# gavin-gqzhang/UniGen

Measured on NVIDIA B200. Metric: denoise steps/sec at 1024^2 Flux-arch +1 cond, higher is better.
Workload: dtype bf16

## Files before the change

### include/unigen_b200.h

```cpp
#ifndef UNIGEN_B200_H_
#define UNIGEN_B200_H_

#include <stddef.h>
#include <stdint.h>

#ifdef __cplusplus
extern "C" {
#endif

#define UG_ABI_VERSION 9

typedef enum {
  UG_OK = 0,
  UG_ERR_INVALID = -1,
  UG_ERR_UNSUPPORTED = -2,
  UG_ERR_CUDA = -3,
  UG_ERR_NO_DEVICE = -4
} ug_status;

const char* ug_last_error(void);
int ug_abi_version(void);
int ug_device_check(void);
int64_t ug_launch_count(void);
void ug_reset_launch_count(void);

#define UG_ACT_NONE 0
#define UG_ACT_GELU_TANH 1
#define UG_MAX_SEGMENTS 8
#define UG_MAX_PEERS 8
#define UG_PEER_HEADER_BYTES 4096
#define UG_PEER_HANDLE_BYTES 64

typedef struct ug_gemm_args {
  const void* a;
  int64_t a_row_stride;
  int64_t a_batch_stride;
  const void* w;
  int64_t w_row_stride;
  int64_t w_batch_stride;
  void* c;
  int64_t c_row_stride;
  int64_t c_batch_stride;
  int32_t batch;
  int32_t rows;
  int32_t n;
  int32_t k;
  const void* bias;
  int64_t bias_batch_stride;
  const float* gate;
  int64_t gate_batch_stride;
  float alpha;
  int32_t act;
  const void* residual;
  int64_t res_row_stride;
  int64_t res_batch_stride;
  int32_t variant;
  int32_t reserved;
  const float* lora_t;
  int64_t lora_t_row_stride;
  int64_t lora_t_batch_stride;
  const void* lora_b;
  int32_t lora_rank;
  int32_t lora_block_n;
  int32_t lora_nseg;
  int32_t lora_seg_bounds[UG_MAX_SEGMENTS + 1];
  int32_t lora_seg_group[UG_MAX_SEGMENTS];
  const void* qk_norm_weight;
  const float* qk_cos_sin;
  int32_t qk_head_dim;
  int32_t qk_d;
  float qk_eps;
  int32_t reserved2;
  int64_t gate_seg_stride;
  const void* a2;
  int64_t a2_row_stride, a2_batch_stride;
  const void* w2;
  int64_t w2_row_stride;
  int32_t k2;
  int32_t colmask_block;
} ug_gemm_args;

int ug_gemm_bf16(const ug_gemm_args* args, void* stream);

int ug_lora_down(const void* x, int64_t x_row_stride, int64_t x_batch_stride, const void* a_stack, float* t,
                 int64_t t_row_stride, int64_t t_batch_stride, int32_t batch, int32_t rows, int32_t k,
                 int32_t rank_total, int32_t nseg, const int32_t* seg_bounds_host, const int32_t* seg_group_host,
                 void* stream);
int ug_lora_down_wide(const void* x, int64_t x_row_stride, int64_t x_batch_stride, const void* a_stack, void* t_wide,
                      int64_t t_row_stride, int64_t t_batch_stride, int32_t batch, int32_t rows, int32_t k,
                      int32_t rank_total, int32_t groups, int32_t block, int32_t nseg, const int32_t* seg_bounds_host,
                      const int32_t* seg_group_host, void* stream);

typedef struct ug_attn_args {
  const void* q;
  const void* k;
  const void* v;
  void* o;
  int64_t q_row_stride, q_batch_stride;
  int64_t k_row_stride, k_batch_stride;
  int64_t v_row_stride, v_batch_stride;
  int64_t o_row_stride, o_batch_stride;
  int32_t batch, heads, seq, head_dim;
  float scale;
  int32_t n_seg;
  const int32_t* seg_bounds;
  const uint32_t* seg_visible;
  int32_t variant;
  int32_t reserved;
} ug_attn_args;

int ug_attention_bf16(const ug_attn_args* args, void* stream);
int ug_expand_segment_mask(int32_t seq, int32_t n_seg, const int32_t* seg_bounds_host,
                           const uint32_t* seg_visible_host, uint8_t* mask_dev, void* stream);

int ug_ln_modulate(const void* x, int64_t x_row_stride, int64_t x_batch_stride, void* out, int64_t o_row_stride,
                   int64_t o_batch_stride, const float* shift, const float* scale, int64_t mod_batch_stride,
                   int32_t batch, int32_t rows, int32_t d, float eps, void* stream);

int ug_ln_modulate_segs(const void* x, int64_t x_row_stride, int64_t x_batch_stride, void* out, int64_t o_row_stride,
                        int64_t o_batch_stride, const float* shift, const float* scale, int64_t mod_batch_stride,
                        int64_t mod_seg_stride, int32_t nseg, const int32_t* seg_bounds_host, int32_t batch, int32_t rows,
                        int32_t d, float eps, void* stream);

int ug_ln_modulate_slots(const void* x, int64_t x_row_stride, void* out, int64_t o_row_stride, const float* shift,
                         const float* scale, int64_t mod_expert_stride, int64_t mod_index_stride,
                         const int32_t* slot_token, int32_t experts, int32_t capacity, int32_t tokens_per_batch,
                         int32_t empty_index, int32_t d, float eps, void* stream);
int ug_gated_add_slots(void* x, int64_t x_row_stride, const void* y, int64_t y_row_stride, const float* gate,
                       int64_t mod_expert_stride, int64_t mod_index_stride, const int32_t* slot_token, int32_t experts,
                       int32_t capacity, int32_t tokens_per_batch, int32_t empty_index, int32_t d, void* stream);

int ug_qk_rmsnorm_rope(void* x, int64_t row_stride, int64_t batch_stride, int32_t batch, int32_t rows,
                       int32_t heads, int32_t head_dim, const void* norm_weight_bf16, int32_t heads_per_weight,
                       float eps, const float* cos_sin, void* stream);

int ug_rope_table(const float* ids, int32_t rows, const int32_t* axes_dim_host, float theta, float* cos_sin,
                  void* stream);

int ug_gemv(const float* x, int64_t x_stride, const void* w, const void* bias, float* out, int64_t out_stride,
            int32_t batch, int32_t n, int32_t k, int32_t silu_in, int32_t silu_out, int32_t accumulate,
            void* stream);

#define UG_MAX_GEMV_JOBS 1024
struct ug_peer_table;
typedef struct ug_gemv_job {
  const void* w;
  const void* bias;
  const float* x;
  float* out;
  int64_t x_stride, out_stride;
  int32_t n, k;
  int32_t first_group;
  int32_t flags;
} ug_gemv_job;
int ug_gemv_grouped(const ug_gemv_job* jobs_dev, int32_t n_jobs, int32_t total_groups, int32_t batch, int32_t group_begin,
                    int32_t group_end, const struct ug_peer_table* peers_or_null, void* stream);
int ug_silu_f32(const float* x, float* out, int64_t n, void* stream);

int ug_timestep_embedding(const float* t, int64_t t_stride, int32_t batch, int32_t dim, float scale, float* out, void* stream);

int ug_add_bf16(const void* a, int64_t a_row_stride, int64_t a_batch_stride, const void* b, int64_t b_row_stride,
                int64_t b_batch_stride, void* out, int64_t o_row_stride, int64_t o_batch_stride, int32_t batch,
                int32_t rows, int32_t d, void* stream);
int ug_copy_bf16(const void* src, int64_t s_row_stride, int64_t s_batch_stride, void* dst, int64_t d_row_stride,
                 int64_t d_batch_stride, int32_t batch, int32_t rows, int32_t d, void* stream);
int ug_cast_f32_to_bf16(const float* src, void* dst, int64_t n, void* stream);
int ug_cast_bf16_to_f32(const void* src, float* dst, int64_t n, void* stream);

int ug_moe_route(const void* x, const float* wg, const float* rts_uniform, int32_t tokens, int32_t d,
                 int32_t experts, int32_t capacity, int32_t* expert_idx, int32_t* slot, float* prob,
                 int32_t* slot_token, int64_t* exp_counts, float* l_aux, float* workspace, void* stream);

int ug_moe_gather_modulate(const void* x, const int32_t* slot_token, const float* mod, int64_t mod_expert_stride,
                           int64_t mod_batch_stride, const void* addend, void* out, int32_t experts,
                           int32_t capacity, int32_t tokens_per_batch, int32_t d, void* stream);
int ug_moe_combine(const void* y, const int32_t* expert_idx, const int32_t* slot, const float* prob, void* out,
                   int32_t tokens, int32_t capacity, int32_t d, void* stream);

int ug_euler_step(void* latents_bf16, const void* velocity_bf16, float sigma, float sigma_next, int64_t n, void* stream);
int ug_euler_step_table(void* latents_bf16, const void* velocity_bf16, const float* sigmas_dev, int32_t step, int64_t n,
                        void* stream);
int ug_cfg_combine(const void* uncond_bf16, const void* text_bf16, float guidance_scale, void* out_bf16, int64_t n, void* stream);
int ug_pack_latents(const void* src_bf16, void* dst_bf16, int32_t batch, int32_t channels, int32_t height, int32_t width,
                    int32_t unpack, void* stream);

typedef struct ug_peer_table {
  int32_t world, rank;
  void* base[UG_MAX_PEERS];
} ug_peer_table;

int ug_peer_alloc(size_t bytes, void** dev_ptr);
int ug_peer_free(void* dev_ptr);
int ug_peer_export(const void* dev_ptr, uint8_t handle[UG_PEER_HANDLE_BYTES]);
int ug_peer_open(const uint8_t handle[UG_PEER_HANDLE_BYTES], void** peer_ptr);
int ug_peer_close(void* peer_ptr);
int ug_peer_barrier(const ug_peer_table* table, void* stream);
int ug_peer_set_timeout_ms(int64_t milliseconds);
int ug_peer_error(const ug_peer_table* table, int32_t* error_host);
int ug_peer_error_async(const ug_peer_table* table, int32_t* error_host_pinned, void* stream);

typedef struct ug_qkv_scatter_args {
  const void* qkv;
  int64_t row_stride;
  int32_t rows, heads, head_dim;
  float eps;
  const void* norm_weight;
  const float* cos_sin;
  int64_t dst_offset;
  int32_t seq_total, dst_row0;
} ug_qkv_scatter_args;
int ug_qkv_scatter(const ug_peer_table* table, const ug_qkv_scatter_args* args, void* stream);

int ug_attention_bf16_peer(const ug_attn_args* args, const ug_peer_table* table, int64_t o_offset, int32_t rows_per_rank,
                           void* stream);

int ug_peer_bcast_rows(const ug_peer_table* table, const void* src, int64_t src_row_stride, int32_t rows, int32_t d,
                       int64_t dst_offset, int64_t dst_row_stride, int32_t dst_row0, void* stream);

int ug_unpatchify(const void* tokens_bf16, void* image_bf16, int32_t batch, int32_t h, int32_t w, int32_t p, int32_t channels,
                  void* stream);

#define UG_FLUX_MAX_CONDITIONS 4
typedef struct ug_flux_desc {
  int32_t num_layers, num_single_layers;
  int32_t heads, head_dim;
  int32_t in_channels, joint_dim, pooled_dim;
  int32_t guidance_embeds;
  int32_t axes_dims_rope[3];
  float theta;
  int32_t n_ctrl_double, n_ctrl_single;
  int32_t experts, condition_nums;
  int32_t use_shared_expert, single_add, use_pooled_prompt_embeds;
// ... 68 lines not shown
```

### unigen_b200/_lib.py

```python
from __future__ import annotations

import ctypes as C
from pathlib import Path

PKG_DIR = Path(__file__).resolve().parent
LIB_PATH = PKG_DIR / "libunigen_b200.so"

UG_ACT_NONE = 0
UG_ACT_GELU_TANH = 1
UG_MAX_SEGMENTS = 8
UG_GROUPNORM_MAX_CHUNKS = 1024
UG_ABI_VERSION = 9


class UgError(RuntimeError):
    pass


class GemmArgs(C.Structure):
    _fields_ = [
        ("a", C.c_void_p), ("a_row_stride", C.c_int64), ("a_batch_stride", C.c_int64),
        ("w", C.c_void_p), ("w_row_stride", C.c_int64), ("w_batch_stride", C.c_int64),
        ("c", C.c_void_p), ("c_row_stride", C.c_int64), ("c_batch_stride", C.c_int64),
        ("batch", C.c_int32), ("rows", C.c_int32), ("n", C.c_int32), ("k", C.c_int32),
        ("bias", C.c_void_p), ("bias_batch_stride", C.c_int64),
        ("gate", C.c_void_p), ("gate_batch_stride", C.c_int64),
        ("alpha", C.c_float), ("act", C.c_int32),
        ("residual", C.c_void_p), ("res_row_stride", C.c_int64), ("res_batch_stride", C.c_int64),
        ("variant", C.c_int32), ("reserved", C.c_int32),
        ("lora_t", C.c_void_p), ("lora_t_row_stride", C.c_int64), ("lora_t_batch_stride", C.c_int64),
        ("lora_b", C.c_void_p), ("lora_rank", C.c_int32), ("lora_block_n", C.c_int32), ("lora_nseg", C.c_int32),
        ("lora_seg_bounds", C.c_int32 * (UG_MAX_SEGMENTS + 1)), ("lora_seg_group", C.c_int32 * UG_MAX_SEGMENTS),
        ("qk_norm_weight", C.c_void_p), ("qk_cos_sin", C.c_void_p), ("qk_head_dim", C.c_int32), ("qk_d", C.c_int32),
        ("qk_eps", C.c_float), ("reserved2", C.c_int32), ("gate_seg_stride", C.c_int64),
        ("a2", C.c_void_p), ("a2_row_stride", C.c_int64), ("a2_batch_stride", C.c_int64),
        ("w2", C.c_void_p), ("w2_row_stride", C.c_int64), ("k2", C.c_int32), ("colmask_block", C.c_int32),
    ]


class Conv2dArgs(C.Structure):
    _fields_ = [("x", C.c_void_p), ("w", C.c_void_p), ("bias", C.c_void_p), ("residual", C.c_void_p), ("res_pixel_stride", C.c_int64),
                ("y", C.c_void_p), ("y_pixel_stride", C.c_int64), ("batch", C.c_int32), ("h", C.c_int32), ("w_px", C.c_int32),
                ("c_in", C.c_int32), ("c_out", C.c_int32), ("alpha", C.c_float), ("variant", C.c_int32), ("reserved", C.c_int32)]


UG_MAX_PEERS = 8
UG_PEER_HEADER_BYTES = 4096
UG_PEER_HANDLE_BYTES = 64


class PeerTable(C.Structure):
    _fields_ = [("world", C.c_int32), ("rank", C.c_int32), ("base", C.c_void_p * UG_MAX_PEERS)]


class QkvScatterArgs(C.Structure):
    _fields_ = [("qkv", C.c_void_p), ("row_stride", C.c_int64), ("rows", C.c_int32), ("heads", C.c_int32),
                ("head_dim", C.c_int32), ("eps", C.c_float), ("norm_weight", C.c_void_p), ("cos_sin", C.c_void_p),
                ("dst_offset", C.c_int64), ("seq_total", C.c_int32), ("dst_row0", C.c_int32)]


UG_MAX_GEMV_JOBS = 1024


class GemvJob(C.Structure):
    _fields_ = [("w", C.c_void_p), ("bias", C.c_void_p), ("x", C.c_void_p), ("out", C.c_void_p),
                ("x_stride", C.c_int64), ("out_stride", C.c_int64), ("n", C.c_int32), ("k", C.c_int32),
                ("first_group", C.c_int32), ("flags", C.c_int32)]


UG_FLUX_MAX_CONDITIONS = 4


class FluxDesc(C.Structure):
    _fields_ = [("num_layers", C.c_int32), ("num_single_layers", C.c_int32), ("heads", C.c_int32), ("head_dim", C.c_int32),
                ("in_channels", C.c_int32), ("joint_dim", C.c_int32), ("pooled_dim", C.c_int32), ("guidance_embeds", C.c_int32),
                ("axes_dims_rope", C.c_int32 * 3), ("theta", C.c_float), ("n_ctrl_double", C.c_int32), ("n_ctrl_single", C.c_int32),
                ("experts", C.c_int32), ("condition_nums", C.c_int32), ("use_shared_expert", C.c_int32), ("single_add", C.c_int32),
                ("use_pooled_prompt_embeds", C.c_int32)]


class FluxInputs(C.Structure):
    _fields_ = [("batch", C.c_int32), ("n_img", C.c_int32), ("n_txt", C.c_int32), ("conditioning_scale", C.c_float),
                ("hidden_states", C.c_void_p), ("encoder_hidden_states", C.c_void_p), ("pooled_projections", C.c_void_p),
                ("timestep", C.c_void_p), ("timestep_stride", C.c_int64), ("guidance", C.c_void_p), ("img_ids", C.c_void_p),
                ("txt_ids", C.c_void_p), ("condition_hidden_states", C.c_void_p * UG_FLUX_MAX_CONDITIONS),
                ("condition_pooled_projections", C.c_void_p * UG_FLUX_MAX_CONDITIONS),
                ("condition_ids", C.c_void_p * UG_FLUX_MAX_CONDITIONS), ("rts_uniform", C.c_void_p * UG_FLUX_MAX_CONDITIONS)]


class FluxOutputs(C.Structure):
    _fields_ = [("velocity", C.c_void_p), ("expert_counts", C.c_void_p), ("l_aux", C.c_void_p)]


class AttnArgs(C.Structure):
    _fields_ = [
        ("q", C.c_void_p), ("k", C.c_void_p), ("v", C.c_void_p), ("o", C.c_void_p),
        ("q_row_stride", C.c_int64), ("q_batch_stride", C.c_int64),
        ("k_row_stride", C.c_int64), ("k_batch_stride", C.c_int64),
        ("v_row_stride", C.c_int64), ("v_batch_stride", C.c_int64),
        ("o_row_stride", C.c_int64), ("o_batch_stride", C.c_int64),
        ("batch", C.c_int32), ("heads", C.c_int32), ("seq", C.c_int32), ("head_dim", C.c_int32),
        ("scale", C.c_float), ("n_seg", C.c_int32),
        ("seg_bounds", C.POINTER(C.c_int32)), ("seg_visible", C.POINTER(C.c_uint32)),
        ("variant", C.c_int32), ("reserved", C.c_int32),
    ]


_VP, _I32, _I64, _F32 = C.c_void_p, C.c_int32, C.c_int64, C.c_float
SIGNATURES = {
    "ug_last_error": (C.c_char_p, []),
    "ug_abi_version": (C.c_int, []),
    "ug_device_check": (C.c_int, []),
    "ug_launch_count": (C.c_int64, []),
    "ug_reset_launch_count": (None, []),
    "ug_gemm_bf16": (C.c_int, [C.POINTER(GemmArgs), _VP]),
    "ug_lora_down": (C.c_int, [_VP, _I64, _I64, _VP, _VP, _I64, _I64, _I32, _I32, _I32, _I32, _I32,
                               C.POINTER(C.c_int32), C.POINTER(C.c_int32), _VP]),
    "ug_lora_down_wide": (C.c_int, [_VP, _I64, _I64, _VP, _VP, _I64, _I64, _I32, _I32, _I32, _I32, _I32, _I32, _I32,
                                    C.POINTER(C.c_int32), C.POINTER(C.c_int32), _VP]),
    "ug_attention_bf16": (C.c_int, [C.POINTER(AttnArgs), _VP]),
    "ug_expand_segment_mask": (C.c_int, [_I32, _I32, C.POINTER(C.c_int32), C.POINTER(C.c_uint32), _VP, _VP]),
    "ug_ln_modulate": (C.c_int, [_VP, _I64, _I64, _VP, _I64, _I64, _VP, _VP, _I64, _I32, _I32, _I32, _F32, _VP]),
    "ug_ln_modulate_segs": (C.c_int, [_VP, _I64, _I64, _VP, _I64, _I64, _VP, _VP, _I64, _I64, _I32, C.POINTER(C.c_int32), _I32, _I32,
                                      _I32, _F32, _VP]),
    "ug_ln_modulate_slots": (C.c_int, [_VP, _I64, _VP, _I64, _VP, _VP, _I64, _I64, _VP, _I32, _I32, _I32, _I32, _I32, _F32, _VP]),
    "ug_gated_add_slots": (C.c_int, [_VP, _I64, _VP, _I64, _VP, _I64, _I64, _VP, _I32, _I32, _I32, _I32, _I32, _VP]),
    "ug_qk_rmsnorm_rope": (C.c_int, [_VP, _I64, _I64, _I32, _I32, _I32, _I32, _VP, _I32, _F32, _VP, _VP]),
    "ug_rope_table": (C.c_int, [_VP, _I32, C.POINTER(C.c_int32), _F32, _VP, _VP]),
    "ug_gemv": (C.c_int, [_VP, _I64, _VP, _VP, _VP, _I64, _I32, _I32, _I32, _I32, _I32, _I32, _VP]),
    "ug_gemv_grouped": (C.c_int, [_VP, _I32, _I32, _I32, _I32, _I32, C.POINTER(PeerTable), _VP]),
    "ug_silu_f32": (C.c_int, [_VP, _VP, _I64, _VP]),
    "ug_flux_create": (C.c_int, [C.POINTER(FluxDesc), C.POINTER(C.c_void_p)]),
    "ug_flux_destroy": (None, [_VP]),
    "ug_flux_bind_weight": (C.c_int, [_VP, C.c_char_p, _VP, _I32, C.POINTER(C.c_int64), _I32]),
    "ug_flux_workspace_bytes": (C.c_size_t, [_VP, _I32, _I32, _I32]),
    "ug_flux_forward": (C.c_int, [_VP, C.POINTER(FluxInputs), C.POINTER(FluxOutputs), _VP, C.c_size_t, _VP]),
    "ug_timestep_embedding": (C.c_int, [_VP, _I64, _I32, _I32, _F32, _VP, _VP]),
    "ug_add_bf16": (C.c_int, [_VP, _I64, _I64, _VP, _I64, _I64, _VP, _I64, _I64, _I32, _I32, _I32, _VP]),
    "ug_copy_bf16": (C.c_int, [_VP, _I64, _I64, _VP, _I64, _I64, _I32, _I32, _I32, _VP]),
    "ug_cast_f32_to_bf16": (C.c_int, [_VP, _VP, _I64, _VP]),
    "ug_cast_bf16_to_f32": (C.c_int, [_VP, _VP, _I64, _VP]),
    "ug_moe_route": (C.c_int, [_VP, _VP, _VP, _I32, _I32, _I32, _I32, _VP, _VP, _VP, _VP, _VP, _VP, _VP, _VP]),
    "ug_moe_gather_modulate": (C.c_int, [_VP, _VP, _VP, _I64, _I64, _VP, _VP, _I32, _I32, _I32, _I32, _VP]),
    "ug_moe_combine": (C.c_int, [_VP, _VP, _VP, _VP, _VP, _I32, _I32, _I32, _VP]),
    "ug_euler_step": (C.c_int, [_VP, _VP, _F32, _F32, _I64, _VP]),
    "ug_euler_step_table": (C.c_int, [_VP, _VP, _VP, _I32, _I64, _VP]),
    "ug_cfg_combine": (C.c_int, [_VP, _VP, _F32, _VP, _I64, _VP]),
    "ug_pack_latents": (C.c_int, [_VP, _VP, _I32, _I32, _I32, _I32, _I32, _VP]),
    "ug_peer_alloc": (C.c_int, [C.c_size_t, C.POINTER(C.c_void_p)]),
    "ug_peer_free": (C.c_int, [_VP]),
    "ug_peer_export": (C.c_int, [_VP, C.POINTER(C.c_uint8)]),
    "ug_peer_open": (C.c_int, [C.POINTER(C.c_uint8), C.POINTER(C.c_void_p)]),
    "ug_peer_close": (C.c_int, [_VP]),
    "ug_peer_barrier": (C.c_int, [C.POINTER(PeerTable), _VP]),
    "ug_peer_error": (C.c_int, [C.POINTER(PeerTable), C.POINTER(C.c_int32)]),
    "ug_peer_set_timeout_ms": (C.c_int, [_I64]),
    "ug_peer_error_async": (C.c_int, [C.POINTER(PeerTable), _VP, _VP]),
    "ug_qkv_scatter": (C.c_int, [C.POINTER(PeerTable), C.POINTER(QkvScatterArgs), _VP]),
    "ug_attention_bf16_peer": (C.c_int, [C.POINTER(AttnArgs), C.POINTER(PeerTable), _I64, _I32, _VP]),
    "ug_peer_bcast_rows": (C.c_int, [C.POINTER(PeerTable), _VP, _I64, _I32, _I32, _I64, _I64, _I32, _VP]),
    "ug_unpatchify": (C.c_int, [_VP, _VP, _I32, _I32, _I32, _I32, _I32, _VP]),
    "ug_conv3x3_bf16": (C.c_int, [C.POINTER(Conv2dArgs), _VP]),
    "ug_im2col_bf16": (C.c_int, [_VP, _I32, _I64, _I64, _I64, _I64, _VP, _I32, _I32, _I32, _I32, _I32, _I32, _I32, _I32, _I32, _I32, _I32,
                                 _I32, _F32, _F32, _VP]),
    "ug_groupnorm_bf16": (C.c_int, [_VP, _VP, _VP, _VP, _VP, _I32, _I32, _I32, _I32, _F32, _I32, _VP]),
    "ug_upsample2x_nhwc_bf16": (C.c_int, [_VP, _VP, _I32, _I32, _I32, _I32, _VP]),
    "ug_softmax_rows_bf16": (C.c_int, [_VP, _I64, _I32, _I32, _VP]),
    "ug_nhwc_to_nchw": (C.c_int, [_VP, _I64, _VP, _I32, _I32, _I32, _I32, _I32, _VP]),
    "ug_vae_sample": (C.c_int, [_VP, _I64, _VP, _VP, _I32, _I32, _I32, _F32, _F32, _VP]),
}

_lib = None


def load() -> C.CDLL:
    global _lib
    if _lib is not None:
        return _lib
    if not LIB_PATH.exists():
        raise UgError(
            f"{LIB_PATH} is missing: run `python -c 'import __graft_entry__ as g; g.build()'` "
            "(there is no CPU fallback for the UniGen hot path)")
    lib = C.CDLL(str(LIB_PATH))
    for name, (res, args) in SIGNATURES.items():
        fn = getattr(lib, name)
        fn.restype = res
        fn.argtypes = args
    got = int(lib.ug_abi_version())
    if got != UG_ABI_VERSION:
# ... 11 lines not shown
```

### unigen_b200/csrc/ug_flux.cu

```cuda
#include <cuda_bf16.h>

#include <cmath>
#include <cstring>
#include <map>
#include <string>
#include <vector>

#include "ug_host.h"

namespace {

struct Tensor {
  const void* p = nullptr;
  int dtype = 0;
  int64_t shape[4] = {0, 0, 0, 0};
  int ndim = 0;
};

struct Lin { const void* w = nullptr; const void* b = nullptr; };

struct DoubleW {
  Lin norm1, norm1_ctx, qkv, add_qkv, to_out, to_add_out, ff1, ff2, ffc1, ffc2;
  const void* rms = nullptr;
  const void* rms_ctx = nullptr;
};
struct SingleW { Lin norm, qkv, mlp, out; const void* rms = nullptr; };
struct TimeTextW { Lin t1, t2, g1, g2, p1, p2; };

struct View {
  void* p; int64_t rs, bs; int rows;
};

constexpr size_t kAlign = 256;
inline size_t align_up(size_t x) { return (x + kAlign - 1) / kAlign * kAlign; }

}

struct ug_flux {
  ug_flux_desc d;
  int D = 0;
  std::map<std::string, Tensor> weights;
  bool resolved = false;
  Lin x_embedder, context_embedder, norm_out, proj_out, control_context_embedder, control_x_embedder;
  TimeTextW time_text, control_time_text, control_condition;
  std::vector<DoubleW> dbl, cdbl, shared;
  std::vector<SingleW> sgl, csgl;
  std::vector<Lin> add_dbl, add_sgl;
  const float* gate_wg = nullptr;
  const void *exp_w[2] = {nullptr, nullptr}, *exp_b[2] = {nullptr, nullptr}, *exp_mod_w[2] = {nullptr, nullptr}, *exp_mod_b[2] = {nullptr, nullptr};
  cudaStream_t side = nullptr, text = nullptr;
  cudaEvent_t ev_fork = nullptr, ev_mod = nullptr, ev_t0 = nullptr, ev_t1 = nullptr;
  void* plan_ws = nullptr;
  int plan_B = 0, plan_N = 0, plan_T = 0;
  int early_jobs = 0, early_groups = 0, late_jobs = 0, late_groups = 0;
};

using namespace ug;

#define UG_TRY(expr)            \
  do {                          \
    int st__ = (expr);          \
    if (st__ != UG_OK) return st__; \
  } while (0)

extern "C" int ug_flux_create(const ug_flux_desc* desc, ug_flux** out) {
  UG_CHECK_ARG(desc && out, "flux_create: null argument");
  UG_CHECK_ARG(desc->num_layers >= 1 && desc->num_single_layers >= 0 && desc->heads >= 1 && (desc->head_dim == 64 || desc->head_dim == 128),
               "flux_create: bad architecture (head_dim must be 64 or 128)");
  UG_CHECK_ARG(desc->axes_dims_rope[0] + desc->axes_dims_rope[1] + desc->axes_dims_rope[2] == desc->head_dim,
               "flux_create: axes_dims_rope must sum to head_dim");
  UG_CHECK_ARG(desc->n_ctrl_double >= 1 && desc->n_ctrl_double <= desc->num_layers && desc->n_ctrl_single >= 0 &&
                   desc->n_ctrl_single <= desc->num_single_layers, "flux_create: control block counts out of range");
  UG_CHECK_ARG(desc->condition_nums >= 1 && desc->condition_nums <= UG_FLUX_MAX_CONDITIONS && desc->experts >= 1 && desc->experts <= 32,
               "flux_create: 1..%d conditions and 1..32 experts", UG_FLUX_MAX_CONDITIONS);
  ug_flux* h = new ug_flux();
  h->d = *desc;
  h->D = desc->heads * desc->head_dim;
  cudaError_t e = cudaStreamCreateWithFlags(&h->side, cudaStreamNonBlocking);
  if (e == cudaSuccess) e = cudaStreamCreateWithFlags(&h->text, cudaStreamNonBlocking);
  for (cudaEvent_t* ev : {&h->ev_fork, &h->ev_mod, &h->ev_t0, &h->ev_t1})
    if (e == cudaSuccess) e = cudaEventCreateWithFlags(ev, cudaEventDisableTiming);
  if (e != cudaSuccess) {
    set_error("flux_create: %s", cudaGetErrorString(e));
    delete h;
    return UG_ERR_CUDA;
  }
  *out = h;
  return UG_OK;
}

extern "C" void ug_flux_destroy(ug_flux* h) {
  if (!h) return;
  if (h->side) cudaStreamDestroy(h->side);
  if (h->text) cudaStreamDestroy(h->text);
  for (cudaEvent_t ev : {h->ev_fork, h->ev_mod, h->ev_t0, h->ev_t1})
    if (ev) cudaEventDestroy(ev);
  delete h;
}

extern "C" int ug_flux_bind_weight(ug_flux* h, const char* name, const void* dev_ptr, int32_t dtype, const int64_t* shape, int32_t ndim) {
  UG_CHECK_ARG(h && name && dev_ptr && shape && ndim >= 1 && ndim <= 4 && (dtype == 0 || dtype == 1), "flux_bind_weight: bad argument");
  Tensor t;
  t.p = dev_ptr; t.dtype = dtype; t.ndim = ndim;
  for (int i = 0; i < ndim; ++i) t.shape[i] = shape[i];
  h->weights[name] = t;
  h->resolved = false;
  h->plan_ws = nullptr;
  return UG_OK;
}

namespace {

struct Resolver {
  ug_flux* h;
  int status = UG_OK;
  const Tensor* get(const std::string& name, int dtype, int64_t s0, int64_t s1 = -1) {
    auto it = h->weights.find(name);
    if (it == h->weights.end()) { fail("weight %s is not bound", name); return nullptr; }
    const Tensor& t = it->second;
    if (t.dtype != dtype) { fail("weight %s has the wrong dtype", name); return nullptr; }
    if (t.shape[0] != s0 || (s1 >= 0 && (t.ndim < 2 || t.shape[1] != s1)) || (s1 < 0 && t.ndim != 1)) {
      fail("weight %s has the wrong shape", name);
      return nullptr;
    }
    return &t;
  }
  void fail(const char* fmt, const std::string& name) {
    if (status == UG_OK) { set_error(fmt, name.c_str()); status = UG_ERR_INVALID; }
  }
  Lin lin(const std::string& p, int64_t out_f, int64_t in_f) {
    Lin l;
    const Tensor* w = get(p + ".weight", 0, out_f, in_f);
    const Tensor* b = get(p + ".bias", 0, out_f);
    if (w && b) { l.w = w->p; l.b = b->p; }
    return l;
  }
  Lin fused(const std::vector<std::string>& names, int64_t out_each, int64_t in_f) {
    Lin first = lin(names[0], out_each, in_f);
    for (size_t i = 1; i < names.size() && status == UG_OK; ++i) {
      Lin l = lin(names[i], out_each, in_f);
      if (status != UG_OK) break;
      const char* want_w = static_cast<const char*>(first.w) + i * out_each * in_f * 2;
      const char* want_b = static_cast<const char*>(first.b) + i * out_each * 2;
      if (l.w != want_w || l.b != want_b) fail("%s: q / k / v (stacked expert) weights must be bound as one contiguous block", names[i]);
    }
    return first;
  }
  const void* rms_pair(const std::string& a, const std::string& b, int64_t dh) {
    const Tensor* ta = get(a, 0, dh);
    const Tensor* tb = get(b, 0, dh);
    if (!ta || !tb) return nullptr;
    if (static_cast<const char*>(tb->p) != static_cast<const char*>(ta->p) + dh * 2) fail("%s: norm_q / norm_k weights must be contiguous", b);
    return ta->p;
  }
  DoubleW dbl(const std::string& p, int64_t D, int64_t dh) {
    DoubleW w;
    w.norm1 = lin(p + ".norm1.linear", 6 * D, D);
    w.norm1_ctx = lin(p + ".norm1_context.linear", 6 * D, D);
    w.qkv = fused({p + ".attn.to_q", p + ".attn.to_k", p + ".attn.to_v"}, D, D);
    w.add_qkv = fused({p + ".attn.add_q_proj", p + ".attn.add_k_proj", p + ".attn.add_v_proj"}, D, D);
    w.to_out = lin(p + ".attn.to_out.0", D, D);
    w.to_add_out = lin(p + ".attn.to_add_out", D, D);
    w.rms = rms_pair(p + ".attn.norm_q.weight", p + ".attn.norm_k.weight", dh);
    w.rms_ctx = rms_pair(p + ".attn.norm_added_q.weight", p + ".attn.norm_added_k.weight", dh);
    w.ff1 = lin(p + ".ff.net.0.proj", 4 * D, D);
    w.ff2 = lin(p + ".ff.net.2", D, 4 * D);
    w.ffc1 = lin(p + ".ff_context.net.0.proj", 4 * D, D);
    w.ffc2 = lin(p + ".ff_context.net.2", D, 4 * D);
    return w;
  }
  SingleW sgl(const std::string& p, int64_t D, int64_t dh) {
    SingleW w;
    w.norm = lin(p + ".norm.linear", 3 * D, D);
    w.qkv = fused({p + ".attn.to_q", p + ".attn.to_k", p + ".attn.to_v"}, D, D);
    w.mlp = lin(p + ".proj_mlp", 4 * D, D);
    w.out = lin(p + ".proj_out", D, 5 * D);
    w.rms = rms_pair(p + ".attn.norm_q.weight", p + ".attn.norm_k.weight", dh);
    return w;
  }
  TimeTextW time_text(const std::string& p, int64_t D, int64_t pooled, bool guidance) {
    TimeTextW w;
    w.t1 = lin(p + ".timestep_embedder.linear_1", D, 256);
    w.t2 = lin(p + ".timestep_embedder.linear_2", D, D);
    if (guidance) {
      w.g1 = lin(p + ".guidance_embedder.linear_1", D, 256);
      w.g2 = lin(p + ".guidance_embedder.linear_2", D, D);
    }
    w.p1 = lin(p + ".text_embedder.linear_1", D, pooled);
    w.p2 = lin(p + ".text_embedder.linear_2", D, D);
    return w;
  }
};

int resolve(ug_flux* h) {
  if (h->resolved) return UG_OK;
  const ug_flux_desc& d = h->d;
  const int64_t D = h->D, dh = d.head_dim, P = d.pooled_dim, E = d.experts;
  Resolver r{h};
  auto idx = [](const char* p, int i) { return std::string(p) + "." + std::to_string(i); };
  h->x_embedder = r.lin("x_embedder", D, d.in_channels);
  h->context_embedder = r.lin("context_embedder", D, d.joint_dim);
  h->time_text = r.time_text("time_text_embed", D, P, d.guidance_embeds != 0);
  h->dbl.clear(); h->sgl.clear(); h->cdbl.clear(); h->csgl.clear(); h->add_dbl.clear(); h->add_sgl.clear(); h->shared.clear();
  for (int i = 0; i < d.num_layers; ++i) h->dbl.push_back(r.dbl(idx("transformer_blocks", i), D, dh));
  for (int i = 0; i < d.num_single_layers; ++i) h->sgl.push_back(r.sgl(idx("single_transformer_blocks", i), D, dh));
  h->norm_out = r.lin("norm_out.linear", 2 * D, D);
  h->proj_out = r.lin("proj_out", d.in_channels, D);
  h->control_time_text = r.time_text("control_time_text_embed", D, P, d.guidance_embeds != 0);
  h->control_condition = r.time_text("control_condition_embed", D, P, d.guidance_embeds != 0);
  h->control_context_embedder = r.lin("control_context_embedder", D, D);
  h->control_x_embedder = r.lin("control_x_embedder", D, d.in_channels);
  for (int j = 0; j < d.n_ctrl_double; ++j) {
    h->cdbl.push_back(r.dbl(idx("control_joint_trans_blocks", j), D, dh));
    h->add_dbl.push_back(r.lin(idx("controlnet_add_joint_blocks", j), D, D));
  }
  for (int j = 0; j < d.n_ctrl_single; ++j) {
    h->csgl.push_back(r.sgl(idx("control_single_trans_blocks", j), D, dh));
    h->add_sgl.push_back(r.lin(idx("controlnet_add_single_blocks", j), D, D));
  }
  if (const Tensor* g = r.get("moe.moe_layer.gate.wg.weight", 1, E, D)) h->gate_wg = static_cast<const float*>(g->p);
  for (int br = 0; br < 2; ++br) {
    std::vector<std::string> lin0, lin1;
    for (int e = 0; e < E; ++e) {
      const std::string p = "moe.moe_layer.experts.deepspeed_experts." + std::to_string(e) + "." + std::to_string(br);
      lin0.push_back(p + ".0");
      lin1.push_back(p + ".1");
    }
    Lin a = r.fused(lin0, D, D), m = r.fused(lin1, D, P);
    h->exp_w[br] = a.w; h->exp_b[br] = a.b; h->exp_mod_w[br] = m.w; h->exp_mod_b[br] = m.b;
  }
  if (d.use_shared_expert)
    for (int s = 0; s < 2; ++s) h->shared.push_back(r.dbl(idx("shared_expert", s), D, dh));
  if (r.status != UG_OK) return r.status;
  h->resolved = true;
  return UG_OK;
}

struct Layout {
  size_t X, NX, QKV, AO, FF, CAT, CH, CS, CENC, COND, HC, G, A, YC, YH, EH, EC, CIN, MOD, TEMBS, STEMBS, tmp, t_emb, g_emb, MODC, MODH,
      rope, rope0, rope1, NO, route_idx, route_slot, route_prob, route_slot_token, route_ws, jobs, total;
  int n_mod, capacity;
};

Layout make_layout(const ug_flux* h, int B, int N, int T) {
  const ug_flux_desc& d = h->d;
  const size_t D = h->D, S = T + N, Smax = T + 2 * (size_t)N, E = d.experts;
  Layout L;
  size_t off = 0;
  auto take = [&](size_t bytes) { size_t o = off; off = align_up(off + bytes); return o; };
  L.capacity = (int)((B * (size_t)N + E - 1) / E);
  if (L.capacity < 4) L.capacity = 4;
  const size_t C = L.capacity;
  L.n_mod = 12 * (d.num_layers + d.n_ctrl_double + 1 + d.condition_nums) + 3 * (d.num_single_layers + d.n_ctrl_single) + 2;
  L.X = take(B * S * D * 2); L.NX = take(B * Smax * D * 2); L.QKV = take(B * Smax * 3 * D * 2); L.AO = take(B * Smax * D * 2);
  L.FF = take(B * Smax * 4 * D * 2); L.CAT = take(B * S * 5 * D * 2); L.CH = take(B * (size_t)N * D * 2); L.CS = take(B * S * D * 2);
  L.CENC = take(B * (size_t)T * D * 2); L.COND = take(B * (size_t)N * D * 2); L.HC = take(B * 2 * (size_t)N * D * 2);
  L.G = take(B * (size_t)N * D * 2); L.A = take(E * C * D * 2); L.YC = take(E * C * D * 2); L.YH = take(E * C * D * 2);
  L.EH = take(B * (size_t)N * D * 2); L.EC = take(B * (size_t)N * D * 2); L.CIN = take(B * (size_t)N * D * 2);
  L.MOD = take((size_t)B * L.n_mod * D * 4);
  L.TEMBS = take((3 + d.condition_nums) * (size_t)B * D * 4); L.STEMBS = take((3 + d.condition_nums) * (size_t)B * D * 4);
  L.tmp = take((size_t)B * D * 4); L.t_emb = take((size_t)B * 256 * 4); L.g_emb = take((size_t)B * 256 * 4);
  L.MODC = take((size_t)B * E * D * 4); L.MODH = take((size_t)B * E * D * 4);
  L.rope = take(S * d.head_dim * 4); L.rope0 = take(2 * (size_t)N * d.head_dim * 4); L.rope1 = take(Smax * d.head_dim * 4);
  L.NO = take(B * (size_t)N * D * 2);
  L.route_idx = take((size_t)B * N * 4); L.route_slot = take((size_t)B * N * 4); L.route_prob = take((size_t)B * N * 4);
  L.route_slot_token = take(E * C * 4); L.route_ws = take(((size_t)B * N * E + E) * 4);
  L.jobs = take(UG_MAX_GEMV_JOBS * sizeof(ug_gemv_job));
  L.total = off;
  return L;
}

}

extern "C" size_t ug_flux_workspace_bytes(const ug_flux* h, int32_t batch, int32_t n_img, int32_t n_txt) {
  if (!h || batch < 1 || n_img < 1 || n_txt < 1) return 0;
  return make_layout(h, batch, n_img, n_txt).total;
}

namespace {

struct Step {
  ug_flux* h;
  const ug_flux_inputs* in;
  const ug_flux_outputs* out;
  char* ws;
  Layout L;
  cudaStream_t main;
  int B, N, T, S, D, H, dh, E;
  float cscale;
  float* mod(int slot) const { return reinterpret_cast<float*>(ws + L.MOD) + (size_t)slot * D; }
  int64_t mod_bs() const { return (int64_t)L.n_mod * D; }
  __nv_bfloat16* bf(size_t off) const { return reinterpret_cast<__nv_bfloat16*>(ws + off); }
  float* f32(size_t off) const { return reinterpret_cast<float*>(ws + off); }
  View view(size_t off, int row0, int rows, int64_t rs, int64_t total_rows) const {
    return View{bf(off) + (int64_t)row0 * rs, rs, total_rows * rs, rows};
  }

  int gemm(cudaStream_t s, View a, int k, Lin w, int n, View c, const float* gate = nullptr, const View* res = nullptr, int act = UG_ACT_NONE,
           float alpha = 1.0f, int batch = -1, int64_t w_batch_stride = 0, int64_t bias_batch_stride = 0, const void* qk_rms = nullptr,
           const float* qk_cos_sin = nullptr) const {
    ug_gemm_args g;
    memset(&g, 0, sizeof(g));
    g.a = a.p; g.a_row_stride = a.rs; g.a_batch_stride = a.bs;
    g.w = w.w; g.w_row_stride = k; g.w_batch_stride = w_batch_stride;
    g.c = c.p; g.c_row_stride = c.rs; g.c_batch_stride = c.bs;
    g.batch = batch < 0 ? B : batch; g.rows = a.rows; g.n = n; g.k = k;
    g.bias = w.b; g.bias_batch_stride = bias_batch_stride;
    g.gate = gate; g.gate_batch_stride = gate ? mod_bs() : 0;
    g.alpha = alpha; g.act = act;
    if (res) { g.residual = res->p; g.res_row_stride = res->rs; g.res_batch_stride = res->bs; }
    if (qk_rms) {
      g.qk_norm_weight = qk_rms; g.qk_cos_sin = qk_cos_sin; g.qk_head_dim = dh; g.qk_d = D; g.qk_eps = 1e-6f;
    }
    return ug_gemm_bf16(&g, s);
  }
  int ln(cudaStream_t s, View x, View o, const float* shift, const float* scale) const {
    return ug_ln_modulate(x.p, x.rs, x.bs, o.p, o.rs, o.bs, shift, scale, mod_bs(), B, x.rows, D, 1e-6f, s);
  }
  int gemv(const float* x, Lin w, float* o, int n, int k, int silu_out, int accumulate, int64_t x_stride, int64_t o_stride) const {
    return ug_gemv(x, x_stride, w.w, w.b, o, o_stride, B, n, k, 0, silu_out, accumulate, main);
  }
  int time_text(const TimeTextW& w, const float* pooled, int64_t pooled_stride, float* dst, bool accumulate) const {
    float* tmp = f32(L.tmp);
    UG_TRY(gemv(f32(L.t_emb), w.t1, tmp, D, 256, 1, 0, 256, D));
    UG_TRY(gemv(tmp, w.t2, dst, D, D, 0, accumulate ? 1 : 0, D, D));
    if (in->guidance && w.g1.w) {
      UG_TRY(gemv(f32(L.g_emb), w.g1, tmp, D, 256, 1, 0, 256, D));
      UG_TRY(gemv(tmp, w.g2, dst, D, D, 0, 1, D, D));
    }
    UG_TRY(gemv(pooled, w.p1, tmp, D, h->d.pooled_dim, 1, 0, pooled_stride, D));
    return gemv(tmp, w.p2, dst, D, D, 0, 1, D, D);
  }
  int rope(size_t off, std::initializer_list<std::pair<const float*, int>> tables) const {
    int r0 = 0;
    for (auto& t : tables) {
      UG_TRY(ug_rope_table(t.first, t.second, h->d.axes_dims_rope, h->d.theta, f32(off) + (size_t)r0 * dh, main));
      r0 += t.second;
    }
    return UG_OK;
  }
  int attention(int Sq, View o) const {
    ug_attn_args a;
    memset(&a, 0, sizeof(a));
    __nv_bfloat16* qkv = bf(L.QKV);
    const int64_t rs = 3 * (int64_t)D, bs = (int64_t)(T + 2 * N) * rs;
    a.q = qkv; a.k = qkv + D; a.v = qkv + 2 * D; a.o = o.p;
    a.q_row_stride = a.k_row_stride = a.v_row_stride = rs;
    a.q_batch_stride = a.k_batch_stride = a.v_batch_stride = bs;
    a.o_row_stride = o.rs; a.o_batch_stride = o.bs;
    a.batch = B; a.heads = H; a.seq = Sq; a.head_dim = dh;
    a.scale = (float)(1.0 / sqrt((double)dh));
    return ug_attention_bf16(&a, main);
  }
  int double_block(const DoubleW& w, int slot_smp, int slot_ctx, View smp_in, View ctx_in, View smp_out, const View* ctx_out, size_t rope_off) const {
    const int n_ctx = ctx_in.rows, n_smp = smp_in.rows, Sq = n_ctx + n_smp;
    const int64_t Smax = T + 2 * (int64_t)N;
    View nx_c = view(L.NX, 0, n_ctx, D, Smax), nx_s = view(L.NX, n_ctx, n_smp, D, Smax);
    View qkv_c = view(L.QKV, 0, n_ctx, 3 * D, Smax), qkv_s = view(L.QKV, n_ctx, n_smp, 3 * D, Smax);
    View ff_c = view(L.FF, 0, n_ctx, 4 * D, Smax), ff_s = view(L.FF, n_ctx, n_smp, 4 * D, Smax);
    View ao_c = view(L.AO, 0, n_ctx, D, Smax), ao_s = view(L.AO, n_ctx, n_smp, D, Smax), ao = view(L.AO, 0, Sq, D, Smax);
    const float *sh_a = mod(slot_smp), *sc_a = mod(slot_smp + 1), *g_a = mod(slot_smp + 2), *sh_m = mod(slot_smp + 3), *sc_m = mod(slot_smp + 4),
                *g_m = mod(slot_smp + 5);
    const float *csh_a = mod(slot_ctx), *csc_a = mod(slot_ctx + 1), *cg_a = mod(slot_ctx + 2), *csh_m = mod(slot_ctx + 3),
                *csc_m = mod(slot_ctx + 4), *cg_m = mod(slot_ctx + 5);
    const bool fork = ctx_out != nullptr;
    cudaStream_t ts = fork ? h->text : main;
    if (fork) { cudaEventRecord(h->ev_t0, main); cudaStreamWaitEvent(ts, h->ev_t0, 0); }
    const float* rp = f32(rope_off);
    UG_TRY(ln(ts, ctx_in, nx_c, csh_a, csc_a));
    UG_TRY(gemm(ts, nx_c, D, w.add_qkv, 3 * D, qkv_c, nullptr, nullptr, UG_ACT_NONE, 1.0f, -1, 0, 0, w.rms_ctx, rp));
    UG_TRY(ln(main, smp_in, nx_s, sh_a, sc_a));
    UG_TRY(gemm(main, nx_s, D, w.qkv, 3 * D, qkv_s, nullptr, nullptr, UG_ACT_NONE, 1.0f, -1, 0, 0, w.rms, rp + (size_t)n_ctx * dh));
    if (fork) { cudaEventRecord(h->ev_t1, ts); cudaStreamWaitEvent(main, h->ev_t1, 0); }
    UG_TRY(attention(Sq, ao));
    if (fork) {
      cudaEventRecord(h->ev_t0, main); cudaStreamWaitEvent(ts, h->ev_t0, 0);
      UG_TRY(gemm(ts, ao_c, D, w.to_add_out, D, *ctx_out, cg_a, &ctx_in));
      UG_TRY(ln(ts, *ctx_out, nx_c, csh_m, csc_m));
      UG_TRY(gemm(ts, nx_c, D, w.ffc1, 4 * D, ff_c, nullptr, nullptr, UG_ACT_GELU_TANH));
      UG_TRY(gemm(ts, ff_c, 4 * D, w.ffc2, D, *ctx_out, cg_m, ctx_out));
    }
    UG_TRY(gemm(main, ao_s, D, w.to_out, D, smp_out, g_a, &smp_in));
    UG_TRY(ln(main, smp_out, nx_s, sh_m, sc_m));
    UG_TRY(gemm(main, nx_s, D, w.ff1, 4 * D, ff_s, nullptr, nullptr, UG_ACT_GELU_TANH));
    UG_TRY(gemm(main, ff_s, 4 * D, w.ff2, D, smp_out, g_m, &smp_out));
    if (fork) { cudaEventRecord(h->ev_t1, ts); cudaStreamWaitEvent(main, h->ev_t1, 0); }
    return UG_OK;
  }

  int single_block(const SingleW& w, int slot, View x_in, View x_out) const {
    const int64_t Smax = T + 2 * (int64_t)N;
    View nx = view(L.NX, 0, S, D, Smax), qkv = view(L.QKV, 0, S, 3 * D, Smax);
    View cat = view(L.CAT, 0, S, 5 * D, S);
    View cat_attn = cat, cat_mlp = cat;
    cat_mlp.p = bf(L.CAT) + D;
    UG_TRY(ln(main, x_in, nx, mod(slot), mod(slot + 1)));
    UG_TRY(gemm(main, nx, D, w.qkv, 3 * D, qkv, nullptr, nullptr, UG_ACT_NONE, 1.0f, -1, 0, 0, w.rms, f32(L.rope)));
    UG_TRY(gemm(main, nx, D, w.mlp, 4 * D, cat_mlp, nullptr, nullptr, UG_ACT_GELU_TANH));
    UG_TRY(attention(S, cat_attn));
    return gemm(main, cat, 5 * D, w.out, D, x_out, mod(slot + 2), &x_in);
  }

  int add(View a, View b, View o) const {
    return ug_add_bf16(a.p, a.rs, a.bs, b.p, b.rs, b.bs, o.p, o.rs, o.bs, B, a.rows, D, main);
  }
};

struct JobBuilder {
  std::vector<ug_gemv_job> early, late;
  int g_early = 0, g_late = 0;
  void push(bool is_early, Lin w, const float* x, float* out, int n, int k, int64_t out_stride) {
    ug_gemv_job j;
    memset(&j, 0, sizeof(j));
    j.w = w.w; j.bias = w.b; j.x = x; j.out = out; j.x_stride = k; j.out_stride = out_stride; j.n = n; j.k = k; j.flags = 0;
    int& g = is_early ? g_early : g_late;
    j.first_group = g;
    g += (n + 3) / 4;
    (is_early ? early : late).push_back(j);
  }
};

}

extern "C" int ug_flux_forward(ug_flux* h, const ug_flux_inputs* in, const ug_flux_outputs* out, void* workspace, size_t workspace_bytes,
                               void* stream) {
  UG_CHECK_ARG(h && in && out && workspace, "flux_forward: null argument");
  UG_TRY(resolve(h));
  const ug_flux_desc& d = h->d;
  const int B = in->batch, N = in->n_img, T = in->n_txt, D = h->D, E = d.experts, n_cond = d.condition_nums;
  UG_CHECK_ARG(B >= 1 && B <= 8 && N >= 1 && T >= 1, "flux_forward: bad shape batch %d n_img %d n_txt %d (batch <= 8)", B, N, T);
  UG_CHECK_ARG(T != N, "flux_forward: T == N: the reference MOELayer would also dispatch the text tensor (unsupported)");
  UG_CHECK_ARG(in->hidden_states && in->encoder_hidden_states && in->pooled_projections && in->timestep && in->img_ids && in->txt_ids,
               "flux_forward: missing input");
  UG_CHECK_ARG(!in->guidance == !d.guidance_embeds || !in->guidance, "flux_forward: guidance given to a model without guidance embeddings");
  for (int c = 0; c < n_cond; ++c)
    UG_CHECK_ARG(in->condition_hidden_states[c] && in->condition_pooled_projections[c] && in->condition_ids[c] && in->rts_uniform[c],
                 "flux_forward: missing input of condition %d", c);
  UG_CHECK_ARG(out->velocity && out->expert_counts && out->l_aux, "flux_forward: missing output buffer");
  UG_CHECK_ARG((reinterpret_cast<uintptr_t>(workspace) & (kAlign - 1)) == 0, "flux_forward: workspace must be %d-byte aligned", (int)kAlign);
  Step s;
  s.h = h; s.in = in; s.out = out; s.ws = static_cast<char*>(workspace);
  s.L = make_layout(h, B, N, T);
  UG_CHECK_ARG(workspace_bytes >= s.L.total, "flux_forward: workspace of %zu bytes is smaller than ug_flux_workspace_bytes() = %zu",
               workspace_bytes, s.L.total);
  s.main = reinterpret_cast<cudaStream_t>(stream);
  s.B = B; s.N = N; s.T = T; s.S = T + N; s.D = D; s.H = d.heads; s.dh = d.head_dim; s.E = E;
  s.cscale = in->conditioning_scale;
  const Layout& L = s.L;
  const int S = s.S, C = L.capacity;
  const int64_t Smax = T + 2 * (int64_t)N;
  cudaStream_t main = s.main;

  const int nd = d.num_layers, ncd = d.n_ctrl_double, ns = d.num_single_layers, ncs = d.n_ctrl_single;
  std::vector<int> s_d(nd), s_dc(nd), s_cd(ncd), s_cdc(ncd), s_s(ns), s_cs(ncs), s_sh0(n_cond), s_sh0c(n_cond);
  int s_sh1 = 0, s_sh1c = 0, s_out = 0, slot = 0;
  float* stembs = s.f32(L.STEMBS);
  const float *s_temb = stembs, *s_ctemb = stembs + (size_t)B * D, *s_cdtemb = stembs + 2 * (size_t)B * D;
  JobBuilder jb;
  const int64_t mbs = s.mod_bs();
  auto job = [&](bool early, Lin w, const float* x, int chunks) {
    const int s0 = slot;
    slot += chunks;
    jb.push(early, w, x, s.mod(s0), chunks * D, D, mbs);
    return s0;
  };
  for (int i = 0; i < nd; ++i) { s_d[i] = job(i == 0, h->dbl[i].norm1, s_temb, 6); s_dc[i] = job(i == 0, h->dbl[i].norm1_ctx, s_temb, 6); }
  for (int j = 0; j < ncd; ++j) { s_cd[j] = job(j == 0, h->cdbl[j].norm1, s_cdtemb, 6); s_cdc[j] = job(j == 0, h->cdbl[j].norm1_ctx, s_cdtemb, 6); }
  for (int i = 0; i < ns; ++i) s_s[i] = job(false, h->sgl[i].norm, s_temb, 3);
  for (int j = 0; j < ncs; ++j) s_cs[j] = job(false, h->csgl[j].norm, s_cdtemb, 3);
  if (d.use_shared_expert) {
    for (int c = 0; c < n_cond; ++c) {
      const float* x = stembs + (size_t)(3 + c) * B * D;
      s_sh0[c] = job(true, h->shared[0].norm1, x, 6);
      s_sh0c[c] = job(true, h->shared[0].norm1_ctx, x, 6);
    }
    s_sh1 = job(true, h->shared[1].norm1, s_ctemb, 6);
    s_sh1c = job(true, h->shared[1].norm1_ctx, s_ctemb, 6);
  }
  s_out = job(false, h->norm_out, s_temb, 2);
  UG_CHECK_ARG(slot <= L.n_mod && jb.early.size() + jb.late.size() <= UG_MAX_GEMV_JOBS, "flux_forward: AdaLN job table overflow");
  ug_gemv_job* jobs_dev = reinterpret_cast<ug_gemv_job*>(s.ws + L.jobs);
  if (h->plan_ws != workspace || h->plan_B != B || h->plan_N != N || h->plan_T != T) {
    std::vector<ug_gemv_job> all(jb.early);
    all.insert(all.end(), jb.late.begin(), jb.late.end());
    cudaError_t e = cudaMemcpyAsync(jobs_dev, all.data(), all.size() * sizeof(ug_gemv_job), cudaMemcpyHostToDevice, main);
    if (e == cudaSuccess) e = cudaStreamSynchronize(main);
    if (e != cudaSuccess) {
      set_error("flux_forward: uploading the AdaLN job table failed: %s", cudaGetErrorString(e));
      return UG_ERR_CUDA;
    }
    h->plan_ws = workspace; h->plan_B = B; h->plan_N = N; h->plan_T = T;
  }

  View X = s.view(L.X, 0, S, D, S), x_txt = s.view(L.X, 0, T, D, S), x_img = s.view(L.X, T, N, D, S);
  View hs{const_cast<void*>(in->hidden_states), d.in_channels, (int64_t)N * d.in_channels, N};
  View es{const_cast<void*>(in->encoder_hidden_states), d.joint_dim, (int64_t)T * d.joint_dim, T};
  UG_TRY(s.gemm(main, hs, d.in_channels, h->x_embedder, D, x_img));
  UG_TRY(s.gemm(main, es, d.joint_dim, h->context_embedder, D, x_txt));
  UG_TRY(ug_timestep_embedding(in->timestep, in->timestep_stride, B, 256, 1000.0f, s.f32(L.t_emb), main));
  if (in->guidance) UG_TRY(ug_timestep_embedding(in->guidance, 1, B, 256, 1000.0f, s.f32(L.g_emb), main));
  float* tembs = s.f32(L.TEMBS);
  float *temb = tembs, *ctemb = tembs + (size_t)B * D, *cdtemb = tembs + 2 * (size_t)B * D;
  const int64_t P = d.pooled_dim;
  UG_TRY(s.time_text(h->time_text, in->pooled_projections, P, temb, false));
  if (d.use_pooled_prompt_embeds) {
    UG_TRY(s.time_text(h->control_time_text, in->pooled_projections, P, ctemb, false));
  } else {
    cudaMemsetAsync(s.f32(L.MODC), 0, (size_t)B * P * 4, main);
    UG_TRY(s.time_text(h->control_time_text, s.f32(L.MODC), P, ctemb, false));
  }
  for (int c = 0; c < n_cond; ++c) {
    UG_TRY(s.time_text(h->control_condition, in->condition_pooled_projections[c], P, tembs + (size_t)(3 + c) * B * D, false));
    UG_TRY(s.time_text(h->control_condition, in->condition_pooled_projections[c], P, cdtemb, c > 0));
  }
  UG_TRY(ug_silu_f32(tembs, stembs, (int64_t)(3 + n_cond) * B * D, main));
  UG_TRY(s.rope(L.rope, {{in->txt_ids, T}, {in->img_ids, N}}));

  const int n_early = (int)jb.early.size(), n_late = (int)jb.late.size();
  UG_TRY(ug_gemv_grouped(jobs_dev, n_early, jb.g_early, B, 0, jb.g_early, nullptr, main));
  cudaEventRecord(h->ev_fork, main);
  cudaStreamWaitEvent(h->side, h->ev_fork, 0);
  UG_TRY(ug_gemv_grouped(jobs_dev + n_early, n_late, jb.g_late, B, 0, jb.g_late, nullptr, h->side));
  cudaEventRecord(h->ev_mod, h->side);
  bool mods_joined = false;

  View CENC = s.view(L.CENC, 0, T, D, T), CH = s.view(L.CH, 0, N, D, N), CIN = s.view(L.CIN, 0, N, D, N), COND = s.view(L.COND, 0, N, D, N);
  bool routed = false;
  for (int i = 0; i < nd; ++i) {
    if (i == 1 && !mods_joined) { cudaStreamWaitEvent(main, h->ev_mod, 0); mods_joined = true; }
    UG_TRY(s.double_block(h->dbl[i], s_d[i], s_dc[i], x_img, x_txt, x_img, &x_txt, L.rope));
    const int j = (int)((double)i / ((double)nd / (double)ncd));
    View ctrl_in = x_img;
    if (!routed) {
      UG_TRY(s.gemm(main, x_txt, D, h->control_context_embedder, D, CENC));
      for (int c = 0; c < n_cond; ++c) {
        View cs{const_cast<void*>(in->condition_hidden_states[c]), d.in_channels, (int64_t)N * d.in_channels, N};
        UG_TRY(s.gemm(main, cs, d.in_channels, h->control_x_embedder, D, COND));
        UG_TRY(s.rope(L.rope0, {{in->condition_ids[c], N}, {in->img_ids, N}}));
        UG_TRY(s.rope(L.rope1, {{in->txt_ids, T}, {in->img_ids, N}, {in->condition_ids[c], N}}));
        View G = s.view(L.G, 0, N, D, N);
// ... 64 lines not shown
```

### unigen_b200/csrc/ug_gemm.cu

```cuda
#include <cstdlib>
#include <cstring>

#include "ug_host.h"
#include "ug_ptx.cuh"

namespace ug {

constexpr int kEpiWarps = 8;
constexpr int kGemmThreads = 64 + 32 * kEpiWarps;

struct GemmParams {
  int rows, n, k, batch;
  int m_tiles, n_tiles, k_blocks, total_tiles;
  int group_m;
  int k1_blocks;
  __nv_bfloat16* c;
  long long c_rs, c_bs;
  const __nv_bfloat16* bias;
  long long bias_bs;
  const float* gate;
  long long gate_bs;
  int colmask_block;
  long long gate_seg_stride;
  float alpha;
  int act;
  const __nv_bfloat16* res;
  long long res_rs, res_bs;
  int w_batched;
  const float* lora_t;
  long long lora_t_rs, lora_t_bs;
  const __nv_bfloat16* lora_b;
  int lora_r, lora_block_n, lora_nseg;
  int lora_bounds[UG_MAX_SEGMENTS + 1];
  int lora_group[UG_MAX_SEGMENTS];
  const __nv_bfloat16* qk_w;
  const float* qk_cos_sin;
  int qk_dh, qk_d;
  float qk_eps;
  int conv_cblocks, conv_w;
};

struct ConvDesc {
  const void* x;
  int batch, h, w, c_in;
};

template <int kCta, int BN, int kStages, bool kTmaEpi = false>
struct GemmCfg {
  static constexpr int BM = 128;
  static constexpr int BK = 64;
  static constexpr int BN_LOAD = BN / kCta;
  static constexpr int A_BYTES = BM * BK * 2;
  static constexpr int B_BYTES = BN_LOAD * BK * 2;
  static constexpr int STAGE_BYTES = A_BYTES + B_BYTES;
  static constexpr int TMEM_COLS = 2 * BN;
  static constexpr int EPI_SLABS = BN / (64 * (kEpiWarps / 4));
  static constexpr int EPI_SLAB_BYTES = 32 * 128;
  static constexpr int EPI_WARP_BYTES = EPI_SLABS * EPI_SLAB_BYTES;
  static constexpr int EPI_BYTES = kTmaEpi ? kEpiWarps * EPI_WARP_BYTES : 0;
  static constexpr int EPI_BARS = kTmaEpi ? kEpiWarps * EPI_SLABS : 0;
  static constexpr int BAR_BYTES = (2 * kStages + 4 + EPI_BARS) * 8 + 16;
  static constexpr int SMEM_BYTES = kStages * STAGE_BYTES + EPI_BYTES + BAR_BYTES + 1024;
  static_assert(TMEM_COLS == 256 || TMEM_COLS == 512, "TMEM allocation must be a power of two");
  static_assert(SMEM_BYTES <= 227 * 1024, "shared memory budget");
};

__device__ __forceinline__ int lora_group_of(const GemmParams& p, int r) {
  int g = -1;
  for (int s = 0; s < p.lora_nseg; ++s)
    if (r >= p.lora_bounds[s] && r < p.lora_bounds[s + 1]) g = p.lora_group[s];
  return g;
}

__device__ __forceinline__ int seg_index_of(const GemmParams& p, int r) {
  int g = 0;
  for (int s = 0; s < p.lora_nseg; ++s)
    if (r >= p.lora_bounds[s] && r < p.lora_bounds[s + 1]) g = s;
  return g;
}

__device__ __forceinline__ void epilogue_chunk(const GemmParams& p, const uint32_t (&v)[32], int b, int r, int col0,
                                               int lora_g, const float* gate_row) {
  const long long c_off = (long long)b * p.c_bs + (long long)r * p.c_rs;
  const long long r_off = (long long)b * p.res_bs + (long long)r * p.res_rs;
  uint4 rv4[4];
  if (p.res) {
#pragma unroll
    for (int j = 0; j < 4; ++j)
      rv4[j] = (col0 + 8 * j < p.n) ? *reinterpret_cast<const uint4*>(p.res + r_off + col0 + 8 * j) : make_uint4(0, 0, 0, 0);
  }
  float lt[16];
  const __nv_bfloat16* lb = nullptr;
  if (lora_g >= 0) {
    const float* tp = p.lora_t + (long long)b * p.lora_t_bs + (long long)r * p.lora_t_rs + (col0 / p.lora_block_n) * p.lora_r;
#pragma unroll
    for (int i = 0; i < 16; i += 4) {
      if (i < p.lora_r) {
        const float4 t4 = *reinterpret_cast<const float4*>(tp + i);
        lt[i] = t4.x; lt[i + 1] = t4.y; lt[i + 2] = t4.z; lt[i + 3] = t4.w;
      }
    }
    lb = p.lora_b + ((long long)lora_g * p.n) * p.lora_r;
  }
#pragma unroll
  for (int j = 0; j < 4; ++j) {
    const int c = col0 + 8 * j;
    if (c >= p.n) break;
    float x[8];
#pragma unroll
    for (int i = 0; i < 8; ++i) x[i] = __uint_as_float(v[8 * j + i]);
    if (lb) {
#pragma unroll
      for (int i = 0; i < 8; ++i) {
        const __nv_bfloat16* bp = lb + (long long)(c + i) * p.lora_r;
        float acc = 0.f;
#pragma unroll
        for (int q = 0; q < 16; q += 4) {
          if (q < p.lora_r) {
            const uint2 u = *reinterpret_cast<const uint2*>(bp + q);
            const float2 b0 = unpack_bf16x2(u.x), b1 = unpack_bf16x2(u.y);
            acc += lt[q] * b0.x + lt[q + 1] * b0.y + lt[q + 2] * b1.x + lt[q + 3] * b1.y;
          }
        }
        x[i] += acc;
      }
    }
    if (p.bias) {
      uint4 bv = *reinterpret_cast<const uint4*>(p.bias + (long long)b * p.bias_bs + c);
      float2 f0 = unpack_bf16x2(bv.x), f1 = unpack_bf16x2(bv.y), f2 = unpack_bf16x2(bv.z), f3 = unpack_bf16x2(bv.w);
      x[0] += f0.x; x[1] += f0.y; x[2] += f1.x; x[3] += f1.y;
      x[4] += f2.x; x[5] += f2.y; x[6] += f3.x; x[7] += f3.y;
    }
    if (p.act == UG_ACT_GELU_TANH) {
#pragma unroll
      for (int i = 0; i < 8; ++i) x[i] = gelu_tanh(x[i]);
    }
    if (gate_row) {
      const float* g = gate_row + c;
      float4 g0 = *reinterpret_cast<const float4*>(g), g1 = *reinterpret_cast<const float4*>(g + 4);
      x[0] *= g0.x * p.alpha; x[1] *= g0.y * p.alpha; x[2] *= g0.z * p.alpha; x[3] *= g0.w * p.alpha;
      x[4] *= g1.x * p.alpha; x[5] *= g1.y * p.alpha; x[6] *= g1.z * p.alpha; x[7] *= g1.w * p.alpha;
    } else if (p.alpha != 1.0f) {
#pragma unroll
      for (int i = 0; i < 8; ++i) x[i] *= p.alpha;
    }
    if (p.res) {
      const uint4 rv = rv4[j];
      float2 f0 = unpack_bf16x2(rv.x), f1 = unpack_bf16x2(rv.y), f2 = unpack_bf16x2(rv.z), f3 = unpack_bf16x2(rv.w);
      x[0] += f0.x; x[1] += f0.y; x[2] += f1.x; x[3] += f1.y;
      x[4] += f2.x; x[5] += f2.y; x[6] += f3.x; x[7] += f3.y;
    }
    uint4 o;
    o.x = pack_bf16x2(x[0], x[1]);
    o.y = pack_bf16x2(x[2], x[3]);
    o.z = pack_bf16x2(x[4], x[5]);
    o.w = pack_bf16x2(x[6], x[7]);
    *reinterpret_cast<uint4*>(p.c + c_off + c) = o;
  }
}

__device__ __forceinline__ uint4 epilogue_group8(const GemmParams& p, const uint32_t* v8, int b, int c, const float* gate_row,
                                                 const uint4& rv) {
  float x[8];
#pragma unroll
  for (int i = 0; i < 8; ++i) x[i] = __uint_as_float(v8[i]);
  if (p.bias) {
    const uint4 bv = *reinterpret_cast<const uint4*>(p.bias + (long long)b * p.bias_bs + c);
    const float2 f0 = unpack_bf16x2(bv.x), f1 = unpack_bf16x2(bv.y), f2 = unpack_bf16x2(bv.z), f3 = unpack_bf16x2(bv.w);
    x[0] += f0.x; x[1] += f0.y; x[2] += f1.x; x[3] += f1.y;
    x[4] += f2.x; x[5] += f2.y; x[6] += f3.x; x[7] += f3.y;
  }
  if (p.act == UG_ACT_GELU_TANH) {
#pragma unroll
    for (int i = 0; i < 8; ++i) x[i] = gelu_tanh(x[i]);
  }
  if (gate_row) {
    const float* g = gate_row + c;
    const float4 g0 = *reinterpret_cast<const float4*>(g), g1 = *reinterpret_cast<const float4*>(g + 4);
    x[0] *= g0.x * p.alpha; x[1] *= g0.y * p.alpha; x[2] *= g0.z * p.alpha; x[3] *= g0.w * p.alpha;
    x[4] *= g1.x * p.alpha; x[5] *= g1.y * p.alpha; x[6] *= g1.z * p.alpha; x[7] *= g1.w * p.alpha;
  } else if (p.alpha != 1.0f) {
#pragma unroll
    for (int i = 0; i < 8; ++i) x[i] *= p.alpha;
  }
  if (p.res) {
    const float2 f0 = unpack_bf16x2(rv.x), f1 = unpack_bf16x2(rv.y), f2 = unpack_bf16x2(rv.z), f3 = unpack_bf16x2(rv.w);
    x[0] += f0.x; x[1] += f0.y; x[2] += f1.x; x[3] += f1.y;
    x[4] += f2.x; x[5] += f2.y; x[6] += f3.x; x[7] += f3.y;
  }
  uint4 o;
  o.x = pack_bf16x2(x[0], x[1]);
  o.y = pack_bf16x2(x[2], x[3]);
  o.z = pack_bf16x2(x[4], x[5]);
  o.w = pack_bf16x2(x[6], x[7]);
  return o;
}

__device__ __forceinline__ uint4 epilogue_qk_group8(const GemmParams& p, const uint32_t* v8, int b, int r, int c, int which, float rstd) {
  const int c_in_head = c % p.qk_dh;
  float x[8];
#pragma unroll
  for (int i = 0; i < 8; ++i) x[i] = __uint_as_float(v8[i]);
  if (p.bias) {
    const uint4 bv = *reinterpret_cast<const uint4*>(p.bias + (long long)b * p.bias_bs + c);
    const float2 f0 = unpack_bf16x2(bv.x), f1 = unpack_bf16x2(bv.y), f2 = unpack_bf16x2(bv.z), f3 = unpack_bf16x2(bv.w);
    x[0] += f0.x; x[1] += f0.y; x[2] += f1.x; x[3] += f1.y;
    x[4] += f2.x; x[5] += f2.y; x[6] += f3.x; x[7] += f3.y;
  }
  const uint4 wv = *reinterpret_cast<const uint4*>(p.qk_w + which * p.qk_dh + c_in_head);
  const float2 w0 = unpack_bf16x2(wv.x), w1 = unpack_bf16x2(wv.y), w2 = unpack_bf16x2(wv.z), w3 = unpack_bf16x2(wv.w);
  x[0] *= rstd * w0.x; x[1] *= rstd * w0.y; x[2] *= rstd * w1.x; x[3] *= rstd * w1.y;
  x[4] *= rstd * w2.x; x[5] *= rstd * w2.y; x[6] *= rstd * w3.x; x[7] *= rstd * w3.y;
  if (p.qk_cos_sin) {
    const float* cs = p.qk_cos_sin + (long long)min(r, p.rows - 1) * p.qk_dh + c_in_head;
    const float4 t0 = __ldg(reinterpret_cast<const float4*>(cs)), t1 = __ldg(reinterpret_cast<const float4*>(cs + 4));
    const float co[4] = {t0.x, t0.z, t1.x, t1.z}, si[4] = {t0.y, t0.w, t1.y, t1.w};
#pragma unroll
    for (int q = 0; q < 4; ++q) {
      const float a0 = x[2 * q], a1 = x[2 * q + 1];
      x[2 * q] = a0 * co[q] - a1 * si[q];
      x[2 * q + 1] = a1 * co[q] + a0 * si[q];
    }
  }
  uint4 o;
  o.x = pack_bf16x2(x[0], x[1]);
  o.y = pack_bf16x2(x[2], x[3]);
  o.z = pack_bf16x2(x[4], x[5]);
  o.w = pack_bf16x2(x[6], x[7]);
  return o;
}

__device__ __forceinline__ void epilogue_qkv_chunk(const GemmParams& p, const uint32_t (&v)[32], int b, int r, int col0,
                                                   int c_in_head, int which, float rstd) {
  const long long c_off = (long long)b * p.c_bs + (long long)r * p.c_rs;
  const float* cs = (which < 2 && p.qk_cos_sin) ? p.qk_cos_sin + (long long)r * p.qk_dh + c_in_head : nullptr;
  const __nv_bfloat16* wq = p.qk_w + which * p.qk_dh + c_in_head;
#pragma unroll
  for (int j = 0; j < 4; ++j) {
    const int c = col0 + 8 * j;
    float x[8];
#pragma unroll
    for (int i = 0; i < 8; ++i) x[i] = __uint_as_float(v[8 * j + i]);
    if (p.bias) {
      uint4 bv = *reinterpret_cast<const uint4*>(p.bias + (long long)b * p.bias_bs + c);
      float2 f0 = unpack_bf16x2(bv.x), f1 = unpack_bf16x2(bv.y), f2 = unpack_bf16x2(bv.z), f3 = unpack_bf16x2(bv.w);
      x[0] += f0.x; x[1] += f0.y; x[2] += f1.x; x[3] += f1.y;
      x[4] += f2.x; x[5] += f2.y; x[6] += f3.x; x[7] += f3.y;
    }
    if (which < 2) {
      uint4 wv = *reinterpret_cast<const uint4*>(wq + 8 * j);
      float2 w0 = unpack_bf16x2(wv.x), w1 = unpack_bf16x2(wv.y), w2 = unpack_bf16x2(wv.z), w3 = unpack_bf16x2(wv.w);
      x[0] *= rstd * w0.x; x[1] *= rstd * w0.y; x[2] *= rstd * w1.x; x[3] *= rstd * w1.y;
      x[4] *= rstd * w2.x; x[5] *= rstd * w2.y; x[6] *= rstd * w3.x; x[7] *= rstd * w3.y;
      if (cs) {
        const float4 t0 = *reinterpret_cast<const float4*>(cs + 8 * j), t1 = *reinterpret_cast<const float4*>(cs + 8 * j + 4);
        const float co[4] = {t0.x, t0.z, t1.x, t1.z}, si[4] = {t0.y, t0.w, t1.y, t1.w};
#pragma unroll
        for (int q = 0; q < 4; ++q) {
          const float a0 = x[2 * q], a1 = x[2 * q + 1];
          x[2 * q] = a0 * co[q] - a1 * si[q];
          x[2 * q + 1] = a1 * co[q] + a0 * si[q];
        }
      }
    }
    uint4 o;
    o.x = pack_bf16x2(x[0], x[1]);
    o.y = pack_bf16x2(x[2], x[3]);
    o.z = pack_bf16x2(x[4], x[5]);
    o.w = pack_bf16x2(x[6], x[7]);
    *reinterpret_cast<uint4*>(p.c + c_off + c) = o;
  }
}

__device__ __forceinline__ float chunk_sumsq(const GemmParams& p, const uint32_t (&v)[32], int b, int col0) {
  float ss = 0.f;
#pragma unroll
  for (int j = 0; j < 4; ++j) {
    float x[8];
#pragma unroll
    for (int i = 0; i < 8; ++i) x[i] = __uint_as_float(v[8 * j + i]);
    if (p.bias) {
      uint4 bv = *reinterpret_cast<const uint4*>(p.bias + (long long)b * p.bias_bs + col0 + 8 * j);
      float2 f0 = unpack_bf16x2(bv.x), f1 = unpack_bf16x2(bv.y), f2 = unpack_bf16x2(bv.z), f3 = unpack_bf16x2(bv.w);
      x[0] += f0.x; x[1] += f0.y; x[2] += f1.x; x[3] += f1.y;
      x[4] += f2.x; x[5] += f2.y; x[6] += f3.x; x[7] += f3.y;
    }
#pragma unroll
    for (int i = 0; i < 8; ++i) ss += x[i] * x[i];
  }
  return ss;
}

__device__ __forceinline__ void tile_coords(const GemmParams& p, int tile, int mb_count, int& mb, int& nt) {
  const int band = p.group_m * p.n_tiles;
  const int g = tile / band, in_band = tile - g * band;
  const int first = g * p.group_m;
  const int size = min(mb_count - first, p.group_m);
  mb = first + in_band % size;
  nt = in_band / size;
}

template <int kCta, int BN, int kStages, bool kTmaEpi>
__global__ void __launch_bounds__(kGemmThreads, 1)
gemm_bf16_kernel(const __grid_constant__ CUtensorMap tma_a, const __grid_constant__ CUtensorMap tma_w,
                 const __grid_constant__ CUtensorMap tma_a2, const __grid_constant__ CUtensorMap tma_w2,
                 const __grid_constant__ CUtensorMap tma_c, const __grid_constant__ CUtensorMap tma_r, const GemmParams p) {
  using Cfg = GemmCfg<kCta, BN, kStages, kTmaEpi>;
  extern __shared__ uint8_t smem_raw[];
  uint8_t* smem = smem_raw + ((1024u - (smem_u32(smem_raw) & 1023u)) & 1023u);
  uint8_t* smem_a = smem;
  uint8_t* smem_b = smem + kStages * Cfg::A_BYTES;
  uint8_t* smem_epi = smem + kStages * Cfg::STAGE_BYTES;
  uint64_t* full = reinterpret_cast<uint64_t*>(smem + kStages * Cfg::STAGE_BYTES + Cfg::EPI_BYTES);
  uint64_t* empty = full + kStages;
  uint64_t* tmem_full = empty + kStages;
  uint64_t* tmem_empty = tmem_full + 2;
  uint64_t* res_bars = tmem_empty + 2;
  uint32_t* tmem_slot = reinterpret_cast<uint32_t*>(res_bars + Cfg::EPI_BARS);

  const int warp = threadIdx.x >> 5;
  const int lane = threadIdx.x & 31;
  const uint32_t cta_rank = (kCta == 2) ? cluster_ctarank() : 0u;

  if (warp == 0 && lane == 0) {
    tma_prefetch_desc(&tma_a);
    tma_prefetch_desc(&tma_w);
    if (p.k1_blocks < p.k_blocks) {
      tma_prefetch_desc(&tma_a2);
      tma_prefetch_desc(&tma_w2);
    }
    for (int s = 0; s < kStages; ++s) {
      mbar_init(&full[s], 1);
      mbar_init(&empty[s], 1);
    }
    for (int s = 0; s < 2; ++s) {
      mbar_init(&tmem_full[s], 1);
      mbar_init(&tmem_empty[s], kEpiWarps * kCta);
    }
    for (int s = 0; s < Cfg::EPI_BARS; ++s) mbar_init(&res_bars[s], 1);
    if constexpr (kTmaEpi) {
      tma_prefetch_desc(&tma_c);
      if (p.res) tma_prefetch_desc(&tma_r);
    }
    fence_mbar_init();
  }
  if (warp == 1) tmem_alloc<kCta>(tmem_slot, Cfg::TMEM_COLS);
  tc_fence_before();
  if constexpr (kCta == 2) cluster_sync_all(); else __syncthreads();
  tc_fence_after();
  const uint32_t tmem_base = *tmem_slot;

  const int unit = (kCta == 2) ? (blockIdx.x >> 1) : blockIdx.x;
  const int num_units = (kCta == 2) ? (gridDim.x >> 1) : gridDim.x;
  const int mb_count = p.m_tiles * p.batch;

  if (warp == 0) {
    int stage = 0;
    uint32_t phase = 0;
    for (int tile = unit; tile < p.total_tiles; tile += num_units) {
      int mb, nt;
      tile_coords(p, tile, mb_count, mb, nt);
      const int b = mb / p.m_tiles, mt = mb % p.m_tiles;
      const int row0 = mt * (Cfg::BM * kCta) + (int)cta_rank * Cfg::BM;
      const int wrow0 = nt * BN + (int)cta_rank * Cfg::BN_LOAD;
      const int wb = p.w_batched ? b : 0;
      int conv_y0 = 0, conv_x0 = 0, conv_tap = 0, conv_cb = 0;
      if (p.conv_cblocks) {
        conv_y0 = row0 / p.conv_w;
        conv_x0 = row0 - conv_y0 * p.conv_w;
      }
      for (int kb = 0; kb < p.k_blocks; ++kb) {
        mbar_wait(&empty[stage], phase ^ 1);
        if (elect_one_sync()) {
          void* sa = smem_a + stage * Cfg::A_BYTES;
          void* sb = smem_b + stage * Cfg::B_BYTES;
          if (p.conv_cblocks) {
            const int dy = conv_tap / 3, dx = conv_tap - 3 * dy;
            if constexpr (kCta == 1) {
              mbar_arrive_expect_tx(&full[stage], Cfg::STAGE_BYTES);
              tma_load_4d(sa, &tma_a, &full[stage], conv_cb * Cfg::BK, conv_x0 + dx - 1, conv_y0 + dy - 1, b);
              tma_load_3d(sb, &tma_w, &full[stage], kb * Cfg::BK, wrow0, 0);
            } else {
              if (cta_rank == 0) mbar_arrive_expect_tx(&full[stage], 2 * Cfg::STAGE_BYTES);
              tma_load_4d_2sm(sa, &tma_a, &full[stage], conv_cb * Cfg::BK, conv_x0 + dx - 1, conv_y0 + dy - 1, b);
              tma_load_3d_2sm(sb, &tma_w, &full[stage], kb * Cfg::BK, wrow0, 0);
            }
          } else {
            const bool second = kb >= p.k1_blocks;
            const CUtensorMap* ma = second ? &tma_a2 : &tma_a;
            const CUtensorMap* mw = second ? &tma_w2 : &tma_w;
            const int kc = (second ? kb - p.k1_blocks : kb) * Cfg::BK;
            if constexpr (kCta == 1) {
              mbar_arrive_expect_tx(&full[stage], Cfg::STAGE_BYTES);
              tma_load_3d(sa, ma, &full[stage], kc, row0, b);
              tma_load_3d(sb, mw, &full[stage], kc, wrow0, second ? 0 : wb);
            } else {
              if (cta_rank == 0) mbar_arrive_expect_tx(&full[stage], 2 * Cfg::STAGE_BYTES);
              tma_load_3d_2sm(sa, ma, &full[stage], kc, row0, b);
              tma_load_3d_2sm(sb, mw, &full[stage], kc, wrow0, second ? 0 : wb);
            }
          }
        }
        if (p.conv_cblocks && ++conv_cb == p.conv_cblocks) { conv_cb = 0; ++conv_tap; }
        __syncwarp();
        if (++stage == kStages) { stage = 0; phase ^= 1; }
      }
    }
  } else if (warp == 1) {
    if (cta_rank == 0) {
      constexpr uint32_t idesc = make_idesc_bf16(Cfg::BM * kCta, BN, false, false);
      int stage = 0;
      uint32_t phase = 0;
      int it = 0;
      for (int tile = unit; tile < p.total_tiles; tile += num_units, ++it) {
        const int as = it & 1;
        const uint32_t aphase = (it >> 1) & 1;
        mbar_wait(&tmem_empty[as], aphase ^ 1);
        tc_fence_after();
        const uint32_t d_tmem = tmem_base + as * BN;
        for (int kb = 0; kb < p.k_blocks; ++kb) {
          mbar_wait(&full[stage], phase);
          tc_fence_after();
          if (elect_one_sync()) {
            const uint64_t a_desc = make_sdesc_sw128(smem_u32(smem_a + stage * Cfg::A_BYTES), 16, 1024);
            const uint64_t b_desc = make_sdesc_sw128(smem_u32(smem_b + stage * Cfg::B_BYTES), 16, 1024);
#pragma unroll
            for (int k = 0; k < Cfg::BK / 16; ++k) {
              umma_ss<kCta>(d_tmem, a_desc + 2 * k, b_desc + 2 * k, idesc, (kb | k) != 0 ? 1u : 0u);
            }
            if constexpr (kCta == 1) {
              umma_commit(&empty[stage]);
              if (kb == p.k_blocks - 1) umma_commit(&tmem_full[as]);
            } else {
              umma_commit_2sm(&empty[stage], 0b11);
              if (kb == p.k_blocks - 1) umma_commit_2sm(&tmem_full[as], 0b11);
            }
          }
          __syncwarp();
          if (++stage == kStages) { stage = 0; phase ^= 1; }
        }
      }
    }
  } else {
    const int q = warp & 3;
    const int col_half = (warp - 2) >> 2;
    const int row_local = q * 32 + lane;
    uint32_t res_phase = 0;
    (void)res_phase;
    int it = 0;
    for (int tile = unit; tile < p.total_tiles; tile += num_units, ++it) {
      int mb, nt;
      tile_coords(p, tile, mb_count, mb, nt);
      const int b = mb / p.m_tiles, mt = mb % p.m_tiles;
      const int r = mt * (Cfg::BM * kCta) + (int)cta_rank * Cfg::BM + row_local;
      const int n0 = nt * BN;
      const int as = it & 1;
      const uint32_t aphase = (it >> 1) & 1;
      if constexpr (!kTmaEpi) {
        mbar_wait(&tmem_full[as], aphase);
        tc_fence_after();
      }
      const uint32_t taddr = tmem_base + ((uint32_t)(q * 32) << 16) + as * BN;
      const int lora_g = (p.lora_t || p.colmask_block) ? lora_group_of(p, r) : -1;
      const float* gate_row = p.gate ? p.gate + (long long)b * p.gate_bs + (p.gate_seg_stride ? seg_index_of(p, r) * p.gate_seg_stride : 0)
                                     : nullptr;
      auto release_acc = [&]() {
        tc_fence_before();
        __syncwarp();
        if (lane == 0) {
          if (kCta == 1 || cta_rank == 0) mbar_arrive(&tmem_empty[as]);
          else mbar_arrive_cluster(&tmem_empty[as], 0);
        }
      };
      if constexpr (kTmaEpi) {
        const int ew = warp - 2;
        uint8_t* slab0 = smem_epi + ew * Cfg::EPI_WARP_BYTES;
        uint64_t* rbar = res_bars + ew * Cfg::EPI_SLABS;
        const int r0 = mt * (Cfg::BM * kCta) + (int)cta_rank * Cfg::BM + q * 32;
        const int cw0 = n0 + col_half * (BN / (kEpiWarps / 4));
        if (lane == 0) bulk_wait_group_read<0>();
        __syncwarp();
        if (p.res && lane == 0) {
#pragma unroll
          for (int sl = 0; sl < Cfg::EPI_SLABS; ++sl) {
            if (cw0 + 64 * sl < p.n) {
              mbar_arrive_expect_tx(&rbar[sl], Cfg::EPI_SLAB_BYTES);
              tma_load_3d(slab0 + sl * Cfg::EPI_SLAB_BYTES, &tma_r, &rbar[sl], cw0 + 64 * sl, r0, b);
            }
          }
        }
        mbar_wait(&tmem_full[as], aphase);
        tc_fence_after();
        constexpr int kChunksPerWarp = (BN / 32) / (kEpiWarps / 4);
        const int ch0 = col_half * kChunksPerWarp;
        int qk_which = 2;
        float qk_rstd[2] = {1.f, 1.f};
        if constexpr (BN == 256) {
          if (p.qk_w && cw0 < p.n) qk_which = cw0 / p.qk_d;
          if (qk_which < 2) {
            float ss[2] = {0.f, 0.f};
#pragma unroll
            for (int ch = 0; ch < kChunksPerWarp; ++ch) {
              uint32_t v[32];
              tmem_ld_32x32(taddr + (ch0 + ch) * 32, v);
              tmem_ld_wait();
              if (cw0 + 32 * ch < p.n) ss[(p.qk_dh == 64) ? (ch >> 1) : 0] += chunk_sumsq(p, v, b, cw0 + 32 * ch);
            }
            if (p.qk_dh != 64) ss[1] = ss[0];
            qk_rstd[0] = rsqrtf(ss[0] / (float)p.qk_dh + p.qk_eps);
            qk_rstd[1] = rsqrtf(ss[1] / (float)p.qk_dh + p.qk_eps);
          }
        }
#pragma unroll 1
        for (int sl = 0; sl < Cfg::EPI_SLABS; ++sl) {
          const int cs0 = cw0 + 64 * sl;
          const bool active = cs0 < p.n;
          uint8_t* slab = slab0 + sl * Cfg::EPI_SLAB_BYTES;
          if (p.res && active) {
            mbar_wait(&rbar[sl], (res_phase >> sl) & 1u);
            res_phase ^= 1u << sl;
          }
#pragma unroll
          for (int h = 0; h < 2; ++h) {
            uint32_t v[32];
            tmem_ld_32x32(taddr + (ch0 + 2 * sl + h) * 32, v);
            tmem_ld_wait();
            if (sl == Cfg::EPI_SLABS - 1 && h == 1) release_acc();
            if (active) {
#pragma unroll
              for (int j = 0; j < 4; ++j) {
                const int c = cs0 + 32 * h + 8 * j;
                uint4* cell = reinterpret_cast<uint4*>(slab + lane * 128 + (((4 * h + j) ^ (lane & 7)) << 4));
                if (c < p.n) {
                  if (qk_which < 2) *cell = epilogue_qk_group8(p, &v[8 * j], b, r, c, qk_which, sl == 0 ? qk_rstd[0] : qk_rstd[1]);
                  else *cell = epilogue_group8(p, &v[8 * j], b, c, gate_row, p.res ? *cell : make_uint4(0, 0, 0, 0));
                }
              }
            }
          }
          if (active) {
            fence_proxy_async_smem();
            __syncwarp();
            if (lane == 0) {
              tma_store_3d(&tma_c, slab, cs0, r0, b);
              bulk_commit_group();
            }
          }
        }
      } else if (p.qk_w) {
        const int cph = p.qk_dh >> 5;
        constexpr int kHalf = BN / (kEpiWarps / 4);
        const bool split = (kHalf % p.qk_dh) == 0;
        const int c_lo = split ? col_half * kHalf : 0;
        const int c_hi = split ? c_lo + kHalf : (col_half == 0 ? BN : 0);
        if (c_hi == 0) release_acc();
#pragma unroll 1
        for (int c_h = c_lo; c_h < c_hi; c_h += p.qk_dh) {
          const int col_h = n0 + c_h;
          const bool active = col_h < p.n;
          const int which = active ? col_h / p.qk_d : 2;
          float rstd = 1.f;
          if (which < 2) {
            float ss = 0.f;
#pragma unroll 1
            for (int ch = 0; ch < cph; ++ch) {
              uint32_t v[32];
              tmem_ld_32x32(taddr + c_h + ch * 32, v);
              tmem_ld_wait();
              ss += chunk_sumsq(p, v, b, col_h + ch * 32);
            }
            rstd = rsqrtf(ss / (float)p.qk_dh + p.qk_eps);
          }
#pragma unroll 1
          for (int ch = 0; ch < cph; ++ch) {
            uint32_t v[32];
            tmem_ld_32x32(taddr + c_h + ch * 32, v);
            tmem_ld_wait();
            if (c_h + p.qk_dh >= c_hi && ch == cph - 1) release_acc();
            if (r < p.rows && active) epilogue_qkv_chunk(p, v, b, r, col_h + ch * 32, ch * 32, which, rstd);
          }
        }
      } else {
        constexpr int kChunksPerWarp = (BN / 32) / (kEpiWarps / 4);
        const int ch0 = col_half * kChunksPerWarp;
#pragma unroll 1
        for (int ch = ch0; ch < ch0 + kChunksPerWarp; ++ch) {
          uint32_t v[32];
          tmem_ld_32x32(taddr + ch * 32, v);
          tmem_ld_wait();
          if (ch == ch0 + kChunksPerWarp - 1) release_acc();
          const int col0 = n0 + ch * 32;
          if (p.colmask_block && col0 / p.colmask_block != lora_g) {
#pragma unroll
            for (int i = 0; i < 32; ++i) v[i] = 0u;
            if (r < p.rows && col0 < p.n) epilogue_chunk(p, v, b, r, col0, -1, nullptr);
          } else if (r < p.rows && col0 < p.n) epilogue_chunk(p, v, b, r, col0, p.lora_t ? lora_g : -1, gate_row);
        }
      }
    }
  }

  if constexpr (kTmaEpi) {
    if (warp >= 2 && lane == 0) bulk_wait_group<0>();
  }
  tc_fence_before();
  if constexpr (kCta == 2) cluster_sync_all(); else __syncthreads();
  if (warp == 1) {
    tc_fence_after();
    tmem_dealloc<kCta>(tmem_base, Cfg::TMEM_COLS);
  }
}

template <int kCta, int BN, int kStages, bool kTmaEpi = false>
static int launch_gemm(const ug_gemm_args& a, cudaStream_t stream, const ConvDesc* conv = nullptr) {
  using Cfg = GemmCfg<kCta, BN, kStages, kTmaEpi>;
  auto kern = gemm_bf16_kernel<kCta, BN, kStages, kTmaEpi>;
  static bool attr_done[64] = {false};
  if (int st = ensure_dynamic_smem(kern, Cfg::SMEM_BYTES, attr_done, "gemm"); st != UG_OK) return st;
  CUtensorMap tma_a, tma_w;
  if (conv) {
    const uint32_t bw = conv->w % Cfg::BM == 0 ? (uint32_t)Cfg::BM : (uint32_t)conv->w;
    uint64_t dims[4] = {(uint64_t)conv->c_in, (uint64_t)conv->w, (uint64_t)conv->h, (uint64_t)conv->batch};
    uint64_t strides[3] = {(uint64_t)conv->c_in * 2, (uint64_t)conv->w * conv->c_in * 2, (uint64_t)conv->h * conv->w * conv->c_in * 2};
    uint32_t box[4] = {(uint32_t)Cfg::BK, bw, (uint32_t)Cfg::BM / bw, 1};
    int st = encode_tmap_bf16(&tma_a, conv->x, 4, dims, strides, box);
    if (st != UG_OK) return st;
  } else {
    uint64_t dims[3] = {(uint64_t)a.k, (uint64_t)a.rows, (uint64_t)a.batch};
    uint64_t bs = a.batch > 1 ? (uint64_t)a.a_batch_stride : (uint64_t)a.rows * a.a_row_stride;
    uint64_t strides[2] = {(uint64_t)a.a_row_stride * 2, bs * 2};
    uint32_t box[3] = {(uint32_t)Cfg::BK, (uint32_t)Cfg::BM, 1};
    int st = encode_tmap_bf16(&tma_a, a.a, 3, dims, strides, box);
    if (st != UG_OK) return st;
  }
  const bool w_batched = a.w_batch_stride != 0 && a.batch > 1;
  {
    uint64_t dims[3] = {(uint64_t)a.k, (uint64_t)a.n, (uint64_t)(w_batched ? a.batch : 1)};
    uint64_t bs = w_batched ? (uint64_t)a.w_batch_stride : (uint64_t)a.n * a.w_row_stride;
    uint64_t strides[2] = {(uint64_t)a.w_row_stride * 2, bs * 2};
    uint32_t box[3] = {(uint32_t)Cfg::BK, (uint32_t)Cfg::BN_LOAD, 1};
    int st = encode_tmap_bf16(&tma_w, a.w, 3, dims, strides, box);
    if (st != UG_OK) return st;
  }
  CUtensorMap tma_a2 = tma_a, tma_w2 = tma_w;
  int k2_blocks = 0;
  if (a.a2) {
    {
      uint64_t dims[3] = {(uint64_t)a.k2, (uint64_t)a.rows, (uint64_t)a.batch};
      uint64_t bs = a.batch > 1 ? (uint64_t)a.a2_batch_stride : (uint64_t)a.rows * a.a2_row_stride;
      uint64_t strides[2] = {(uint64_t)a.a2_row_stride * 2, bs * 2};
      uint32_t box[3] = {(uint32_t)Cfg::BK, (uint32_t)Cfg::BM, 1};
      int st = encode_tmap_bf16(&tma_a2, a.a2, 3, dims, strides, box);
      if (st != UG_OK) return st;
    }
    {
      uint64_t dims[3] = {(uint64_t)a.k2, (uint64_t)a.n, 1};
      uint64_t strides[2] = {(uint64_t)a.w2_row_stride * 2, (uint64_t)a.n * a.w2_row_stride * 2};
      uint32_t box[3] = {(uint32_t)Cfg::BK, (uint32_t)Cfg::BN_LOAD, 1};
      int st = encode_tmap_bf16(&tma_w2, a.w2, 3, dims, strides, box);
      if (st != UG_OK) return st;
    }
    k2_blocks = (a.k2 + Cfg::BK - 1) / Cfg::BK;
  }
  CUtensorMap tma_c = tma_a, tma_r = tma_a;
  if constexpr (kTmaEpi) {
    uint32_t box[3] = {64, 32, 1};
    {
      uint64_t dims[3] = {(uint64_t)a.n, (uint64_t)a.rows, (uint64_t)a.batch};
      uint64_t bs = a.batch > 1 ? (uint64_t)a.c_batch_stride : (uint64_t)a.rows * a.c_row_stride;
      uint64_t strides[2] = {(uint64_t)a.c_row_stride * 2, bs * 2};
      int st = encode_tmap_bf16(&tma_c, a.c, 3, dims, strides, box);
      if (st != UG_OK) return st;
    }
    if (a.residual) {
      uint64_t dims[3] = {(uint64_t)a.n, (uint64_t)a.rows, (uint64_t)a.batch};
      uint64_t bs = a.batch > 1 ? (uint64_t)a.res_batch_stride : (uint64_t)a.rows * a.res_row_stride;
      uint64_t strides[2] = {(uint64_t)a.res_row_stride * 2, bs * 2};
      int st = encode_tmap_bf16(&tma_r, a.residual, 3, dims, strides, box);
      if (st != UG_OK) return st;
    }
  }
  GemmParams p;
  p.rows = a.rows; p.n = a.n; p.k = a.k; p.batch = a.batch;
  p.m_tiles = (a.rows + Cfg::BM * kCta - 1) / (Cfg::BM * kCta);
  p.n_tiles = (a.n + BN - 1) / BN;
  {
    const long long a_bytes = (long long)a.batch * a.rows * (a.k + (a.a2 ? a.k2 : 0)) * 2;
    const int mb_all = p.m_tiles * a.batch;
    p.group_m = mb_all;
    if (a_bytes > (40LL << 20) && !(a.w_batch_stride != 0 && a.batch > 1)) {
      const long long tile_bytes = (long long)Cfg::BM * kCta * (a.k + (a.a2 ? a.k2 : 0)) * 2;
      long long gm = (24LL << 20) / tile_bytes;
      gm = gm < 2 ? 2 : (gm > 16 ? 16 : gm);
      p.group_m = gm < mb_all ? (int)gm : mb_all;
    }
  }
  p.k1_blocks = (a.k + Cfg::BK - 1) / Cfg::BK;
  p.k_blocks = p.k1_blocks + k2_blocks;
  p.total_tiles = p.m_tiles * p.n_tiles * a.batch;
  p.c = (__nv_bfloat16*)a.c; p.c_rs = a.c_row_stride; p.c_bs = a.c_batch_stride;
  p.bias = (const __nv_bfloat16*)a.bias; p.bias_bs = a.bias_batch_stride;
  p.gate = a.gate; p.gate_bs = a.gate_batch_stride; p.gate_seg_stride = a.gate_seg_stride; p.colmask_block = a.colmask_block;
  p.alpha = a.alpha; p.act = a.act;
  p.res = (const __nv_bfloat16*)a.residual; p.res_rs = a.res_row_stride; p.res_bs = a.res_batch_stride;
  p.w_batched = w_batched ? 1 : 0;
  p.qk_w = (const __nv_bfloat16*)a.qk_norm_weight; p.qk_cos_sin = a.qk_cos_sin; p.qk_dh = a.qk_head_dim;
  p.qk_d = a.qk_d; p.qk_eps = a.qk_eps;
  p.conv_cblocks = conv ? conv->c_in / Cfg::BK : 0;
  p.conv_w = conv ? conv->w : 0;
  p.lora_t = a.lora_t; p.lora_t_rs = a.lora_t_row_stride; p.lora_t_bs = a.lora_t_batch_stride;
  p.lora_b = (const __nv_bfloat16*)a.lora_b;
  p.lora_r = a.lora_rank; p.lora_block_n = a.lora_block_n > 0 ? a.lora_block_n : a.n; p.lora_nseg = a.lora_nseg;
  for (int i = 0; i <= UG_MAX_SEGMENTS; ++i) p.lora_bounds[i] = i <= a.lora_nseg ? a.lora_seg_bounds[i] : a.rows;
  for (int i = 0; i < UG_MAX_SEGMENTS; ++i) p.lora_group[i] = i < a.lora_nseg ? a.lora_seg_group[i] : -1;

  const int sms = num_sms();
  int units = kCta == 2 ? sms / 2 : sms;
  if (units > p.total_tiles) units = p.total_tiles;
  cudaLaunchConfig_t cfg = {};
  cfg.gridDim = dim3(units * kCta);
  cfg.blockDim = dim3(kGemmThreads);
  cfg.dynamicSmemBytes = Cfg::SMEM_BYTES;
  cfg.stream = stream;
  cudaLaunchAttribute attr[1];
  attr[0].id = cudaLaunchAttributeClusterDimension;
  attr[0].val.clusterDim.x = kCta;
  attr[0].val.clusterDim.y = 1;
  attr[0].val.clusterDim.z = 1;
  cfg.attrs = attr;
  cfg.numAttrs = 1;
  cudaError_t e = cudaLaunchKernelEx(&cfg, kern, tma_a, tma_w, tma_a2, tma_w2, tma_c, tma_r, p);
  if (e != cudaSuccess) {
    set_error("gemm: launch failed: %s", cudaGetErrorString(e));
    return UG_ERR_CUDA;
  }
  count_launch();
  return UG_OK;
}

static bool staged_epilogue_default() {
  static int cached = -1;
  if (cached < 0) {
    const char* e = getenv("UG_GEMM_EPILOGUE");
    cached = (e && strcmp(e, "direct") == 0) ? 0 : 1;
  }
  return cached == 1;
}

static int pick_tile_variant(int batch, int rows, int n) {
  const int sms = num_sms();
  struct Cand { int v, tm, tn; double rate; int units; };
  const Cand cands[3] = {{2, 256, 256, 2.0, sms / 2}, {1, 128, 256, 0.98, sms}, {3, 128, 128, 0.67, sms}};
  double best = 0.0;
  int variant = 0;
  for (const Cand& c : cands) {
    const long long tiles = (long long)batch * ((rows + c.tm - 1) / c.tm) * ((n + c.tn - 1) / c.tn);
    const long long waves = (tiles + c.units - 1) / c.units;
    const double t = (double)waves * c.tm * c.tn / c.rate;
    if (variant == 0 || t < best) { best = t; variant = c.v; }
  }
  return variant;
}

}

extern "C" int ug_gemm_bf16(const ug_gemm_args* args, void* stream) {
  using namespace ug;
  UG_CHECK_ARG(args != nullptr, "gemm: null args");
  const ug_gemm_args& a = *args;
  UG_CHECK_ARG(a.a && a.w && a.c, "gemm: null operand pointer");
  UG_CHECK_ARG(a.batch >= 1 && a.rows >= 1 && a.n >= 1 && a.k >= 1, "gemm: empty problem (batch %d rows %d n %d k %d)",
               a.batch, a.rows, a.n, a.k);
  UG_CHECK_ARG(a.k % 8 == 0 && a.n % 8 == 0, "gemm: n (%d) and k (%d) must be multiples of 8", a.n, a.k);
  UG_CHECK_ARG(a.a_row_stride % 8 == 0 && a.w_row_stride % 8 == 0 && a.c_row_stride % 8 == 0,
               "gemm: row strides must be multiples of 8 elements (16 bytes)");
  UG_CHECK_ARG(a.a_row_stride >= a.k && a.w_row_stride >= a.k && a.c_row_stride >= a.n, "gemm: row stride smaller than row");
  UG_CHECK_ARG((reinterpret_cast<uintptr_t>(a.c) & 15) == 0, "gemm: C not 16-byte aligned");
  UG_CHECK_ARG(a.batch == 1 || (a.a_batch_stride % 8 == 0 && a.c_batch_stride % 8 == 0), "gemm: batch strides must be multiples of 8");
  if (a.residual) {
    UG_CHECK_ARG(a.res_row_stride % 8 == 0 && (reinterpret_cast<uintptr_t>(a.residual) & 15) == 0, "gemm: residual alignment");
  }
  if (a.bias) UG_CHECK_ARG((reinterpret_cast<uintptr_t>(a.bias) & 15) == 0 && a.bias_batch_stride % 8 == 0, "gemm: bias alignment");
  if (a.gate) UG_CHECK_ARG((reinterpret_cast<uintptr_t>(a.gate) & 15) == 0 && a.gate_batch_stride % 4 == 0, "gemm: gate alignment");
  if (a.gate_seg_stride) {
    UG_CHECK_ARG(a.gate && a.gate_seg_stride % 4 == 0 && a.lora_nseg >= 1 && a.lora_nseg <= UG_MAX_SEGMENTS,
                 "gemm: gate_seg_stride needs a gate and the row-segment table (lora_nseg / lora_seg_bounds)");
  }
  UG_CHECK_ARG(a.act == UG_ACT_NONE || a.act == UG_ACT_GELU_TANH, "gemm: unknown activation %d", a.act);
  if (a.qk_norm_weight) {
    UG_CHECK_ARG(a.qk_head_dim == 64 || a.qk_head_dim == 128, "gemm: fused QK-norm needs head_dim 64 or 128 (got %d)", a.qk_head_dim);
    UG_CHECK_ARG(a.qk_d > 0 && a.qk_d % a.qk_head_dim == 0 && a.n % a.qk_head_dim == 0 && a.n == 3 * a.qk_d,
                 "gemm: fused QK-norm expects n = 3 * qk_d with qk_d a multiple of head_dim (n %d, qk_d %d)", a.n, a.qk_d);
    UG_CHECK_ARG(!a.lora_t && !a.gate && !a.residual && a.act == UG_ACT_NONE && a.alpha == 1.0f,
                 "gemm: the fused QK-norm epilogue composes with bias only");
    UG_CHECK_ARG((reinterpret_cast<uintptr_t>(a.qk_norm_weight) & 15) == 0 &&
                     (!a.qk_cos_sin || (reinterpret_cast<uintptr_t>(a.qk_cos_sin) & 15) == 0), "gemm: QK-norm operand alignment");
  }
  if (a.lora_t) {
    UG_CHECK_ARG(a.lora_b && (a.lora_rank == 4 || a.lora_rank == 8 || a.lora_rank == 12 || a.lora_rank == 16),
                 "gemm: LoRA needs lora_b and a rank in {4, 8, 12, 16} (got %d)", a.lora_rank);
    UG_CHECK_ARG(a.lora_nseg >= 1 && a.lora_nseg <= UG_MAX_SEGMENTS, "gemm: lora_nseg %d out of range", a.lora_nseg);
    UG_CHECK_ARG((a.lora_block_n <= 0 ? a.n : a.lora_block_n) % 32 == 0, "gemm: lora_block_n must be a multiple of 32");
    UG_CHECK_ARG(a.lora_t_row_stride % 4 == 0 && (reinterpret_cast<uintptr_t>(a.lora_t) & 15) == 0 &&
                     (reinterpret_cast<uintptr_t>(a.lora_b) & 7) == 0,
                 "gemm: LoRA operand alignment");
  }
  if (a.colmask_block) {
    UG_CHECK_ARG(a.colmask_block % 32 == 0 && a.lora_nseg >= 1 && a.lora_nseg <= UG_MAX_SEGMENTS && !a.bias && !a.gate && !a.residual &&
                     a.act == UG_ACT_NONE && !a.lora_t,
                 "gemm: colmask_block must be a multiple of 32, needs the row-segment table and composes with no other epilogue op");
  }
  if (a.a2) {
    UG_CHECK_ARG(a.w2 && a.k2 >= 8 && a.k2 % 8 == 0, "gemm: second operand pair needs w2 and k2 (%d) a positive multiple of 8", a.k2);
    UG_CHECK_ARG(a.a2_row_stride % 8 == 0 && a.w2_row_stride % 8 == 0 && a.a2_row_stride >= a.k2 && a.w2_row_stride >= a.k2 &&
                     (a.batch == 1 || a.a2_batch_stride % 8 == 0),
                 "gemm: second operand pair strides must be multiples of 8 elements and cover k2");
  }
  cudaStream_t s = reinterpret_cast<cudaStream_t>(stream);
  int variant = a.variant;
  if (variant == 0) {
    variant = pick_tile_variant(a.batch, a.rows, a.n);
    if (a.n <= 128) variant = 3;
  }
  const bool special = a.lora_t || a.colmask_block;
  if (a.variant == 0 && !special && staged_epilogue_default() && !(a.qk_norm_weight && a.qk_d % 128 != 0)) {
    if (a.qk_norm_weight && variant == 3) {
      const int sms = num_sms();
      const long long t2 = (long long)a.batch * ((a.rows + 255) / 256) * ((a.n + 255) / 256);
      const long long t1 = (long long)a.batch * ((a.rows + 127) / 128) * ((a.n + 255) / 256);
      const double c2 = (double)((t2 + sms / 2 - 1) / (sms / 2)) * 256 * 256 / 2.0, c1 = (double)((t1 + sms - 1) / sms) * 128 * 256 / 0.98;
      variant = c2 <= c1 ? 2 : 1;
    }
    variant = variant == 2 ? 4 : (variant == 1 ? 5 : 6);
  }
  if (variant >= 4 && variant <= 6) {
    UG_CHECK_ARG(!special, "gemm: variants 4-6 (staged epilogue) do not compose with lora_t / colmask_block");
    UG_CHECK_ARG(!a.qk_norm_weight || (variant != 6 && a.qk_d % 128 == 0),
                 "gemm: the staged fused QK-norm epilogue needs a 256-column tile (variants 4 / 5) and qk_d a multiple of 128");
    UG_CHECK_ARG(!a.residual || a.res_batch_stride % 8 == 0 || a.batch == 1, "gemm: residual batch stride must be a multiple of 8");
  }
  switch (variant) {
    case 1: return launch_gemm<1, 256, 4>(a, s);
    case 2: return launch_gemm<2, 256, 6>(a, s);
    case 3: return launch_gemm<1, 128, 6>(a, s);
    case 4: return launch_gemm<2, 256, 5, true>(a, s);
    case 5: return launch_gemm<1, 256, 3, true>(a, s);
    case 6: return launch_gemm<1, 128, 6, true>(a, s);
    default:
      set_error("gemm: unknown variant %d", a.variant);
      return UG_ERR_INVALID;
  }
}

extern "C" int ug_conv3x3_bf16(const ug_conv2d_args* args, void* stream) {
  using namespace ug;
  UG_CHECK_ARG(args != nullptr, "conv3x3: null args");
  const ug_conv2d_args& c = *args;
  UG_CHECK_ARG(c.x && c.w && c.y, "conv3x3: null operand pointer");
  UG_CHECK_ARG(c.batch >= 1 && c.h >= 1 && c.w_px >= 1, "conv3x3: empty image");
  UG_CHECK_ARG(c.c_in >= 64 && c.c_in % 64 == 0, "conv3x3: c_in (%d) must be a multiple of 64 (use ug_im2col_bf16 + ug_gemm_bf16 otherwise)", c.c_in);
  UG_CHECK_ARG(c.c_out >= 8 && c.c_out % 8 == 0 && c.y_pixel_stride >= c.c_out && c.y_pixel_stride % 8 == 0,
               "conv3x3: c_out (%d) and the output pixel stride (%d) must be multiples of 8", c.c_out, (int)c.y_pixel_stride);
  UG_CHECK_ARG(c.w_px % 128 == 0 || (c.w_px <= 128 && 128 % c.w_px == 0),
               "conv3x3: image width %d must be a multiple of 128 or divide 128 (use ug_im2col_bf16 + ug_gemm_bf16 otherwise)", c.w_px);
  UG_CHECK_ARG((reinterpret_cast<uintptr_t>(c.y) & 15) == 0 && (reinterpret_cast<uintptr_t>(c.x) & 15) == 0 &&
                   (reinterpret_cast<uintptr_t>(c.w) & 15) == 0, "conv3x3: operands must be 16-byte aligned");
  if (c.bias) UG_CHECK_ARG((reinterpret_cast<uintptr_t>(c.bias) & 15) == 0, "conv3x3: bias alignment");
  if (c.residual)
    UG_CHECK_ARG((reinterpret_cast<uintptr_t>(c.residual) & 15) == 0 && c.res_pixel_stride >= c.c_out && c.res_pixel_stride % 8 == 0,
                 "conv3x3: residual alignment / pixel stride");
  ug_gemm_args g;
  memset(&g, 0, sizeof(g));
  const int rows = c.h * c.w_px;
  g.a = c.x; g.a_row_stride = c.c_in; g.a_batch_stride = (int64_t)rows * c.c_in;
  g.w = c.w; g.w_row_stride = 9 * c.c_in;
  g.c = c.y; g.c_row_stride = c.y_pixel_stride; g.c_batch_stride = (int64_t)rows * c.y_pixel_stride;
  g.batch = c.batch; g.rows = rows; g.n = c.c_out; g.k = 9 * c.c_in;
  g.bias = c.bias; g.alpha = c.alpha == 0.0f ? 1.0f : c.alpha; g.act = UG_ACT_NONE;
  g.residual = c.residual; g.res_row_stride = c.res_pixel_stride; g.res_batch_stride = (int64_t)rows * c.res_pixel_stride;
  const ConvDesc cd{c.x, c.batch, c.h, c.w_px, c.c_in};
  cudaStream_t s = reinterpret_cast<cudaStream_t>(stream);
  int variant = c.variant;
  if (variant == 0) {
    variant = pick_tile_variant(c.batch, rows, c.c_out);
    variant = variant == 2 ? 4 : (variant == 1 ? 5 : 6);
    if (c.c_out <= 128) {
      const long long pairs = (long long)c.batch * ((rows + 255) / 256);
      variant = pairs >= num_sms() / 2 ? 7 : 6;
    }
  }
  switch (variant) {
    case 1: return launch_gemm<1, 256, 4>(g, s, &cd);
    case 2: return launch_gemm<2, 256, 6>(g, s, &cd);
    case 3: return launch_gemm<1, 128, 6>(g, s, &cd);
    case 4: return launch_gemm<2, 256, 5, true>(g, s, &cd);
    case 5: return launch_gemm<1, 256, 3, true>(g, s, &cd);
    case 6: return launch_gemm<1, 128, 6, true>(g, s, &cd);
    case 7: return launch_gemm<2, 128, 7, true>(g, s, &cd);
    default:
      set_error("conv3x3: unknown variant %d", c.variant);
      return UG_ERR_INVALID;
  }
}
```

### unigen_b200/model.py

```python
from __future__ import annotations

import collections
import math
import types
from typing import Any, Dict, List, Optional, Sequence, Tuple

import torch

from . import ops
from .ops import UG_ACT_GELU_TANH

BF16 = torch.bfloat16


class FluxArch:

    def __init__(self, num_layers=19, num_single_layers=38, attention_head_dim=128, num_attention_heads=24, in_channels=64,
                 joint_attention_dim=4096, pooled_projection_dim=768, guidance_embeds=False, axes_dims_rope=(16, 56, 56),
                 theta=10000.0):
        self.num_layers, self.num_single_layers = num_layers, num_single_layers
        self.attention_head_dim, self.num_attention_heads = attention_head_dim, num_attention_heads
        self.in_channels, self.joint_attention_dim = in_channels, joint_attention_dim
        self.pooled_projection_dim, self.guidance_embeds = pooled_projection_dim, guidance_embeds
        self.axes_dims_rope, self.theta = tuple(axes_dims_rope), theta
        self.hidden_size = num_layers and num_attention_heads * attention_head_dim

    @staticmethod
    def tiny():
        return FluxArch(num_layers=2, num_single_layers=4, attention_head_dim=64, num_attention_heads=6, axes_dims_rope=(8, 28, 28))


class _Weights:

    def __init__(self, device):
        self.device = device
        self.views: Dict[str, torch.Tensor] = {}

    def alloc(self, *shape, dtype=BF16) -> torch.Tensor:
        return torch.zeros(*shape, device=self.device, dtype=dtype)

    def linear(self, name: str, out_f: int, in_f: int, w: Optional[torch.Tensor] = None, b: Optional[torch.Tensor] = None):
        w = self.alloc(out_f, in_f) if w is None else w
        b = self.alloc(out_f) if b is None else b
        self.views[name + ".weight"], self.views[name + ".bias"] = w, b
        return w, b

    def fused(self, names: Sequence[str], out_each: int, in_f: int):
        W, Bv = self.alloc(len(names) * out_each, in_f), self.alloc(len(names) * out_each)
        for i, n in enumerate(names):
            self.views[n + ".weight"] = W[i * out_each:(i + 1) * out_each]
            self.views[n + ".bias"] = Bv[i * out_each:(i + 1) * out_each]
        return W, Bv


class _DoubleBlockW:
    def __init__(self, ws: _Weights, p: str, D: int, dh: int):
        self.norm1 = ws.linear(p + ".norm1.linear", 6 * D, D)
        self.norm1_ctx = ws.linear(p + ".norm1_context.linear", 6 * D, D)
        self.qkv = ws.fused([f"{p}.attn.to_q", f"{p}.attn.to_k", f"{p}.attn.to_v"], D, D)
        self.add_qkv = ws.fused([f"{p}.attn.add_q_proj", f"{p}.attn.add_k_proj", f"{p}.attn.add_v_proj"], D, D)
        self.to_out = ws.linear(p + ".attn.to_out.0", D, D)
        self.to_add_out = ws.linear(p + ".attn.to_add_out", D, D)
        self.rms = ws.alloc(2, dh)
        self.rms_ctx = ws.alloc(2, dh)
        ws.views[p + ".attn.norm_q.weight"], ws.views[p + ".attn.norm_k.weight"] = self.rms[0], self.rms[1]
        ws.views[p + ".attn.norm_added_q.weight"], ws.views[p + ".attn.norm_added_k.weight"] = self.rms_ctx[0], self.rms_ctx[1]
        self.ff1 = ws.linear(p + ".ff.net.0.proj", 4 * D, D)
        self.ff2 = ws.linear(p + ".ff.net.2", D, 4 * D)
        self.ffc1 = ws.linear(p + ".ff_context.net.0.proj", 4 * D, D)
        self.ffc2 = ws.linear(p + ".ff_context.net.2", D, 4 * D)


class _SingleBlockW:
    def __init__(self, ws: _Weights, p: str, D: int, dh: int):
        self.norm = ws.linear(p + ".norm.linear", 3 * D, D)
        self.qkv = ws.fused([f"{p}.attn.to_q", f"{p}.attn.to_k", f"{p}.attn.to_v"], D, D)
        self.mlp = ws.linear(p + ".proj_mlp", 4 * D, D)
        self.out = ws.linear(p + ".proj_out", D, 5 * D)
        self.rms = ws.alloc(2, dh)
        ws.views[p + ".attn.norm_q.weight"], ws.views[p + ".attn.norm_k.weight"] = self.rms[0], self.rms[1]


class _TimeTextW:
    def __init__(self, ws: _Weights, p: str, D: int, pooled: int, guidance: bool):
        self.t1 = ws.linear(p + ".timestep_embedder.linear_1", D, 256)
        self.t2 = ws.linear(p + ".timestep_embedder.linear_2", D, D)
        self.g1 = ws.linear(p + ".guidance_embedder.linear_1", D, 256) if guidance else None
        self.g2 = ws.linear(p + ".guidance_embedder.linear_2", D, D) if guidance else None
        self.p1 = ws.linear(p + ".text_embedder.linear_1", D, pooled)
        self.p2 = ws.linear(p + ".text_embedder.linear_2", D, D)


class _DenoiserBase(torch.nn.Module):

    def _init_base(self, device):
        self.device_ = torch.device(device)
        if self.device_.type != "cuda":
            raise ops.UgError(f"{type(self).__name__} (B200-native) needs a CUDA device: the hot path has no CPU fallback")
        self._ws = _Weights(self.device_)
        self._control_ready = False
        self._workspaces: "collections.OrderedDict[Any, Any]" = collections.OrderedDict()
        self.max_workspaces = 4
        self._buf = None
        self._graphs: Dict[Any, Any] = {}
        self.use_cuda_graph = False
        self.gemm_variant = 0
        self.attn_variant = 0
        self.overlap_mod_gemv = True
        self._side_stream = torch.cuda.Stream(device=self.device_)
        self.overlap_text_stream = True
        self._text_stream = torch.cuda.Stream(device=self.device_)
        self.fuse_qk_norm = True
        self.trace: Optional[Dict[str, torch.Tensor]] = None
        self.clone_outputs = True

    @property
    def dtype(self):
        return BF16

    @property
    def device(self):
        return self.device_

    def state_dict(self, *args, **kwargs):
        return dict(self._ws.views)

    def parameters(self, recurse: bool = True):
        return iter(self._ws.views.values())

    def load_state_dict(self, state_dict, strict: bool = True, assign: bool = False):
        missing = [k for k in self._ws.views if k not in state_dict]
        unexpected = [k for k in state_dict if k not in self._ws.views]
        if strict and (missing or unexpected):
            raise RuntimeError(f"load_state_dict: missing {missing[:5]}... unexpected {unexpected[:5]}...")
        with torch.no_grad():
            for k, v in state_dict.items():
                if k in self._ws.views:
                    dst = self._ws.views[k]
                    if tuple(dst.shape) != tuple(v.shape):
                        raise RuntimeError(f"size mismatch for {k}: {tuple(v.shape)} vs {tuple(dst.shape)}")
                    dst.copy_(v.to(device=dst.device, dtype=dst.dtype))
        self._weights_loaded()
        return types.SimpleNamespace(missing_keys=missing, unexpected_keys=unexpected)

    def _weights_loaded(self):
        """Hook: derived (non-state-dict) device tensors are rebuilt after a load / random init."""

    @torch.no_grad()
    def init_random_(self, seed: int = 0, zero_linear_std: Optional[float] = 0.02):
        gen = torch.Generator(device=self.device_).manual_seed(seed)
        for k, v in self._ws.views.items():
            if k.endswith(".pos_embed"):
                continue
            if k.startswith("controlnet_add_"):
                if zero_linear_std is None:
                    v.zero_()
                else:
                    v.copy_(torch.randn(v.shape, device=v.device, generator=gen) * zero_linear_std)
            elif ".norm_q." in k or ".norm_k." in k or ".norm_added_" in k:
                v.fill_(1.0)
            else:
                w = self._ws.views[k[:-4] + "weight"] if k.endswith(".bias") else v
                bound = 1.0 / math.sqrt(w[0].numel())
                v.copy_((torch.rand(v.shape, device=v.device, generator=gen) * 2 - 1) * bound)
        self._weights_loaded()
        return self

    def _time_text(self, w: "_TimeTextW", t_emb: torch.Tensor, pooled: torch.Tensor, out: torch.Tensor, tmp: torch.Tensor,
                   g_emb: Optional[torch.Tensor] = None, accumulate: bool = False):
        ops.gemv(t_emb, w.t1[0], w.t1[1], out=tmp, silu_out=True)
        ops.gemv(tmp, w.t2[0], w.t2[1], out=out, accumulate=accumulate)
        if g_emb is not None and w.g1 is not None:
            ops.gemv(g_emb, w.g1[0], w.g1[1], out=tmp, silu_out=True)
            ops.gemv(tmp, w.g2[0], w.g2[1], out=out, accumulate=True)
        ops.gemv(pooled, w.p1[0], w.p1[1], out=tmp, silu_out=True)
        ops.gemv(tmp, w.p2[0], w.p2[1], out=out, accumulate=True)
        return out

    def _mods(self, buf, slot: int, n_chunks: int, w, temb: torch.Tensor) -> List[torch.Tensor]:
        D = self.inner_dim
        region = buf.MOD[:, slot * D:(slot + n_chunks) * D]
        ops.gemv(temb, w[0], w[1], out=region, silu_in=True)
        return [region[:, i * D:(i + 1) * D] for i in range(n_chunks)]

    def _rec(self, name: str, t: torch.Tensor):
        if self.trace is not None:
            self.trace[name] = t.detach().float().clone()

    def _cached_workspace(self, key, make):
        ws = self._workspaces
        b = ws.get(key)
        if b is None:
            while len(ws) >= max(int(self.max_workspaces), 1):
                _, old = ws.popitem(last=False)
                self._drop_graphs(old)
            b = ws[key] = make()
        else:
            ws.move_to_end(key)
            self._trim_workspaces()
        self._buf = b
        return b

    def _trim_workspaces(self):
        ws = self._workspaces
        while len(ws) > max(int(self.max_workspaces), 1):
            _, old = ws.popitem(last=False)
            self._drop_graphs(old)

    def _drop_graphs(self, buf=None):
        if buf is None:
            self._graphs.clear()
            return
        for k in [k for k, g in self._graphs.items() if g[4] is buf]:
            del self._graphs[k]

    def _run_staged(self, key, staged: Dict[str, Optional[torch.Tensor]], *args):
        if not self.use_cuda_graph or self.trace is not None:
            return self._forward_impl(*args, **staged)
        g = self._graphs.get(key)
        if g is not None and not any(g[4] is b for b in self._workspaces.values()):
            del self._graphs[key]
            g = None
        if g is None:
            static = {k: (v.clone() if v is not None else None) for k, v in staged.items()}
            self._forward_impl(*args, **static)
            torch.cuda.synchronize()
            graph = torch.cuda.CUDAGraph()
            with torch.cuda.graph(graph):
                out = self._forward_impl(*args, **static)
            g = self._graphs[key] = (graph, static, out, ops.launch_count_in_last_capture(), self._buf)
        graph, static, out, n_launch, buf = g
        ws_key = next(k for k, b in self._workspaces.items() if b is buf)
        self._workspaces.move_to_end(ws_key)
        self._trim_workspaces()
        self._buf = buf
        for k, v in staged.items():
            if v is not None:
                static[k].copy_(v)
        graph.replay()
        ops.add_launches(n_launch)
        return out


class UniGenFlux(_DenoiserBase):

    def __init__(self, arch: Optional[FluxArch] = None, device: Any = "cuda", **config):
        super().__init__()
        self.arch = arch or FluxArch(**config)
        self._init_base(device)
        a = self.arch
        self.config = types.SimpleNamespace(in_channels=a.in_channels, guidance_embeds=a.guidance_embeds,
                                            num_attention_heads=a.num_attention_heads, attention_head_dim=a.attention_head_dim,
                                            pooled_projection_dim=a.pooled_projection_dim, joint_attention_dim=a.joint_attention_dim,
                                            axes_dims_rope=a.axes_dims_rope, num_layers=a.num_layers,
                                            num_single_layers=a.num_single_layers)
        self.inner_dim = a.num_attention_heads * a.attention_head_dim
        D, dh = self.inner_dim, a.attention_head_dim
        ws = self._ws
        self.x_embedder_w = ws.linear("x_embedder", D, a.in_channels)
        self.context_embedder_w = ws.linear("context_embedder", D, a.joint_attention_dim)
        self.time_text = _TimeTextW(ws, "time_text_embed", D, a.pooled_projection_dim, a.guidance_embeds)
        self.double = [_DoubleBlockW(ws, f"transformer_blocks.{i}", D, dh) for i in range(a.num_layers)]
        self.single = [_SingleBlockW(ws, f"single_transformer_blocks.{i}", D, dh) for i in range(a.num_single_layers)]
        self.norm_out_w = ws.linear("norm_out.linear", 2 * D, D)
# ... 96 lines not shown
        self.consis = [_DoubleBlockW(ws, f"consis_module.{s}", D, dh) for s in (0, 1)] if self.use_consis_module else []
        self.trainable_control_modules = {k: None for k in (
            "control_pos_embed_input", "control_time_text_embed", "control_condition_embed", "control_context_embedder",
            "control_x_embedder", "control_joint_trans_blocks", "controlnet_add_joint_blocks", "control_single_trans_blocks",
            "controlnet_add_single_blocks", "moe") + (("shared_expert",) if self.use_shared_expert else ())
            + (("consis_module",) if self.use_consis_module else ())}
        self._control_ready = True
        if get("use_transformer_params", False):
            self.init_control_param()

    @torch.no_grad()
    def init_control_param(self):
        v = self._ws.views

        def copy_prefix(dst: str, src: str):
            for k in [k for k in v if k.startswith(src + ".")]:
                kd = dst + k[len(src):]
                if kd in v and v[kd].shape == v[k].shape:
                    v[kd].copy_(v[k])

        copy_prefix("control_time_text_embed", "time_text_embed")
        copy_prefix("control_condition_embed", "time_text_embed")
        for j in range(self.cn_joint_layers):
            copy_prefix(f"control_joint_trans_blocks.{j}", f"transformer_blocks.{j}")
        for j in range(len(self.ctrl_single)):
            copy_prefix(f"control_single_trans_blocks.{j}", f"single_transformer_blocks.{j}")
        self._weights_loaded()

    def _workspace(self, B: int, N: int, T: int):
        return self._cached_workspace((B, N, T), lambda: self._make_workspace(B, N, T))

    def _make_workspace(self, B: int, N: int, T: int):
        D, dev = self.inner_dim, self.device_
        S = T + N
        Smax = T + 2 * N
        consis = self.use_consis_module and self.use_shared_expert
        if consis:
            Smax = max(Smax, 3 * N)
        E = self.expert_nums
        C = ops.moe_capacity(B * N, E)
        z = lambda *s, dt=BF16: torch.empty(*s, device=dev, dtype=dt)
        n_mod = (6 * 2 * (self.arch.num_layers + self.cn_joint_layers + 1 + self.condition_nums) + 3 * (self.arch.num_single_layers + len(self.ctrl_single)) + 2)
        if consis:
            n_mod += 6 * 2 * (1 + self.condition_nums)
        b = types.SimpleNamespace(
            X=z(B, S, D), NX=z(B, Smax, D), QKV=z(B, Smax, 3 * D), AO=z(B, Smax, D), FF=z(B, Smax, 4 * D),
            CAT=z(B, S, 5 * D), CH=z(B, N, D), CS=z(B, S, D), CENC=z(B, T, D), COND=z(B, N, D), HC=z(B, 2 * N, D),
            G=z(B * N, D), A=z(E * C, D), YC=z(E * C, D), YH=z(E * C, D), EH=z(B * N, D), EC=z(B * N, D), CIN=z(B, N, D),
            MOD=z(B, n_mod * D, dt=torch.float32), n_mod=n_mod, tmp=z(B, D, dt=torch.float32),
            TEMBS=z(3 + self.condition_nums, B, D, dt=torch.float32), STEMBS=z(3 + self.condition_nums, B, D, dt=torch.float32),
            MODC=z(B, E, D, dt=torch.float32), MODH=z(B, E, D, dt=torch.float32),
            rope=z(S, self.arch.attention_head_dim, dt=torch.float32),
            rope0=z(2 * N, self.arch.attention_head_dim, dt=torch.float32),
            rope1=z(Smax, self.arch.attention_head_dim, dt=torch.float32),
            NO=z(B, N, D), OUT=z(B, N, self.arch.in_channels), capacity=C)
        b.temb, b.ctemb, b.cdtemb = b.TEMBS[0], b.TEMBS[1], b.TEMBS[2]
        b.cdtemb_c = [b.TEMBS[3 + c] for c in range(self.condition_nums)]
        b.mod_plans = None
        if consis:
            b.CONS = z(B, 2 * N, D)
            b.ropek0 = z(2 * N, self.arch.attention_head_dim, dt=torch.float32)
            b.ropek1 = z(3 * N, self.arch.attention_head_dim, dt=torch.float32)
        return b

    def _conditioning_vectors(self, buf, B, timestep, guidance, pooled, cond_pooled):
        n_cond = self.condition_nums
        t_emb = ops.timestep_embedding(timestep, scale=1000.0, batch=B)
        g_emb = ops.timestep_embedding(guidance, scale=1000.0, batch=B) if guidance is not None else None
        self._time_text(self.time_text, t_emb, pooled, buf.temb, buf.tmp, g_emb)
        ctrl_pooled = pooled if self.use_pooled_prompt_embeds else torch.zeros_like(pooled)
        self._time_text(self.control_time_text, t_emb, ctrl_pooled, buf.ctemb, buf.tmp, g_emb)
        for c in range(n_cond):
            self._time_text(self.control_condition, t_emb, cond_pooled[c], buf.cdtemb_c[c], buf.tmp, g_emb)
            self._time_text(self.control_condition, t_emb, cond_pooled[c], buf.cdtemb, buf.tmp, g_emb, accumulate=c > 0)
        ops.silu(buf.TEMBS, buf.STEMBS)

    def _mod_plans(self, buf, pool=None):
        key = (buf.MOD.data_ptr(), id(pool))
        mp = buf.mod_plans
        if mp is not None and mp.key == key:
            return mp
        D, n_cond = self.inner_dim, self.condition_nums
        s_temb, s_ctemb, s_cdtemb = buf.STEMBS[0], buf.STEMBS[1], buf.STEMBS[2]
        slot = [0]
        early, late = [], []

        def job(w, x, n_chunks, dst):
            s0 = slot[0]
            slot[0] += n_chunks
            region = buf.MOD[:, s0 * D:(s0 + n_chunks) * D]
            dst.append((w[0], w[1], x, region, False))
            return [region[:, i * D:(i + 1) * D] for i in range(n_chunks)]

        mp = types.SimpleNamespace(key=key)
        mp.m_double = [(job(w.norm1, s_temb, 6, early if i == 0 else late), job(w.norm1_ctx, s_temb, 6, early if i == 0 else late))
                       for i, w in enumerate(self.double)]
        mp.m_cdouble = [(job(w.norm1, s_cdtemb, 6, early if j == 0 else late), job(w.norm1_ctx, s_cdtemb, 6, early if j == 0 else late))
                        for j, w in enumerate(self.ctrl_double)]
        mp.m_single = [job(w.norm, s_temb, 3, late) for w in self.single]
        mp.m_csingle = [job(w.norm, s_cdtemb, 3, late) for w in self.ctrl_single]
        mp.mods_s0, mp.mods_s1 = [None] * n_cond, None
        if self.use_shared_expert:
            mp.mods_s0 = [(job(self.shared[0].norm1, buf.STEMBS[3 + c], 6, early), job(self.shared[0].norm1_ctx, buf.STEMBS[3 + c], 6, early))
                          for c in range(n_cond)]
            mp.mods_s1 = (job(self.shared[1].norm1, s_ctemb, 6, early), job(self.shared[1].norm1_ctx, s_ctemb, 6, early))
        mp.mods_k0, mp.mods_k1 = [None] * n_cond, None
        if self.use_consis_module and self.use_shared_expert:
            k0 = self.consis[0]
            mp.mods_k0 = [(job(k0.norm1, buf.STEMBS[3 + c], 6, early), job(k0.norm1_ctx, buf.STEMBS[3 + c], 6, early))
                          for c in range(n_cond)]
            mp.mods_k1 = (job(k0.norm1, s_ctemb, 6, early), job(k0.norm1_ctx, s_ctemb, 6, early))
        mp.m_out = job(self.norm_out_w, s_temb, 2, late)
        assert slot[0] <= buf.n_mod, (slot[0], buf.n_mod)
        dev = self.device_
        if pool is None:
            mp.early, mp.late, mp.all = ops.GemvPlan(early, dev), ops.GemvPlan(late, dev), None
        else:
            mp.early = mp.late = None
            mp.all = ops.GemvPlan(early + late, dev, pool=pool)
        buf.mod_plans = mp
        return mp

    def _rope(self, out: torch.Tensor, *id_tables: torch.Tensor):
        a, r0 = self.arch, 0
        for ids in id_tables:
            ops.rope_table(ids, a.axes_dims_rope, a.theta, out=out[r0:r0 + ids.shape[0]])
            r0 += ids.shape[0]
        return out

    def _attend(self, buf, S: int, out: torch.Tensor):
        a, D = self.arch, self.inner_dim
        ops.attention(buf.QKV[:, :S, 0:D], buf.QKV[:, :S, D:2 * D], buf.QKV[:, :S, 2 * D:3 * D], out, a.num_attention_heads,
                      a.attention_head_dim, variant=self.attn_variant)
        return out

    def _qk_norm(self, rms_w: torch.Tensor, rope_rows: Optional[torch.Tensor]):
        if not self.fuse_qk_norm:
            return None
        return dict(weight=rms_w, head_dim=self.arch.attention_head_dim, d=self.inner_dim, cos_sin=rope_rows, eps=1e-6)

    def _joint_attention(self, buf, B, n_ctx, n_smp, rms_ctx, rms_smp, rope):
        a = self.arch
        H, dh, D = a.num_attention_heads, a.attention_head_dim, self.inner_dim
        S = n_ctx + n_smp
        if not self.fuse_qk_norm:
            qk = buf.QKV[:, :S, :2 * D]
            if n_ctx:
                ops.qk_rmsnorm_rope(qk[:, :n_ctx], 2 * H, dh, rms_ctx, rope[:n_ctx] if rope is not None else None, heads_per_weight=H)
            if n_smp:
                ops.qk_rmsnorm_rope(qk[:, n_ctx:], 2 * H, dh, rms_smp, rope[n_ctx:S] if rope is not None else None, heads_per_weight=H)
        return self._attend(buf, S, buf.AO[:, :S])

    def _double_block(self, buf, w: _DoubleBlockW, mod_smp, mod_ctx, smp_in, ctx_in, smp_out, ctx_out, rope):
        D = self.inner_dim
        B, n_smp, n_ctx = smp_in.shape[0], smp_in.shape[1], ctx_in.shape[1]
        S = n_ctx + n_smp
        gv = self.gemm_variant
        sh_a, sc_a, g_a, sh_m, sc_m, g_m = mod_smp
        csh_a, csc_a, cg_a, csh_m, csc_m, cg_m = mod_ctx
        nx_c, nx_s = buf.NX[:, :n_ctx], buf.NX[:, n_ctx:S]
        main = torch.cuda.current_stream()
        side = self._text_stream if (self.overlap_text_stream and ctx_out is not None and n_ctx and n_smp
                                     and not getattr(self, "_sp_active", False)) else None
        if n_ctx:
            if side is not None:
                side.wait_stream(main)
            with torch.cuda.stream(side if side is not None else main):
                ops.ln_modulate(ctx_in, nx_c, csh_a, csc_a)
                ops.gemm(nx_c, w.add_qkv[0], out=buf.QKV[:, :n_ctx], bias=w.add_qkv[1], variant=gv,
                         qk_norm=self._qk_norm(w.rms_ctx, rope[:n_ctx] if rope is not None else None))
        if n_smp:
            ops.ln_modulate(smp_in, nx_s, sh_a, sc_a)
            ops.gemm(nx_s, w.qkv[0], out=buf.QKV[:, n_ctx:S], bias=w.qkv[1], variant=gv,
                     qk_norm=self._qk_norm(w.rms, rope[n_ctx:S] if rope is not None else None))
        if side is not None:
            main.wait_stream(side)
        ao = self._joint_attention(buf, B, n_ctx, n_smp, w.rms_ctx, w.rms, rope)
        if ctx_out is not None and n_ctx:
            if side is not None:
                side.wait_stream(main)
            with torch.cuda.stream(side if side is not None else main):
                ops.gemm(ao[:, :n_ctx], w.to_add_out[0], out=ctx_out, bias=w.to_add_out[1], gate=cg_a, residual=ctx_in, variant=gv)
                ops.ln_modulate(ctx_out, nx_c, csh_m, csc_m)
                ops.gemm(nx_c, w.ffc1[0], out=buf.FF[:, :n_ctx], bias=w.ffc1[1], act=UG_ACT_GELU_TANH, variant=gv)
                ops.gemm(buf.FF[:, :n_ctx], w.ffc2[0], out=ctx_out, bias=w.ffc2[1], gate=cg_m, residual=ctx_out, variant=gv)
        if n_smp:
            ops.gemm(ao[:, n_ctx:S], w.to_out[0], out=smp_out, bias=w.to_out[1], gate=g_a, residual=smp_in, variant=gv)
            ops.ln_modulate(smp_out, nx_s, sh_m, sc_m)
            ops.gemm(nx_s, w.ff1[0], out=buf.FF[:, n_ctx:S], bias=w.ff1[1], act=UG_ACT_GELU_TANH, variant=gv)
            ops.gemm(buf.FF[:, n_ctx:S], w.ff2[0], out=smp_out, bias=w.ff2[1], gate=g_m, residual=smp_out, variant=gv)
        if side is not None:
            main.wait_stream(side)

    def _single_attention(self, buf, S: int, rms: torch.Tensor, rope, out: torch.Tensor):
        a, D = self.arch, self.inner_dim
        H, dh = a.num_attention_heads, a.attention_head_dim
        if not self.fuse_qk_norm:
            ops.qk_rmsnorm_rope(buf.QKV[:, :S, :2 * D], 2 * H, dh, rms, rope[:S] if rope is not None else None, heads_per_weight=H)
        return self._attend(buf, S, out)

    def _single_block(self, buf, w: _SingleBlockW, mod, x_in, x_out, rope):
        a = self.arch
        H, dh, D = a.num_attention_heads, a.attention_head_dim, self.inner_dim
        B, S = x_in.shape[0], x_in.shape[1]
        gv = self.gemm_variant
        shift, scale, gate = mod
        nx, cat = buf.NX[:, :S], buf.CAT[:, :S]
        ops.ln_modulate(x_in, nx, shift, scale)
        ops.gemm(nx, w.qkv[0], out=buf.QKV[:, :S], bias=w.qkv[1], variant=gv,
                 qk_norm=self._qk_norm(w.rms, rope[:S] if rope is not None else None))
        ops.gemm(nx, w.mlp[0], out=cat[:, :, D:], bias=w.mlp[1], act=UG_ACT_GELU_TANH, variant=gv)
        self._single_attention(buf, S, w.rms, rope, cat[:, :, :D])
        ops.gemm(cat, w.out[0], out=x_out, bias=w.out[1], gate=gate, residual=x_in, variant=gv)

    def _prestage(self, buf, B, N, T, h_img, cond_tokens, pooled, cond_pooled, rts_uniform, mods_s0, mods_s1, cond_index,
                  txt_ids, img_ids, cond_ids, mods_k0=None, mods_k1=None):
        a = self.arch
        D, E, C = self.inner_dim, self.expert_nums, buf.capacity
        gv = self.gemm_variant
        ops.gemm(cond_tokens, self.control_x_embedder_w[0], out=buf.COND, bias=self.control_x_embedder_w[1], variant=gv)
        self._rope(buf.rope0, cond_ids, img_ids)
        self._rope(buf.rope1, txt_ids, img_ids, cond_ids)
        g = buf.G.view(B, N, D)
        ops.add(h_img, buf.COND, g)
        tag = "moe" if cond_index == 0 and self.condition_nums == 1 else f"moe.cond{cond_index}"
        self._rec(tag + ".cond_embed", buf.COND); self._rec(tag + ".gate_input", g)
        route = ops.moe_route(buf.G, self.gate_wg, rts_uniform, C)
        if self.trace is not None:
            for k in ("expert_idx", "slot", "prob", "slot_token", "exp_counts"):
                self.trace[f"{tag}.route.{k}"] = route[k].detach().clone()
        ops.gemv(cond_pooled, self.exp_mod_w[0], self.exp_mod_b[0], out=buf.MODC.view(B, E * D))
        ops.gemv(pooled, self.exp_mod_w[1], self.exp_mod_b[1], out=buf.MODH.view(B, E * D))
        ops.moe_gather_modulate(buf.COND.view(B * N, D), route["slot_token"], buf.MODC, E, C, N, out=buf.A)
        ops.gemm(buf.A.view(E, C, D), self.exp_w[0], out=buf.YC.view(E, C, D), bias=self.exp_b[0], variant=gv)
        hid_flat = buf.EH
        ops.copy(h_img, hid_flat.view(B, N, D))
        ops.moe_gather_modulate(hid_flat, route["slot_token"], buf.MODH, E, C, N, addend=buf.YC, out=buf.A)
        ops.gemm(buf.A.view(E, C, D), self.exp_w[1], out=buf.YH.view(E, C, D), bias=self.exp_b[1], variant=gv)
        hc_h, hc_c = buf.HC[:, :N], buf.HC[:, N:]
        if self.use_shared_expert:
            self._double_block(buf, self.shared[0], mods_s0[0], mods_s0[1], h_img, buf.COND, hc_h, hc_c, buf.rope0)
            self._double_block(buf, self.shared[1], mods_s1[0], mods_s1[1], buf.HC, buf.CENC, buf.HC, None, buf.rope1)
        ops.moe_combine(buf.YH, route, C, buf.EH)
        ops.moe_combine(buf.YC, route, C, buf.EC)
        self._rec(tag + ".expert_hidden", buf.EH.view(B, N, D)); self._rec(tag + ".expert_cond", buf.EC.view(B, N, D))
        if self.use_consis_module and self.use_shared_expert:
            eh, ec = buf.EH.view(B, N, D), buf.EC.view(B, N, D)
            self._rope(buf.ropek0, cond_ids, cond_ids)
            self._rope(buf.ropek1, img_ids, img_ids, cond_ids)
            ops.copy(eh, buf.CONS[:, :N])
            self._double_block(buf, self.consis[0], mods_k0[0], mods_k0[1], ec, buf.COND, buf.CONS[:, N:], None, buf.ropek0)
            self._double_block(buf, self.consis[0], mods_k1[0], mods_k1[1], buf.CONS, h_img, buf.CONS, None, buf.ropek1)
            self._rec(tag + ".consis_hidden", buf.CONS[:, :N]); self._rec(tag + ".consis_cond", buf.CONS[:, N:])
            ops.add(eh, buf.CONS[:, :N], eh)
            ops.add(ec, buf.CONS[:, N:], ec)
        if not self.use_shared_expert:
            if cond_index == 0:
                ops.add(buf.EH.view(B, N, D), buf.EC.view(B, N, D), buf.CIN)
            else:
                ops.add(buf.CIN, buf.EH.view(B, N, D), buf.CIN)
                ops.add(buf.CIN, buf.EC.view(B, N, D), buf.CIN)
            return route
        self._rec(tag + ".shared_hidden", hc_h); self._rec(tag + ".shared_cond", hc_c)
        if cond_index == 0:
            ops.add(hc_h, buf.EH.view(B, N, D), buf.CIN)
        else:
            ops.add(buf.CIN, hc_h, buf.CIN)
            ops.add(buf.CIN, buf.EH.view(B, N, D), buf.CIN)
        ops.add(buf.CIN, hc_c, buf.CIN)
        ops.add(buf.CIN, buf.EC.view(B, N, D), buf.CIN)
        return route

    @torch.no_grad()
    def forward(self, hidden_states, condition_hidden_states=None, conditioning_scale: float = 1.0,
                encoder_hidden_states=None, pooled_projections=None, condition_pooled_projections=None, timestep=None,
                img_ids=None, txt_ids=None, guidance=None, condition_ids=None, joint_attention_kwargs=None,
                skip_layers=None, rts_uniform=None, **kwargs):
        if not self._control_ready:
            raise ops.UgError("call init_condition_block(condition_nums=..., control_params=...) before forward")
        if encoder_hidden_states is None or condition_hidden_states is None or timestep is None:
            raise ops.UgError("forward needs hidden_states, condition_hidden_states, encoder_hidden_states and timestep")
        B, N, _ = hidden_states.shape
        T = encoder_hidden_states.shape[1]
        multi = isinstance(condition_hidden_states, (list, tuple))
        cond_list = list(condition_hidden_states) if multi else [condition_hidden_states]
        cpool_list = list(condition_pooled_projections) if multi else [condition_pooled_projections]
        cid_list = list(condition_ids) if multi else [condition_ids]
        if len(cond_list) != self.condition_nums or len(cpool_list) != len(cond_list) or len(cid_list) != len(cond_list):
            raise ops.UgError(f"expected {self.condition_nums} condition(s) (init_condition_block), got {len(cond_list)}")
        if any(c.shape[-2] != N for c in cond_list):
            raise ops.UgError("condition tokens must match the image token count (Nc == N) for the CoMoE pre-stage")
        if T == N:
            raise ops.UgError("T == N: the reference MOELayer would also dispatch the text tensor (SURVEY.md §8 A9); unsupported")
        dev = self.device_
        f32 = lambda t: t.to(device=dev, dtype=torch.float32).contiguous()
        sq = lambda t: t[0] if t.dim() == 3 else t
        if rts_uniform is None:
            u_list = [torch.rand(B * N, self.expert_nums, device=dev, dtype=torch.float32) for _ in cond_list]
        else:
            u_list = list(rts_uniform) if isinstance(rts_uniform, (list, tuple)) else [rts_uniform]
        staged = dict(
            hs=hidden_states.to(dev), es=encoder_hidden_states.to(dev), pooled=f32(pooled_projections),
            timestep=f32(timestep), guidance=f32(guidance) if guidance is not None else None,
            txt_ids=f32(sq(txt_ids)), img_ids=f32(sq(img_ids)))
        for c in range(len(cond_list)):
            x = cond_list[c].to(dev)
            staged[f"cs{c}"] = x if x.dim() == 3 else x.unsqueeze(0)
            cp = f32(cpool_list[c])
            staged[f"cp{c}"] = cp if cp.dim() == 2 else cp.unsqueeze(0)
            staged[f"cid{c}"] = f32(sq(cid_list[c]))
            staged[f"u{c}"] = f32(u_list[c])
        key = (B, N, T, float(conditioning_scale), guidance is not None,
               tuple((k, v.dtype) for k, v in staged.items() if v is not None))
        out, add_losses, add_outputs = self._run_staged(key, staged, float(conditioning_scale))
        if self.clone_outputs:
            out = ops.copy(out, torch.empty(out.shape, device=out.device, dtype=out.dtype))
            add_losses = {k: v.clone() for k, v in add_losses.items()}
            add_outputs = {k: v.clone() for k, v in add_outputs.items()}
        return out, add_losses, add_outputs

    def _forward_impl(self, conditioning_scale, hs, es, pooled, timestep, guidance, txt_ids, img_ids, **cond):
        a = self.arch
        n_cond = self.condition_nums
        cs = [cond[f"cs{c}"] for c in range(n_cond)]
        cond_pooled = [cond[f"cp{c}"] for c in range(n_cond)]
        condition_ids = [cond[f"cid{c}"] for c in range(n_cond)]
        rts_uniform = [cond[f"u{c}"] for c in range(n_cond)]
        D, H, dh = self.inner_dim, a.num_attention_heads, a.attention_head_dim
        B, N, _ = hs.shape
        T = es.shape[1]
        S = T + N
        buf = self._workspace(B, N, T)
        n0 = ops.launch_count()
        hs, es = ops.to_bf16(hs.contiguous()), ops.to_bf16(es.contiguous())
        cs = [ops.to_bf16(c.contiguous()) for c in cs]
        gv = self.gemm_variant

        x_txt, x_img = buf.X[:, :T], buf.X[:, T:]
        ops.gemm(hs, self.x_embedder_w[0], out=x_img, bias=self.x_embedder_w[1], variant=gv)
        ops.gemm(es, self.context_embedder_w[0], out=x_txt, bias=self.context_embedder_w[1], variant=gv)
        self._conditioning_vectors(buf, B, timestep, guidance, pooled, cond_pooled)
        self._rope(buf.rope, txt_ids, img_ids)
        self._rec("temb", buf.temb); self._rec("x_embed", x_img); self._rec("context_embed", x_txt)
        self._rec("control_temb", buf.ctemb); self._rec("condition_temb", buf.cdtemb)
        for c in range(n_cond):
# ... 78 lines not shown
```

### unigen_b200/ops.py

```python
from __future__ import annotations

import ctypes as C
import math
from typing import Optional, Sequence

import torch

from . import _lib
from ._lib import UG_ACT_GELU_TANH, UG_ACT_NONE, AttnArgs, GemmArgs, QkvScatterArgs, UgError, check

__all__ = ["gemm", "lora_down", "lora_down_wide", "attention", "attention_peer", "qkv_scatter", "peer_bcast_rows", "peer_barrier", "expand_segment_mask", "ln_modulate", "qk_rmsnorm_rope", "rope_table", "gemv", "GemvPlan", "gemv_grouped", "silu",
           "timestep_embedding", "add", "copy", "to_bf16", "to_f32", "moe_route", "moe_gather_modulate",
           "moe_combine", "ln_modulate_segs", "ln_modulate_slots", "gated_add_slots", "unpatchify", "euler_step", "euler_step_table", "cfg_combine", "pack_latents", "unpack_latents", "conv3x3", "conv3x3_implicit_ok", "im2col", "groupnorm", "upsample2x", "softmax_rows_", "nhwc_to_nchw", "vae_sample", "launch_count", "reset_launch_count", "UG_ACT_NONE", "UG_ACT_GELU_TANH", "UgError"]

BF16 = torch.bfloat16


def _stream() -> C.c_void_p:
    return C.c_void_p(torch.cuda.current_stream().cuda_stream)


def _dev(t: torch.Tensor, name: str, dtype=None) -> torch.Tensor:
    if not t.is_cuda:
        raise UgError(f"{name}: expected a CUDA tensor — the UniGen hot path has no CPU fallback")
    if dtype is not None and t.dtype != dtype:
        raise UgError(f"{name}: expected dtype {dtype}, got {t.dtype}")
    return t


def _view3(t: torch.Tensor, name: str) -> torch.Tensor:
    if t.dim() == 2:
        t = t.unsqueeze(0)
    if t.dim() != 3 or t.stride(2) != 1:
        raise UgError(f"{name}: expected a [batch, rows, cols] view with contiguous cols, got shape {tuple(t.shape)} "
                      f"strides {t.stride()}")
    return t


def launch_count() -> int:
    return int(_lib.load().ug_launch_count()) + _extra_launches


def reset_launch_count() -> None:
    global _extra_launches
    _extra_launches = 0
    _lib.load().ug_reset_launch_count()


_extra_launches = 0
_last_forward_launches = 0


def note_capture_launches(n: int) -> None:
    global _last_forward_launches
    _last_forward_launches = int(n)


def launch_count_in_last_capture() -> int:
    return _last_forward_launches


def add_launches(n: int) -> None:
    global _extra_launches
    _extra_launches += int(n)


def device_check() -> None:
    check(_lib.load().ug_device_check(), "ug_device_check")


def gemm(a: torch.Tensor, w: torch.Tensor, out: Optional[torch.Tensor] = None, bias: Optional[torch.Tensor] = None,
         gate: Optional[torch.Tensor] = None, alpha: float = 1.0, act: int = UG_ACT_NONE,
         residual: Optional[torch.Tensor] = None, variant: int = 0, lora: Optional[dict] = None,
         qk_norm: Optional[dict] = None, gate_seg_stride: int = 0, seg_bounds: Optional[Sequence[int]] = None,
         a2: Optional[torch.Tensor] = None, w2: Optional[torch.Tensor] = None, colmask: Optional[dict] = None) -> torch.Tensor:
    a = _view3(_dev(a, "gemm.a", BF16), "gemm.a")
    _dev(w, "gemm.w", BF16)
    B, R, K = a.shape
    N = w.shape[-2]
    if w.shape[-1] != K:
        raise UgError(f"gemm: K mismatch a {tuple(a.shape)} w {tuple(w.shape)}")
    if out is None:
        out = torch.empty(B, R, N, device=a.device, dtype=BF16)
    o3 = _view3(_dev(out, "gemm.out", BF16), "gemm.out")
    g = GemmArgs()
    g.a, g.a_row_stride, g.a_batch_stride = a.data_ptr(), a.stride(1), a.stride(0)
    g.w, g.w_row_stride = w.data_ptr(), w.stride(-2)
    g.w_batch_stride = w.stride(0) if w.dim() == 3 else 0
    g.c, g.c_row_stride, g.c_batch_stride = o3.data_ptr(), o3.stride(1), o3.stride(0)
    g.batch, g.rows, g.n, g.k = B, R, N, K
    if bias is not None:
        _dev(bias, "gemm.bias", BF16)
        g.bias = bias.data_ptr()
        g.bias_batch_stride = bias.stride(0) if bias.dim() == 2 else 0
    if gate is not None:
        _dev(gate, "gemm.gate", torch.float32)
        if gate.dim() == 1:
            gate = gate.unsqueeze(0)
        g.gate, g.gate_batch_stride = gate.data_ptr(), gate.stride(0)
    g.alpha, g.act = float(alpha), int(act)
    if gate_seg_stride:
        g.gate_seg_stride = int(gate_seg_stride)
        sb = seg_bounds if seg_bounds is not None else (lora["seg_bounds"] if lora is not None else None)
        if gate is None or sb is None:
            raise UgError("gemm: gate_seg_stride needs gate and seg_bounds (or a lora segment table)")
        g.lora_nseg = len(sb) - 1
        for i, v in enumerate(sb):
            g.lora_seg_bounds[i] = int(v)
    if residual is not None:
        r3 = _view3(_dev(residual, "gemm.residual", BF16), "gemm.residual")
        g.residual, g.res_row_stride, g.res_batch_stride = r3.data_ptr(), r3.stride(1), r3.stride(0)
    g.variant = variant
    if lora is not None:
        t, lb = lora["t"], lora["b"]
        _dev(t, "gemm.lora_t", torch.float32), _dev(lb, "gemm.lora_b", BF16)
        t3 = t if t.dim() == 3 else t.unsqueeze(0)
        if not lb.is_contiguous() or t3.stride(2) != 1:
            raise UgError("gemm: lora_b must be contiguous [groups, N, rank]; lora_t needs a unit inner stride")
        g.lora_t, g.lora_t_row_stride, g.lora_t_batch_stride = t3.data_ptr(), t3.stride(1), t3.stride(0)
        g.lora_b, g.lora_rank, g.lora_block_n = lb.data_ptr(), int(lora["rank"]), int(lora.get("block_n", 0))
        sb, sg = lora["seg_bounds"], lora["seg_group"]
        g.lora_nseg = len(sg)
        for i, v in enumerate(sb):
            g.lora_seg_bounds[i] = int(v)
        for i, v in enumerate(sg):
            g.lora_seg_group[i] = int(v)
    if colmask is not None:
        g.colmask_block = int(colmask["block"])
        sb, sg = colmask["seg_bounds"], colmask["seg_group"]
        g.lora_nseg = len(sg)
        for i, v in enumerate(sb):
            g.lora_seg_bounds[i] = int(v)
        for i, v in enumerate(sg):
            g.lora_seg_group[i] = int(v)
    if a2 is not None:
        a23 = _view3(_dev(a2, "gemm.a2", BF16), "gemm.a2")
        _dev(w2, "gemm.w2", BF16)
        if a23.shape[:2] != (B, R) or w2.dim() != 2 or w2.shape[0] != N or w2.shape[1] != a23.shape[2] or w2.stride(1) != 1:
            raise UgError(f"gemm: a2 {tuple(a23.shape)} / w2 {tuple(w2.shape)} do not match a {tuple(a.shape)} / n {N}")
        g.a2, g.a2_row_stride, g.a2_batch_stride = a23.data_ptr(), a23.stride(1), a23.stride(0)
        g.w2, g.w2_row_stride, g.k2 = w2.data_ptr(), w2.stride(0), a23.shape[2]
    if qk_norm is not None:
        wq = _dev(qk_norm["weight"], "gemm.qk_norm.weight", BF16)
        g.qk_norm_weight, g.qk_head_dim, g.qk_d = wq.data_ptr(), int(qk_norm["head_dim"]), int(qk_norm["d"])
        g.qk_eps = float(qk_norm.get("eps", 1e-6))
        cs = qk_norm.get("cos_sin")
        if cs is not None:
            _dev(cs, "gemm.qk_norm.cos_sin", torch.float32)
            if cs.shape[0] < R or not cs.is_contiguous():
                raise UgError("gemm: qk_norm cos_sin table too short / not contiguous")
            g.qk_cos_sin = cs.data_ptr()
    check(_lib.load().ug_gemm_bf16(C.byref(g), _stream()), "ug_gemm_bf16")
    return out


def lora_down(x: torch.Tensor, a_stack: torch.Tensor, seg_bounds: Sequence[int], seg_group: Sequence[int],
              out: Optional[torch.Tensor] = None) -> torch.Tensor:
    x3 = _view3(_dev(x, "lora_down.x", BF16), "lora_down.x")
    _dev(a_stack, "lora_down.a", BF16)
    B, R, K = x3.shape
    G, RT, K2 = a_stack.shape
    if K2 != K or not a_stack.is_contiguous():
        raise UgError("lora_down: a_stack must be contiguous [groups, rank_total, K]")
    if out is None:
        out = torch.empty(B, R, RT, device=x.device, dtype=torch.float32)
    n = len(seg_group)
    sb = (C.c_int32 * (n + 1))(*[int(v) for v in seg_bounds])
    sg = (C.c_int32 * n)(*[int(v) for v in seg_group])
    check(_lib.load().ug_lora_down(x3.data_ptr(), x3.stride(1), x3.stride(0), a_stack.data_ptr(), out.data_ptr(),
                                   out.stride(1), out.stride(0), B, R, K, RT, n, sb, sg, _stream()), "ug_lora_down")
    return out


def _attn_args(q, k, v, heads, head_dim, seg_bounds, seg_visible, scale, variant):
    q, k, v = (_view3(_dev(t, n, BF16), n) for t, n in ((q, "attn.q"), (k, "attn.k"), (v, "attn.v")))
    B, S, HD = q.shape
    if HD != heads * head_dim:
        raise UgError(f"attention: inner dim {HD} != heads {heads} x head_dim {head_dim}")
    a = AttnArgs()
    a.q, a.k, a.v = q.data_ptr(), k.data_ptr(), v.data_ptr()
    a.q_row_stride, a.q_batch_stride = q.stride(1), q.stride(0)
    a.k_row_stride, a.k_batch_stride = k.stride(1), k.stride(0)
    a.v_row_stride, a.v_batch_stride = v.stride(1), v.stride(0)
    a.batch, a.heads, a.seq, a.head_dim = B, heads, S, head_dim
    a.scale = float(scale if scale is not None else 1.0 / math.sqrt(head_dim))
    keep = None
    if seg_bounds is not None:
        n = len(seg_bounds) - 1
        sb = (C.c_int32 * (n + 1))(*seg_bounds)
        sv = (C.c_uint32 * n)(*seg_visible)
        keep = (sb, sv)
        a.n_seg, a.seg_bounds, a.seg_visible = n, sb, sv
    a.variant = variant
    return a, keep


def lora_down_wide(x: torch.Tensor, a_stack: torch.Tensor, seg_bounds: Sequence[int], seg_group: Sequence[int],
                   out: torch.Tensor, block: int = 64) -> torch.Tensor:
    x3 = _view3(_dev(x, "lora_down_wide.x", BF16), "lora_down_wide.x")
    o3 = _view3(_dev(out, "lora_down_wide.out", BF16), "lora_down_wide.out")
    _dev(a_stack, "lora_down_wide.a", BF16)
    B, R, K = x3.shape
    G, RT, K2 = a_stack.shape
    if K2 != K or not a_stack.is_contiguous() or o3.shape[2] != G * block or o3.shape[1] != R:
        raise UgError("lora_down_wide: a_stack must be contiguous [groups, rank_total, K] and out [B, rows, groups*block]")
    n = len(seg_group)
    sb = (C.c_int32 * (n + 1))(*[int(v) for v in seg_bounds])
    sg = (C.c_int32 * n)(*[int(v) for v in seg_group])
    check(_lib.load().ug_lora_down_wide(x3.data_ptr(), x3.stride(1), x3.stride(0), a_stack.data_ptr(), o3.data_ptr(), o3.stride(1),
                                        o3.stride(0), B, R, K, RT, G, block, n, sb, sg, _stream()), "ug_lora_down_wide")
    return out


def attention(q: torch.Tensor, k: torch.Tensor, v: torch.Tensor, out: torch.Tensor, heads: int, head_dim: int,
              seg_bounds: Optional[Sequence[int]] = None, seg_visible: Optional[Sequence[int]] = None,
              scale: Optional[float] = None, variant: int = 0) -> torch.Tensor:
    a, keep = _attn_args(q, k, v, heads, head_dim, seg_bounds, seg_visible, scale, variant)
    o = _view3(_dev(out, "attn.out", BF16), "attn.out")
    a.o, a.o_row_stride, a.o_batch_stride = o.data_ptr(), o.stride(1), o.stride(0)
    check(_lib.load().ug_attention_bf16(C.byref(a), _stream()), "ug_attention_bf16")
    del keep
    return out


def attention_peer(table, q: torch.Tensor, k: torch.Tensor, v: torch.Tensor, heads: int, head_dim: int, o_offset: int,
                   o_row_stride: int, rows_per_rank: int, seg_bounds: Optional[Sequence[int]] = None,
                   seg_visible: Optional[Sequence[int]] = None, scale: Optional[float] = None, variant: int = 0) -> None:
    a, keep = _attn_args(q, k, v, heads, head_dim, seg_bounds, seg_visible, scale, variant)
    a.o, a.o_row_stride, a.o_batch_stride = 0, int(o_row_stride), 0
    check(_lib.load().ug_attention_bf16_peer(C.byref(a), C.byref(table), int(o_offset), int(rows_per_rank), _stream()),
          "ug_attention_bf16_peer")
    del keep


def qkv_scatter(table, qkv_rows: torch.Tensor, heads: int, head_dim: int, norm_weight: Optional[torch.Tensor],
                cos_sin: Optional[torch.Tensor], dst_offset: int, seq_total: int, dst_row0: int, eps: float = 1e-6) -> None:
    _dev(qkv_rows, "qkv_scatter.qkv", BF16)
    if qkv_rows.dim() != 2 or qkv_rows.stride(1) != 1 or qkv_rows.shape[1] != 3 * heads * head_dim:
        raise UgError(f"qkv_scatter: expected a [rows, {3 * heads * head_dim}] view, got {tuple(qkv_rows.shape)}")
    a = QkvScatterArgs()
    a.qkv, a.row_stride, a.rows, a.heads, a.head_dim, a.eps = qkv_rows.data_ptr(), qkv_rows.stride(0), qkv_rows.shape[0], heads, head_dim, eps
    if norm_weight is not None:
        a.norm_weight = _dev(norm_weight, "qkv_scatter.norm_weight", BF16).data_ptr()
    if cos_sin is not None:
        _dev(cos_sin, "qkv_scatter.cos_sin", torch.float32)
        if cos_sin.shape[0] < qkv_rows.shape[0] or not cos_sin.is_contiguous():
            raise UgError("qkv_scatter: cos_sin table too short / not contiguous")
        a.cos_sin = cos_sin.data_ptr()
    a.dst_offset, a.seq_total, a.dst_row0 = int(dst_offset), int(seq_total), int(dst_row0)
    check(_lib.load().ug_qkv_scatter(C.byref(table), C.byref(a), _stream()), "ug_qkv_scatter")


def peer_bcast_rows(table, src: torch.Tensor, dst_offset: int, dst_row_stride: int, dst_row0: int) -> None:
    _dev(src, "peer_bcast.src", BF16)
    if src.dim() != 2 or src.stride(1) != 1:
        raise UgError("peer_bcast_rows: expected a [rows, d] view with contiguous columns")
    check(_lib.load().ug_peer_bcast_rows(C.byref(table), src.data_ptr(), src.stride(0), src.shape[0], src.shape[1], int(dst_offset),
                                         int(dst_row_stride), int(dst_row0), _stream()), "ug_peer_bcast_rows")


def peer_barrier(table) -> None:
    check(_lib.load().ug_peer_barrier(C.byref(table), _stream()), "ug_peer_barrier")


def expand_segment_mask(seq: int, seg_bounds: Sequence[int], seg_visible: Sequence[int], device) -> torch.Tensor:
    n = len(seg_visible)
    m = torch.empty(seq, seq, dtype=torch.uint8, device=device)
    sb = (C.c_int32 * (n + 1))(*seg_bounds)
    sv = (C.c_uint32 * n)(*seg_visible)
    check(_lib.load().ug_expand_segment_mask(seq, n, sb, sv, m.data_ptr(), _stream()), "ug_expand_segment_mask")
    return m.bool()


def ln_modulate(x: torch.Tensor, out: torch.Tensor, shift: torch.Tensor, scale: torch.Tensor, eps: float = 1e-6) -> torch.Tensor:
    x3, o3 = _view3(_dev(x, "ln.x", BF16), "ln.x"), _view3(_dev(out, "ln.out", BF16), "ln.out")
    _dev(shift, "ln.shift", torch.float32), _dev(scale, "ln.scale", torch.float32)
    B, R, D = x3.shape
    if shift.stride(0) != scale.stride(0) and B > 1:
        raise UgError("ln_modulate: shift and scale need the same batch stride")
    check(_lib.load().ug_ln_modulate(x3.data_ptr(), x3.stride(1), x3.stride(0), o3.data_ptr(), o3.stride(1), o3.stride(0),
                                     shift.data_ptr(), scale.data_ptr(), shift.stride(0), B, R, D, float(eps), _stream()),
          "ug_ln_modulate")
    return out


def ln_modulate_segs(x: torch.Tensor, out: torch.Tensor, shift: torch.Tensor, scale: torch.Tensor, seg_bounds: Sequence[int],
                     mod_seg_stride: int, eps: float = 1e-6) -> torch.Tensor:
    x3, o3 = _view3(_dev(x, "ln.x", BF16), "ln.x"), _view3(_dev(out, "ln.out", BF16), "ln.out")
    _dev(shift, "ln.shift", torch.float32), _dev(scale, "ln.scale", torch.float32)
    B, R, D = x3.shape
    n = len(seg_bounds) - 1
    sb = (C.c_int32 * (n + 1))(*[int(v) for v in seg_bounds])
    check(_lib.load().ug_ln_modulate_segs(x3.data_ptr(), x3.stride(1), x3.stride(0), o3.data_ptr(), o3.stride(1), o3.stride(0),
                                          shift.data_ptr(), scale.data_ptr(), shift.stride(0), int(mod_seg_stride), n, sb, B, R, D,
                                          float(eps), _stream()), "ug_ln_modulate_segs")
    return out


def _slot_mod(t: torch.Tensor, name: str):
    _dev(t, name, torch.float32)
    if t.dim() != 3 or t.stride(2) != 1:
        raise UgError(f"{name}: expected an fp32 [experts, index, d] view with contiguous d")
    return t.data_ptr(), t.stride(0), t.stride(1)


def ln_modulate_slots(x: torch.Tensor, out: torch.Tensor, shift: torch.Tensor, scale: torch.Tensor, slot_token: torch.Tensor,
# ... 426 lines not shown
```

Measured before the change: 7.403.

## Fuse text and image double-block GEMMs into one two-segment launch

Adds a second row segment to the GEMM kernel, with its own weight TMA map, bias, gate, residual, output and QK-norm operands. The double block can then run the context and sample projections (qkv, out-proj, ff1, ff2) as one launch over the concatenated rows. This replaces the separate text stream and its fork/join events. The aim is fewer launches and better SM fill on the small text GEMM. The cost is extra per-tile selection logic and extra tensor-map parameters in the kernel, and it only works when segment boundaries line up with row tiles.

Result: faster. 7.514 (median of 6 runs) (+1.5%).

```diff
diff --git a/include/unigen_b200.h b/include/unigen_b200.h
--- a/include/unigen_b200.h
+++ b/include/unigen_b200.h
@@ -8,7 +8,7 @@
 extern "C" {
 #endif
 
-#define UG_ABI_VERSION 9
+#define UG_ABI_VERSION 10
 
 typedef enum {
   UG_OK = 0,
@@ -78,6 +78,19 @@
   int64_t w2_row_stride;
   int32_t k2;
   int32_t colmask_block;
+  int32_t seg1_row0;
+  const void* seg1_w;
+  int64_t seg1_w_row_stride;
+  const void* seg1_bias;
+  const float* seg1_gate;
+  void* seg1_c;
+  int64_t seg1_c_row_stride;
+  int64_t seg1_c_batch_stride;
+  const void* seg1_residual;
+  int64_t seg1_res_row_stride;
+  int64_t seg1_res_batch_stride;
+  const void* seg1_qk_norm_weight;
+  const float* seg1_qk_cos_sin;
 } ug_gemm_args;
 
 int ug_gemm_bf16(const ug_gemm_args* args, void* stream);
diff --git a/unigen_b200/_lib.py b/unigen_b200/_lib.py
--- a/unigen_b200/_lib.py
+++ b/unigen_b200/_lib.py
@@ -10,7 +10,7 @@
 UG_ACT_GELU_TANH = 1
 UG_MAX_SEGMENTS = 8
 UG_GROUPNORM_MAX_CHUNKS = 1024
-UG_ABI_VERSION = 9
+UG_ABI_VERSION = 10
 
 
 class UgError(RuntimeError):
@@ -35,6 +35,10 @@
         ("qk_eps", C.c_float), ("reserved2", C.c_int32), ("gate_seg_stride", C.c_int64),
         ("a2", C.c_void_p), ("a2_row_stride", C.c_int64), ("a2_batch_stride", C.c_int64),
         ("w2", C.c_void_p), ("w2_row_stride", C.c_int64), ("k2", C.c_int32), ("colmask_block", C.c_int32),
+        ("seg1_row0", C.c_int32), ("seg1_w", C.c_void_p), ("seg1_w_row_stride", C.c_int64), ("seg1_bias", C.c_void_p),
+        ("seg1_gate", C.c_void_p), ("seg1_c", C.c_void_p), ("seg1_c_row_stride", C.c_int64), ("seg1_c_batch_stride", C.c_int64),
+        ("seg1_residual", C.c_void_p), ("seg1_res_row_stride", C.c_int64), ("seg1_res_batch_stride", C.c_int64),
+        ("seg1_qk_norm_weight", C.c_void_p), ("seg1_qk_cos_sin", C.c_void_p),
     ]
 
 
diff --git a/unigen_b200/csrc/ug_flux.cu b/unigen_b200/csrc/ug_flux.cu
--- a/unigen_b200/csrc/ug_flux.cu
+++ b/unigen_b200/csrc/ug_flux.cu
@@ -48,8 +48,8 @@
   std::vector<Lin> add_dbl, add_sgl;
   const float* gate_wg = nullptr;
   const void *exp_w[2] = {nullptr, nullptr}, *exp_b[2] = {nullptr, nullptr}, *exp_mod_w[2] = {nullptr, nullptr}, *exp_mod_b[2] = {nullptr, nullptr};
-  cudaStream_t side = nullptr, text = nullptr;
-  cudaEvent_t ev_fork = nullptr, ev_mod = nullptr, ev_t0 = nullptr, ev_t1 = nullptr;
+  cudaStream_t side = nullptr;
+  cudaEvent_t ev_fork = nullptr, ev_mod = nullptr;
   void* plan_ws = nullptr;
   int plan_B = 0, plan_N = 0, plan_T = 0;
   int early_jobs = 0, early_groups = 0, late_jobs = 0, late_groups = 0;
@@ -77,8 +77,7 @@
   h->d = *desc;
   h->D = desc->heads * desc->head_dim;
   cudaError_t e = cudaStreamCreateWithFlags(&h->side, cudaStreamNonBlocking);
-  if (e == cudaSuccess) e = cudaStreamCreateWithFlags(&h->text, cudaStreamNonBlocking);
-  for (cudaEvent_t* ev : {&h->ev_fork, &h->ev_mod, &h->ev_t0, &h->ev_t1})
+  for (cudaEvent_t* ev : {&h->ev_fork, &h->ev_mod})
     if (e == cudaSuccess) e = cudaEventCreateWithFlags(ev, cudaEventDisableTiming);
   if (e != cudaSuccess) {
     set_error("flux_create: %s", cudaGetErrorString(e));
@@ -92,8 +91,7 @@
 extern "C" void ug_flux_destroy(ug_flux* h) {
   if (!h) return;
   if (h->side) cudaStreamDestroy(h->side);
-  if (h->text) cudaStreamDestroy(h->text);
-  for (cudaEvent_t ev : {h->ev_fork, h->ev_mod, h->ev_t0, h->ev_t1})
+  for (cudaEvent_t ev : {h->ev_fork, h->ev_mod})
     if (ev) cudaEventDestroy(ev);
   delete h;
 }
@@ -314,6 +312,29 @@
     }
     return ug_gemm_bf16(&g, s);
   }
+  int gemm_rows(View a, int k, int n, Lin w, View c, const float* gate, const View* res, Lin w1, View c1, const float* gate1,
+                const View* res1, int act = UG_ACT_NONE, const void* qk_rms = nullptr, const void* qk_rms1 = nullptr,
+                const float* qk_cos_sin = nullptr) const {
+    ug_gemm_args g;
+    memset(&g, 0, sizeof(g));
+    g.a = a.p; g.a_row_stride = a.rs; g.a_batch_stride = a.bs;
+    g.w = w.w; g.w_row_stride = k;
+    g.c = c.p; g.c_row_stride = c.rs; g.c_batch_stride = c.bs;
+    g.batch = B; g.rows = a.rows; g.n = n; g.k = k;
+    g.bias = w.b;
+    g.gate = gate; g.gate_batch_stride = gate ? mod_bs() : 0;
+    g.alpha = 1.0f; g.act = act;
+    if (res) { g.residual = res->p; g.res_row_stride = res->rs; g.res_batch_stride = res->bs; }
+    g.seg1_row0 = c.rows;
+    g.seg1_w = w1.w; g.seg1_w_row_stride = k; g.seg1_bias = w1.b; g.seg1_gate = gate1;
+    g.seg1_c = c1.p; g.seg1_c_row_stride = c1.rs; g.seg1_c_batch_stride = c1.bs;
+    if (res1) { g.seg1_residual = res1->p; g.seg1_res_row_stride = res1->rs; g.seg1_res_batch_stride = res1->bs; }
+    if (qk_rms) {
+      g.qk_norm_weight = qk_rms; g.qk_cos_sin = qk_cos_sin; g.qk_head_dim = dh; g.qk_d = D; g.qk_eps = 1e-6f;
+      g.seg1_qk_norm_weight = qk_rms1; g.seg1_qk_cos_sin = qk_cos_sin + (size_t)c.rows * dh;
+    }
+    return ug_gemm_bf16(&g, main);
+  }
   int ln(cudaStream_t s, View x, View o, const float* shift, const float* scale) const {
     return ug_ln_modulate(x.p, x.rs, x.bs, o.p, o.rs, o.bs, shift, scale, mod_bs(), B, x.rows, D, 1e-6f, s);
   }
@@ -358,34 +379,28 @@
     View nx_c = view(L.NX, 0, n_ctx, D, Smax), nx_s = view(L.NX, n_ctx, n_smp, D, Smax);
     View qkv_c = view(L.QKV, 0, n_ctx, 3 * D, Smax), qkv_s = view(L.QKV, n_ctx, n_smp, 3 * D, Smax);
     View ff_c = view(L.FF, 0, n_ctx, 4 * D, Smax), ff_s = view(L.FF, n_ctx, n_smp, 4 * D, Smax);
-    View ao_c = view(L.AO, 0, n_ctx, D, Smax), ao_s = view(L.AO, n_ctx, n_smp, D, Smax), ao = view(L.AO, 0, Sq, D, Smax);
+    View ao_s = view(L.AO, n_ctx, n_smp, D, Smax), ao = view(L.AO, 0, Sq, D, Smax);
     const float *sh_a = mod(slot_smp), *sc_a = mod(slot_smp + 1), *g_a = mod(slot_smp + 2), *sh_m = mod(slot_smp + 3), *sc_m = mod(slot_smp + 4),
                 *g_m = mod(slot_smp + 5);
     const float *csh_a = mod(slot_ctx), *csc_a = mod(slot_ctx + 1), *cg_a = mod(slot_ctx + 2), *csh_m = mod(slot_ctx + 3),
                 *csc_m = mod(slot_ctx + 4), *cg_m = mod(slot_ctx + 5);
-    const bool fork = ctx_out != nullptr;
-    cudaStream_t ts = fork ? h->text : main;
-    if (fork) { cudaEventRecord(h->ev_t0, main); cudaStreamWaitEvent(ts, h->ev_t0, 0); }
     const float* rp = f32(rope_off);
-    UG_TRY(ln(ts, ctx_in, nx_c, csh_a, csc_a));
-    UG_TRY(gemm(ts, nx_c, D, w.add_qkv, 3 * D, qkv_c, nullptr, nullptr, UG_ACT_NONE, 1.0f, -1, 0, 0, w.rms_ctx, rp));
+    View nx = view(L.NX, 0, Sq, D, Smax), ff = view(L.FF, 0, Sq, 4 * D, Smax);
+    UG_TRY(ln(main, ctx_in, nx_c, csh_a, csc_a));
     UG_TRY(ln(main, smp_in, nx_s, sh_a, sc_a));
-    UG_TRY(gemm(main, nx_s, D, w.qkv, 3 * D, qkv_s, nullptr, nullptr, UG_ACT_NONE, 1.0f, -1, 0, 0, w.rms, rp + (size_t)n_ctx * dh));
-    if (fork) { cudaEventRecord(h->ev_t1, ts); cudaStreamWaitEvent(main, h->ev_t1, 0); }
+    UG_TRY(gemm_rows(nx, D, 3 * D, w.add_qkv, qkv_c, nullptr, nullptr, w.qkv, qkv_s, nullptr, nullptr, UG_ACT_NONE, w.rms_ctx, w.rms, rp));
     UG_TRY(attention(Sq, ao));
-    if (fork) {
-      cudaEventRecord(h->ev_t0, main); cudaStreamWaitEvent(ts, h->ev_t0, 0);
-      UG_TRY(gemm(ts, ao_c, D, w.to_add_out, D, *ctx_out, cg_a, &ctx_in));
-      UG_TRY(ln(ts, *ctx_out, nx_c, csh_m, csc_m));
-      UG_TRY(gemm(ts, nx_c, D, w.ffc1, 4 * D, ff_c, nullptr, nullptr, UG_ACT_GELU_TANH));
-      UG_TRY(gemm(ts, ff_c, 4 * D, w.ffc2, D, *ctx_out, cg_m, ctx_out));
-    }
-    UG_TRY(gemm(main, ao_s, D, w.to_out, D, smp_out, g_a, &smp_in));
+    if (!ctx_out) {
+      UG_TRY(gemm(main, ao_s, D, w.to_out, D, smp_out, g_a, &smp_in));
+      UG_TRY(ln(main, smp_out, nx_s, sh_m, sc_m));
+      UG_TRY(gemm(main, nx_s, D, w.ff1, 4 * D, ff_s, nullptr, nullptr, UG_ACT_GELU_TANH));
+      return gemm(main, ff_s, 4 * D, w.ff2, D, smp_out, g_m, &smp_out);
+    }
+    UG_TRY(gemm_rows(ao, D, D, w.to_add_out, *ctx_out, cg_a, &ctx_in, w.to_out, smp_out, g_a, &smp_in));
+    UG_TRY(ln(main, *ctx_out, nx_c, csh_m, csc_m));
     UG_TRY(ln(main, smp_out, nx_s, sh_m, sc_m));
-    UG_TRY(gemm(main, nx_s, D, w.ff1, 4 * D, ff_s, nullptr, nullptr, UG_ACT_GELU_TANH));
-    UG_TRY(gemm(main, ff_s, 4 * D, w.ff2, D, smp_out, g_m, &smp_out));
-    if (fork) { cudaEventRecord(h->ev_t1, ts); cudaStreamWaitEvent(main, h->ev_t1, 0); }
-    return UG_OK;
+    UG_TRY(gemm_rows(nx, D, 4 * D, w.ffc1, ff_c, nullptr, nullptr, w.ff1, ff_s, nullptr, nullptr, UG_ACT_GELU_TANH));
+    return gemm_rows(ff, 4 * D, D, w.ffc2, *ctx_out, cg_m, ctx_out, w.ff2, smp_out, g_m, &smp_out);
   }
 
   int single_block(const SingleW& w, int slot, View x_in, View x_out) const {
diff --git a/unigen_b200/csrc/ug_gemm.cu b/unigen_b200/csrc/ug_gemm.cu
--- a/unigen_b200/csrc/ug_gemm.cu
+++ b/unigen_b200/csrc/ug_gemm.cu
@@ -38,7 +38,25 @@
   int qk_dh, qk_d;
   float qk_eps;
   int conv_cblocks, conv_w;
+  int seg1_row0;
+  const __nv_bfloat16* bias1;
+  const float* gate1;
+  const __nv_bfloat16* qk_w1;
+  const float* qk_cos_sin1;
 };
+
+struct SegOperands {
+  const __nv_bfloat16* bias;
+  const float* gate;
+  const __nv_bfloat16* qk_w;
+  const float* qk_cos_sin;
+  int row0, rows;
+};
+
+__device__ __forceinline__ SegOperands seg_operands(const GemmParams& p, bool seg1) {
+  if (seg1) return SegOperands{p.bias1, p.gate1, p.qk_w1, p.qk_cos_sin1, p.seg1_row0, p.rows - p.seg1_row0};
+  return SegOperands{p.bias, p.gate, p.qk_w, p.qk_cos_sin, 0, p.seg1_row0 ? p.seg1_row0 : p.rows};
+}
 
 struct ConvDesc {
   const void* x;
@@ -159,13 +177,13 @@
   }
 }
 
-__device__ __forceinline__ uint4 epilogue_group8(const GemmParams& p, const uint32_t* v8, int b, int c, const float* gate_row,
-                                                 const uint4& rv) {
+__device__ __forceinline__ uint4 epilogue_group8(const GemmParams& p, const SegOperands& so, const uint32_t* v8, int b, int c,
+                                                 const float* gate_row, const uint4& rv) {
   float x[8];
 #pragma unroll
   for (int i = 0; i < 8; ++i) x[i] = __uint_as_float(v8[i]);
-  if (p.bias) {
-    const uint4 bv = *reinterpret_cast<const uint4*>(p.bias + (long long)b * p.bias_bs + c);
+  if (so.bias) {
+    const uint4 bv = *reinterpret_cast<const uint4*>(so.bias + (long long)b * p.bias_bs + c);
     const float2 f0 = unpack_bf16x2(bv.x), f1 = unpack_bf16x2(bv.y), f2 = unpack_bf16x2(bv.z), f3 = unpack_bf16x2(bv.w);
     x[0] += f0.x; x[1] += f0.y; x[2] += f1.x; x[3] += f1.y;
     x[4] += f2.x; x[5] += f2.y; x[6] += f3.x; x[7] += f3.y;
@@ -196,23 +214,24 @@
   return o;
 }
 
-__device__ __forceinline__ uint4 epilogue_qk_group8(const GemmParams& p, const uint32_t* v8, int b, int r, int c, int which, float rstd) {
+__device__ __forceinline__ uint4 epilogue_qk_group8(const GemmParams& p, const SegOperands& so, const uint32_t* v8, int b, int r, int c,
+                                                    int which, float rstd) {
   const int c_in_head = c % p.qk_dh;
   float x[8];
 #pragma unroll
   for (int i = 0; i < 8; ++i) x[i] = __uint_as_float(v8[i]);
-  if (p.bias) {
-    const uint4 bv = *reinterpret_cast<const uint4*>(p.bias + (long long)b * p.bias_bs + c);
+  if (so.bias) {
+    const uint4 bv = *reinterpret_cast<const uint4*>(so.bias + (long long)b * p.bias_bs + c);
     const float2 f0 = unpack_bf16x2(bv.x), f1 = unpack_bf16x2(bv.y), f2 = unpack_bf16x2(bv.z), f3 = unpack_bf16x2(bv.w);
     x[0] += f0.x; x[1] += f0.y; x[2] += f1.x; x[3] += f1.y;
     x[4] += f2.x; x[5] += f2.y; x[6] += f3.x; x[7] += f3.y;
   }
-  const uint4 wv = *reinterpret_cast<const uint4*>(p.qk_w + which * p.qk_dh + c_in_head);
+  const uint4 wv = *reinterpret_cast<const uint4*>(so.qk_w + which * p.qk_dh + c_in_head);
   const float2 w0 = unpack_bf16x2(wv.x), w1 = unpack_bf16x2(wv.y), w2 = unpack_bf16x2(wv.z), w3 = unpack_bf16x2(wv.w);
   x[0] *= rstd * w0.x; x[1] *= rstd * w0.y; x[2] *= rstd * w1.x; x[3] *= rstd * w1.y;
   x[4] *= rstd * w2.x; x[5] *= rstd * w2.y; x[6] *= rstd * w3.x; x[7] *= rstd * w3.y;
-  if (p.qk_cos_sin) {
-    const float* cs = p.qk_cos_sin + (long long)min(r, p.rows - 1) * p.qk_dh + c_in_head;
+  if (so.qk_cos_sin) {
+    const float* cs = so.qk_cos_sin + (long long)min(r, so.rows - 1) * p.qk_dh + c_in_head;
     const float4 t0 = __ldg(reinterpret_cast<const float4*>(cs)), t1 = __ldg(reinterpret_cast<const float4*>(cs + 4));
     const float co[4] = {t0.x, t0.z, t1.x, t1.z}, si[4] = {t0.y, t0.w, t1.y, t1.w};
 #pragma unroll
@@ -272,15 +291,15 @@
   }
 }
 
-__device__ __forceinline__ float chunk_sumsq(const GemmParams& p, const uint32_t (&v)[32], int b, int col0) {
+__device__ __forceinline__ float chunk_sumsq(const GemmParams& p, const __nv_bfloat16* bias, const uint32_t (&v)[32], int b, int col0) {
   float ss = 0.f;
 #pragma unroll
   for (int j = 0; j < 4; ++j) {
     float x[8];
 #pragma unroll
     for (int i = 0; i < 8; ++i) x[i] = __uint_as_float(v[8 * j + i]);
-    if (p.bias) {
-      uint4 bv = *reinterpret_cast<const uint4*>(p.bias + (long long)b * p.bias_bs + col0 + 8 * j);
+    if (bias) {
+      uint4 bv = *reinterpret_cast<const uint4*>(bias + (long long)b * p.bias_bs + col0 + 8 * j);
       float2 f0 = unpack_bf16x2(bv.x), f1 = unpack_bf16x2(bv.y), f2 = unpack_bf16x2(bv.z), f3 = unpack_bf16x2(bv.w);
       x[0] += f0.x; x[1] += f0.y; x[2] += f1.x; x[3] += f1.y;
       x[4] += f2.x; x[5] += f2.y; x[6] += f3.x; x[7] += f3.y;
@@ -304,7 +323,9 @@
 __global__ void __launch_bounds__(kGemmThreads, 1)
 gemm_bf16_kernel(const __grid_constant__ CUtensorMap tma_a, const __grid_constant__ CUtensorMap tma_w,
                  const __grid_constant__ CUtensorMap tma_a2, const __grid_constant__ CUtensorMap tma_w2,
-                 const __grid_constant__ CUtensorMap tma_c, const __grid_constant__ CUtensorMap tma_r, const GemmParams p) {
+                 const __grid_constant__ CUtensorMap tma_c, const __grid_constant__ CUtensorMap tma_r,
+                 const __grid_constant__ CUtensorMap tma_w1, const __grid_constant__ CUtensorMap tma_c1,
+                 const __grid_constant__ CUtensorMap tma_r1, const GemmParams p) {
   using Cfg = GemmCfg<kCta, BN, kStages, kTmaEpi>;
   extern __shared__ uint8_t smem_raw[];
   uint8_t* smem = smem_raw + ((1024u - (smem_u32(smem_raw) & 1023u)) & 1023u);
@@ -341,6 +362,11 @@
     if constexpr (kTmaEpi) {
       tma_prefetch_desc(&tma_c);
       if (p.res) tma_prefetch_desc(&tma_r);
+      if (p.seg1_row0) {
+        tma_prefetch_desc(&tma_w1);
+        tma_prefetch_desc(&tma_c1);
+        if (p.res) tma_prefetch_desc(&tma_r1);
+      }
     }
     fence_mbar_init();
   }
@@ -364,6 +390,7 @@
       const int row0 = mt * (Cfg::BM * kCta) + (int)cta_rank * Cfg::BM;
       const int wrow0 = nt * BN + (int)cta_rank * Cfg::BN_LOAD;
       const int wb = p.w_batched ? b : 0;
+      const CUtensorMap* mw1 = (kTmaEpi && p.seg1_row0 && mt * (Cfg::BM * kCta) >= p.seg1_row0) ? &tma_w1 : &tma_w;
       int conv_y0 = 0, conv_x0 = 0, conv_tap = 0, conv_cb = 0;
       if (p.conv_cblocks) {
         conv_y0 = row0 / p.conv_w;
@@ -388,7 +415,7 @@
           } else {
             const bool second = kb >= p.k1_blocks;
             const CUtensorMap* ma = second ? &tma_a2 : &tma_a;
-            const CUtensorMap* mw = second ? &tma_w2 : &tma_w;
+            const CUtensorMap* mw = second ? &tma_w2 : mw1;
             const int kc = (second ? kb - p.k1_blocks : kb) * Cfg::BK;
             if constexpr (kCta == 1) {
               mbar_arrive_expect_tx(&full[stage], Cfg::STAGE_BYTES);
@@ -462,8 +489,10 @@
       }
       const uint32_t taddr = tmem_base + ((uint32_t)(q * 32) << 16) + as * BN;
       const int lora_g = (p.lora_t || p.colmask_block) ? lora_group_of(p, r) : -1;
-      const float* gate_row = p.gate ? p.gate + (long long)b * p.gate_bs + (p.gate_seg_stride ? seg_index_of(p, r) * p.gate_seg_stride : 0)
-                                     : nullptr;
+      const bool seg1 = kTmaEpi && p.seg1_row0 && mt * (Cfg::BM * kCta) >= p.seg1_row0;
+      const SegOperands so = seg_operands(p, seg1);
+      const float* gate_row = so.gate ? so.gate + (long long)b * p.gate_bs + (p.gate_seg_stride ? seg_index_of(p, r) * p.gate_seg_stride : 0)
+                                      : nullptr;
       auto release_acc = [&]() {
         tc_fence_before();
         __syncwarp();
@@ -476,7 +505,9 @@
         const int ew = warp - 2;
         uint8_t* slab0 = smem_epi + ew * Cfg::EPI_WARP_BYTES;
         uint64_t* rbar = res_bars + ew * Cfg::EPI_SLABS;
-        const int r0 = mt * (Cfg::BM * kCta) + (int)cta_rank * Cfg::BM + q * 32;
+        const int r0 = mt * (Cfg::BM * kCta) + (int)cta_rank * Cfg::BM + q * 32 - so.row0;
+        const CUtensorMap* map_c = seg1 ? &tma_c1 : &tma_c;
+        const CUtensorMap* map_r = seg1 ? &tma_r1 : &tma_r;
         const int cw0 = n0 + col_half * (BN / (kEpiWarps / 4));
         if (lane == 0) bulk_wait_group_read<0>();
         __syncwarp();
@@ -485,7 +516,7 @@
           for (int sl = 0; sl < Cfg::EPI_SLABS; ++sl) {
             if (cw0 + 64 * sl < p.n) {
               mbar_arrive_expect_tx(&rbar[sl], Cfg::EPI_SLAB_BYTES);
-              tma_load_3d(slab0 + sl * Cfg::EPI_SLAB_BYTES, &tma_r, &rbar[sl], cw0 + 64 * sl, r0, b);
+              tma_load_3d(slab0 + sl * Cfg::EPI_SLAB_BYTES, map_r, &rbar[sl], cw0 + 64 * sl, r0, b);
             }
           }
         }
@@ -496,7 +527,7 @@
         int qk_which = 2;
         float qk_rstd[2] = {1.f, 1.f};
         if constexpr (BN == 256) {
-          if (p.qk_w && cw0 < p.n) qk_which = cw0 / p.qk_d;
+          if (so.qk_w && cw0 < p.n) qk_which = cw0 / p.qk_d;
           if (qk_which < 2) {
             float ss[2] = {0.f, 0.f};
 #pragma unroll
@@ -504,7 +535,7 @@
               uint32_t v[32];
               tmem_ld_32x32(taddr + (ch0 + ch) * 32, v);
               tmem_ld_wait();
-              if (cw0 + 32 * ch < p.n) ss[(p.qk_dh == 64) ? (ch >> 1) : 0] += chunk_sumsq(p, v, b, cw0 + 32 * ch);
+              if (cw0 + 32 * ch < p.n) ss[(p.qk_dh == 64) ? (ch >> 1) : 0] += chunk_sumsq(p, so.bias, v, b, cw0 + 32 * ch);
             }
             if (p.qk_dh != 64) ss[1] = ss[0];
             qk_rstd[0] = rsqrtf(ss[0] / (float)p.qk_dh + p.qk_eps);
@@ -532,8 +563,9 @@
                 const int c = cs0 + 32 * h + 8 * j;
                 uint4* cell = reinterpret_cast<uint4*>(slab + lane * 128 + (((4 * h + j) ^ (lane & 7)) << 4));
                 if (c < p.n) {
-                  if (qk_which < 2) *cell = epilogue_qk_group8(p, &v[8 * j], b, r, c, qk_which, sl == 0 ? qk_rstd[0] : qk_rstd[1]);
-                  else *cell = epilogue_group8(p, &v[8 * j], b, c, gate_row, p.res ? *cell : make_uint4(0, 0, 0, 0));
+                  if (qk_which < 2)
+                    *cell = epilogue_qk_group8(p, so, &v[8 * j], b, r - so.row0, c, qk_which, sl == 0 ? qk_rstd[0] : qk_rstd[1]);
+                  else *cell = epilogue_group8(p, so, &v[8 * j], b, c, gate_row, p.res ? *cell : make_uint4(0, 0, 0, 0));
                 }
               }
             }
@@ -542,7 +574,7 @@
             fence_proxy_async_smem();
             __syncwarp();
             if (lane == 0) {
-              tma_store_3d(&tma_c, slab, cs0, r0, b);
+              tma_store_3d(map_c, slab, cs0, r0, b);
               bulk_commit_group();
             }
           }
@@ -567,7 +599,7 @@
               uint32_t v[32];
               tmem_ld_32x32(taddr + c_h + ch * 32, v);
               tmem_ld_wait();
-              ss += chunk_sumsq(p, v, b, col_h + ch * 32);
+              ss += chunk_sumsq(p, p.bias, v, b, col_h + ch * 32);
             }
             rstd = rsqrtf(ss / (float)p.qk_dh + p.qk_eps);
           }
@@ -663,21 +695,29 @@
     k2_blocks = (a.k2 + Cfg::BK - 1) / Cfg::BK;
   }
   CUtensorMap tma_c = tma_a, tma_r = tma_a;
+  CUtensorMap tma_w1 = tma_w, tma_c1 = tma_a, tma_r1 = tma_a;
   if constexpr (kTmaEpi) {
-    uint32_t box[3] = {64, 32, 1};
-    {
-      uint64_t dims[3] = {(uint64_t)a.n, (uint64_t)a.rows, (uint64_t)a.batch};
-      uint64_t bs = a.batch > 1 ? (uint64_t)a.c_batch_stride : (uint64_t)a.rows * a.c_row_stride;
-      uint64_t strides[2] = {(uint64_t)a.c_row_stride * 2, bs * 2};
-      int st = encode_tmap_bf16(&tma_c, a.c, 3, dims, strides, box);
-      if (st != UG_OK) return st;
-    }
+    auto rows_map = [&](CUtensorMap* m, const void* ptr, int rows, int64_t rs, int64_t bstride) {
+      uint32_t box[3] = {64, 32, 1};
+      uint64_t dims[3] = {(uint64_t)a.n, (uint64_t)rows, (uint64_t)a.batch};
+      uint64_t bs = a.batch > 1 ? (uint64_t)bstride : (uint64_t)rows * rs;
+      uint64_t strides[2] = {(uint64_t)rs * 2, bs * 2};
+      return encode_tmap_bf16(m, ptr, 3, dims, strides, box);
+    };
+    const int rows0 = a.seg1_row0 ? a.seg1_row0 : a.rows, rows1 = a.rows - a.seg1_row0;
+    if (int st = rows_map(&tma_c, a.c, rows0, a.c_row_stride, a.c_batch_stride); st != UG_OK) return st;
     if (a.residual) {
-      uint64_t dims[3] = {(uint64_t)a.n, (uint64_t)a.rows, (uint64_t)a.batch};
-      uint64_t bs = a.batch > 1 ? (uint64_t)a.res_batch_stride : (uint64_t)a.rows * a.res_row_stride;
-      uint64_t strides[2] = {(uint64_t)a.res_row_stride * 2, bs * 2};
-      int st = encode_tmap_bf16(&tma_r, a.residual, 3, dims, strides, box);
-      if (st != UG_OK) return st;
+      if (int st = rows_map(&tma_r, a.residual, rows0, a.res_row_stride, a.res_batch_stride); st != UG_OK) return st;
+    }
+    if (a.seg1_row0) {
+      uint64_t dims[3] = {(uint64_t)a.k, (uint64_t)a.n, 1};
+      uint64_t strides[2] = {(uint64_t)a.seg1_w_row_stride * 2, (uint64_t)a.n * a.seg1_w_row_stride * 2};
+      uint32_t box[3] = {(uint32_t)Cfg::BK, (uint32_t)Cfg::BN_LOAD, 1};
+      if (int st = encode_tmap_bf16(&tma_w1, a.seg1_w, 3, dims, strides, box); st != UG_OK) return st;
+      if (int st = rows_map(&tma_c1, a.seg1_c, rows1, a.seg1_c_row_stride, a.seg1_c_batch_stride); st != UG_OK) return st;
+      if (a.residual) {
+        if (int st = rows_map(&tma_r1, a.seg1_residual, rows1, a.seg1_res_row_stride, a.seg1_res_batch_stride); st != UG_OK) return st;
+      }
     }
   }
   GemmParams p;
@@ -708,6 +748,9 @@
   p.qk_d = a.qk_d; p.qk_eps = a.qk_eps;
   p.conv_cblocks = conv ? conv->c_in / Cfg::BK : 0;
   p.conv_w = conv ? conv->w : 0;
+  p.seg1_row0 = kTmaEpi ? a.seg1_row0 : 0;
+  p.bias1 = (const __nv_bfloat16*)a.seg1_bias; p.gate1 = a.seg1_gate;
+  p.qk_w1 = (const __nv_bfloat16*)a.seg1_qk_norm_weight; p.qk_cos_sin1 = a.seg1_qk_cos_sin;
   p.lora_t = a.lora_t; p.lora_t_rs = a.lora_t_row_stride; p.lora_t_bs = a.lora_t_batch_stride;
   p.lora_b = (const __nv_bfloat16*)a.lora_b;
   p.lora_r = a.lora_rank; p.lora_block_n = a.lora_block_n > 0 ? a.lora_block_n : a.n; p.lora_nseg = a.lora_nseg;
@@ -729,7 +772,7 @@
   attr[0].val.clusterDim.z = 1;
   cfg.attrs = attr;
   cfg.numAttrs = 1;
-  cudaError_t e = cudaLaunchKernelEx(&cfg, kern, tma_a, tma_w, tma_a2, tma_w2, tma_c, tma_r, p);
+  cudaError_t e = cudaLaunchKernelEx(&cfg, kern, tma_a, tma_w, tma_a2, tma_w2, tma_c, tma_r, tma_w1, tma_c1, tma_r1, p);
   if (e != cudaSuccess) {
     set_error("gemm: launch failed: %s", cudaGetErrorString(e));
     return UG_ERR_CUDA;
@@ -816,6 +859,28 @@
                      (a.batch == 1 || a.a2_batch_stride % 8 == 0),
                  "gemm: second operand pair strides must be multiples of 8 elements and cover k2");
   }
+  if (a.seg1_row0) {
+    UG_CHECK_ARG(a.seg1_row0 > 0 && a.seg1_row0 < a.rows, "gemm: seg1_row0 %d outside (0, rows = %d)", a.seg1_row0, a.rows);
+    UG_CHECK_ARG(a.seg1_w && a.seg1_c, "gemm: second row segment needs seg1_w and seg1_c");
+    UG_CHECK_ARG(!a.bias == !a.seg1_bias && !a.gate == !a.seg1_gate && !a.residual == !a.seg1_residual &&
+                     !a.qk_norm_weight == !a.seg1_qk_norm_weight && !a.qk_cos_sin == !a.seg1_qk_cos_sin,
+                 "gemm: the two row segments must use the same epilogue ops (bias / gate / residual / QK-norm / RoPE on both or neither)");
+    UG_CHECK_ARG(!a.lora_t && !a.colmask_block && !a.a2 && !a.gate_seg_stride && (a.w_batch_stride == 0 || a.batch == 1),
+                 "gemm: a second row segment does not compose with LoRA, colmask_block, a2, gate_seg_stride or batched W");
+    UG_CHECK_ARG(a.seg1_w_row_stride % 8 == 0 && a.seg1_w_row_stride >= a.k && a.seg1_c_row_stride % 8 == 0 &&
+                     a.seg1_c_row_stride >= a.n && (reinterpret_cast<uintptr_t>(a.seg1_c) & 15) == 0 &&
+                     (a.batch == 1 || a.seg1_c_batch_stride % 8 == 0),
+                 "gemm: seg1 weight / output strides must be multiples of 8 elements covering the row, C 16-byte aligned");
+    if (a.seg1_residual)
+      UG_CHECK_ARG(a.seg1_res_row_stride % 8 == 0 && (reinterpret_cast<uintptr_t>(a.seg1_residual) & 15) == 0 &&
+                       (a.batch == 1 || a.seg1_res_batch_stride % 8 == 0), "gemm: seg1 residual alignment");
+    if (a.seg1_bias) UG_CHECK_ARG((reinterpret_cast<uintptr_t>(a.seg1_bias) & 15) == 0, "gemm: seg1 bias alignment");
+    if (a.seg1_gate) UG_CHECK_ARG((reinterpret_cast<uintptr_t>(a.seg1_gate) & 15) == 0, "gemm: seg1 gate alignment");
+    if (a.seg1_qk_norm_weight)
+      UG_CHECK_ARG((reinterpret_cast<uintptr_t>(a.seg1_qk_norm_weight) & 15) == 0 &&
+                       (!a.seg1_qk_cos_sin || (reinterpret_cast<uintptr_t>(a.seg1_qk_cos_sin) & 15) == 0),
+                   "gemm: seg1 QK-norm operand alignment");
+  }
   cudaStream_t s = reinterpret_cast<cudaStream_t>(stream);
   int variant = a.variant;
   if (variant == 0) {
@@ -838,6 +903,24 @@
     UG_CHECK_ARG(!a.qk_norm_weight || (variant != 6 && a.qk_d % 128 == 0),
                  "gemm: the staged fused QK-norm epilogue needs a 256-column tile (variants 4 / 5) and qk_d a multiple of 128");
     UG_CHECK_ARG(!a.residual || a.res_batch_stride % 8 == 0 || a.batch == 1, "gemm: residual batch stride must be a multiple of 8");
+  }
+  if (a.seg1_row0) {
+    const int tile_rows = variant == 4 ? 256 : 128;
+    if (!(variant >= 4 && variant <= 6) || a.seg1_row0 % tile_rows != 0) {
+      ug_gemm_args g0 = a, g1 = a;
+      g0.seg1_row0 = 0;
+      g0.rows = a.seg1_row0;
+      g1.seg1_row0 = 0;
+      g1.rows = a.rows - a.seg1_row0;
+      g1.a = static_cast<const __nv_bfloat16*>(a.a) + (int64_t)a.seg1_row0 * a.a_row_stride;
+      g1.w = a.seg1_w; g1.w_row_stride = a.seg1_w_row_stride;
+      g1.bias = a.seg1_bias; g1.gate = a.seg1_gate;
+      g1.c = a.seg1_c; g1.c_row_stride = a.seg1_c_row_stride; g1.c_batch_stride = a.seg1_c_batch_stride;
+      g1.residual = a.seg1_residual; g1.res_row_stride = a.seg1_res_row_stride; g1.res_batch_stride = a.seg1_res_batch_stride;
+      g1.qk_norm_weight = a.seg1_qk_norm_weight; g1.qk_cos_sin = a.seg1_qk_cos_sin;
+      if (int st = ug_gemm_bf16(&g0, stream); st != UG_OK) return st;
+      return ug_gemm_bf16(&g1, stream);
+    }
   }
   switch (variant) {
     case 1: return launch_gemm<1, 256, 4>(a, s);
diff --git a/unigen_b200/model.py b/unigen_b200/model.py
--- a/unigen_b200/model.py
+++ b/unigen_b200/model.py
@@ -108,8 +108,6 @@
         self.attn_variant = 0
         self.overlap_mod_gemv = True
         self._side_stream = torch.cuda.Stream(device=self.device_)
-        self.overlap_text_stream = True
-        self._text_stream = torch.cuda.Stream(device=self.device_)
         self.fuse_qk_norm = True
         self.trace: Optional[Dict[str, torch.Tensor]] = None
         self.clone_outputs = True
@@ -512,45 +510,45 @@
         return self._attend(buf, S, buf.AO[:, :S])
 
     def _double_block(self, buf, w: _DoubleBlockW, mod_smp, mod_ctx, smp_in, ctx_in, smp_out, ctx_out, rope):
-        D = self.inner_dim
         B, n_smp, n_ctx = smp_in.shape[0], smp_in.shape[1], ctx_in.shape[1]
         S = n_ctx + n_smp
-        gv = self.gemm_variant
         sh_a, sc_a, g_a, sh_m, sc_m, g_m = mod_smp
         csh_a, csc_a, cg_a, csh_m, csc_m, cg_m = mod_ctx
         nx_c, nx_s = buf.NX[:, :n_ctx], buf.NX[:, n_ctx:S]
-        main = torch.cuda.current_stream()
-        side = self._text_stream if (self.overlap_text_stream and ctx_out is not None and n_ctx and n_smp
-                                     and not getattr(self, "_sp_active", False)) else None
         if n_ctx:
-            if side is not None:
-                side.wait_stream(main)
-            with torch.cuda.stream(side if side is not None else main):
-                ops.ln_modulate(ctx_in, nx_c, csh_a, csc_a)
-                ops.gemm(nx_c, w.add_qkv[0], out=buf.QKV[:, :n_ctx], bias=w.add_qkv[1], variant=gv,
-                         qk_norm=self._qk_norm(w.rms_ctx, rope[:n_ctx] if rope is not None else None))
+            ops.ln_modulate(ctx_in, nx_c, csh_a, csc_a)
         if n_smp:
             ops.ln_modulate(smp_in, nx_s, sh_a, sc_a)
-            ops.gemm(nx_s, w.qkv[0], out=buf.QKV[:, n_ctx:S], bias=w.qkv[1], variant=gv,
-                     qk_norm=self._qk_norm(w.rms, rope[n_ctx:S] if rope is not None else None))
-        if side is not None:
-            main.wait_stream(side)
+        self._gemm_rows(buf.NX, 0, n_ctx, n_smp,
+                        dict(w=w.add_qkv[0], out=buf.QKV[:, :n_ctx], bias=w.add_qkv[1],
+                             qk_norm=self._qk_norm(w.rms_ctx, rope[:n_ctx] if rope is not None else None)),
+                        dict(w=w.qkv[0], out=buf.QKV[:, n_ctx:S], bias=w.qkv[1],
+                             qk_norm=self._qk_norm(w.rms, rope[n_ctx:S] if rope is not None else None)))
         ao = self._joint_attention(buf, B, n_ctx, n_smp, w.rms_ctx, w.rms, rope)
-        if ctx_out is not None and n_ctx:
-            if side is not None:
-                side.wait_stream(main)
-            with torch.cuda.stream(side if side is not None else main):
-                ops.gemm(ao[:, :n_ctx], w.to_add_out[0], out=ctx_out, bias=w.to_add_out[1], gate=cg_a, residual=ctx_in, variant=gv)
-                ops.ln_modulate(ctx_out, nx_c, csh_m, csc_m)
-                ops.gemm(nx_c, w.ffc1[0], out=buf.FF[:, :n_ctx], bias=w.ffc1[1], act=UG_ACT_GELU_TANH, variant=gv)
-                ops.gemm(buf.FF[:, :n_ctx], w.ffc2[0], out=ctx_out, bias=w.ffc2[1], gate=cg_m, residual=ctx_out, variant=gv)
+        r0 = 0 if ctx_out is not None else n_ctx
+        self._gemm_rows(ao, r0, n_ctx - r0, n_smp,
+                        dict(w=w.to_add_out[0], out=ctx_out, bias=w.to_add_out[1], gate=cg_a, residual=ctx_in),
+                        dict(w=w.to_out[0], out=smp_out, bias=w.to_out[1], gate=g_a, residual=smp_in))
+        if n_ctx > r0:
+            ops.ln_modulate(ctx_out, nx_c, csh_m, csc_m)
         if n_smp:
-            ops.gemm(ao[:, n_ctx:S], w.to_out[0], out=smp_out, bias=w.to_out[1], gate=g_a, residual=smp_in, variant=gv)
             ops.ln_modulate(smp_out, nx_s, sh_m, sc_m)
-            ops.gemm(nx_s, w.ff1[0], out=buf.FF[:, n_ctx:S], bias=w.ff1[1], act=UG_ACT_GELU_TANH, variant=gv)
-            ops.gemm(buf.FF[:, n_ctx:S], w.ff2[0], out=smp_out, bias=w.ff2[1], gate=g_m, residual=smp_out, variant=gv)
-        if side is not None:
-            main.wait_stream(side)
+        self._gemm_rows(buf.NX, r0, n_ctx - r0, n_smp,
+                        dict(w=w.ffc1[0], out=buf.FF[:, :n_ctx], bias=w.ffc1[1], act=UG_ACT_GELU_TANH),
+                        dict(w=w.ff1[0], out=buf.FF[:, n_ctx:S], bias=w.ff1[1], act=UG_ACT_GELU_TANH))
+        self._gemm_rows(buf.FF, r0, n_ctx - r0, n_smp,
+                        dict(w=w.ffc2[0], out=ctx_out, bias=w.ffc2[1], gate=cg_m, residual=ctx_out),
+                        dict(w=w.ff2[0], out=smp_out, bias=w.ff2[1], gate=g_m, residual=smp_out))
+
+    def _gemm_rows(self, src: torch.Tensor, r0: int, n_ctx: int, n_smp: int, ctx: dict, smp: dict):
+        gv = self.gemm_variant
+        a = src[:, r0:r0 + n_ctx + n_smp]
+        if n_ctx and n_smp:
+            ops.gemm(a, variant=gv, **ctx, seg1=dict(row0=n_ctx, **{k: v for k, v in smp.items() if k != "act"}))
+        elif n_ctx:
+            ops.gemm(a, variant=gv, **ctx)
+        elif n_smp:
+            ops.gemm(a, variant=gv, **smp)
 
     def _single_attention(self, buf, S: int, rms: torch.Tensor, rope, out: torch.Tensor):
         a, D = self.arch, self.inner_dim
diff --git a/unigen_b200/ops.py b/unigen_b200/ops.py
--- a/unigen_b200/ops.py
+++ b/unigen_b200/ops.py
@@ -73,7 +73,8 @@
          gate: Optional[torch.Tensor] = None, alpha: float = 1.0, act: int = UG_ACT_NONE,
          residual: Optional[torch.Tensor] = None, variant: int = 0, lora: Optional[dict] = None,
          qk_norm: Optional[dict] = None, gate_seg_stride: int = 0, seg_bounds: Optional[Sequence[int]] = None,
-         a2: Optional[torch.Tensor] = None, w2: Optional[torch.Tensor] = None, colmask: Optional[dict] = None) -> torch.Tensor:
+         a2: Optional[torch.Tensor] = None, w2: Optional[torch.Tensor] = None, colmask: Optional[dict] = None,
+         seg1: Optional[dict] = None) -> torch.Tensor:
     a = _view3(_dev(a, "gemm.a", BF16), "gemm.a")
     _dev(w, "gemm.w", BF16)
     B, R, K = a.shape
@@ -147,11 +148,51 @@
         cs = qk_norm.get("cos_sin")
         if cs is not None:
             _dev(cs, "gemm.qk_norm.cos_sin", torch.float32)
-            if cs.shape[0] < R or not cs.is_contiguous():
+            if cs.shape[0] < (int(seg1["row0"]) if seg1 is not None else R) or not cs.is_contiguous():
                 raise UgError("gemm: qk_norm cos_sin table too short / not contiguous")
             g.qk_cos_sin = cs.data_ptr()
+    if seg1 is not None:
+        _gemm_seg1(g, seg1, B, R, N, K, qk_norm)
     check(_lib.load().ug_gemm_bf16(C.byref(g), _stream()), "ug_gemm_bf16")
     return out
+
+
+def _gemm_seg1(g: GemmArgs, seg1: dict, B: int, R: int, N: int, K: int, qk_norm: Optional[dict]) -> None:
+    row0 = int(seg1["row0"])
+    w1 = _dev(seg1["w"], "gemm.seg1.w", BF16)
+    if tuple(w1.shape) != (N, K) or w1.stride(1) != 1:
+        raise UgError(f"gemm: seg1 w {tuple(w1.shape)} must be [{N}, {K}] with unit inner stride")
+    o1 = _view3(_dev(seg1["out"], "gemm.seg1.out", BF16), "gemm.seg1.out")
+    g.seg1_row0 = row0
+    g.seg1_w, g.seg1_w_row_stride = w1.data_ptr(), w1.stride(0)
+    g.seg1_c, g.seg1_c_row_stride, g.seg1_c_batch_stride = o1.data_ptr(), o1.stride(1), o1.stride(0)
+    b1 = seg1.get("bias")
+    if b1 is not None:
+        if b1.dim() != 1 or g.bias_batch_stride:
+            raise UgError("gemm: seg1 takes a 1-D bias shared by all batches (as the first segment's)")
+        g.seg1_bias = _dev(b1, "gemm.seg1.bias", BF16).data_ptr()
+    g1 = seg1.get("gate")
+    if g1 is not None:
+        _dev(g1, "gemm.seg1.gate", torch.float32)
+        g1 = g1 if g1.dim() == 2 else g1.unsqueeze(0)
+        if B > 1 and g1.stride(0) != g.gate_batch_stride:
+            raise UgError("gemm: the two segments' gates must share one batch stride")
+        g.seg1_gate = g1.data_ptr()
+    r1 = seg1.get("residual")
+    if r1 is not None:
+        r13 = _view3(_dev(r1, "gemm.seg1.residual", BF16), "gemm.seg1.residual")
+        g.seg1_residual, g.seg1_res_row_stride, g.seg1_res_batch_stride = r13.data_ptr(), r13.stride(1), r13.stride(0)
+    q1 = seg1.get("qk_norm")
+    if q1 is not None:
+        if qk_norm is None or (int(q1["head_dim"]), int(q1["d"])) != (int(qk_norm["head_dim"]), int(qk_norm["d"])):
+            raise UgError("gemm: seg1 qk_norm must match the first segment's head_dim / d")
+        g.seg1_qk_norm_weight = _dev(q1["weight"], "gemm.seg1.qk_norm.weight", BF16).data_ptr()
+        cs = q1.get("cos_sin")
+        if cs is not None:
+            _dev(cs, "gemm.seg1.qk_norm.cos_sin", torch.float32)
+            if cs.shape[0] < R - row0 or not cs.is_contiguous():
+                raise UgError("gemm: seg1 qk_norm cos_sin table too short / not contiguous")
+            g.seg1_qk_cos_sin = cs.data_ptr()
 
 
 def lora_down(x: torch.Tensor, a_stack: torch.Tensor, seg_bounds: Sequence[int], seg_group: Sequence[int],
```
